# alanqrwang/nwhead

Measured on AMD Instinct MI355X. Metric: query-predictions/sec, higher is better.
Workload: dtype f32; 1 GPU; K3 predict('full'): B=256 queries/step vs bank N=50000 d=512 C=200, bank sharded 1-way, 26 query batches coalesced per launch; B=256, N_support=50000, d=512, C=200, parallelism=support-shard x1

## Files before the change

include/nwhead_hip.h:

```cpp
#ifndef NWHEAD_HIP_H
#define NWHEAD_HIP_H

#include <stddef.h>
#include <stdint.h>

#ifdef __cplusplus
extern "C" {
#endif

#define NW_ABI_VERSION 2

typedef enum {
    NW_SCORE_EUCLIDEAN = 0,
    NW_SCORE_HYPERSPHERE = 1,
    NW_SCORE_COSINE = 2,
    NW_SCORE_DOT = 3,
    NW_SCORE_CLIP = 4
} nw_score_kind;

typedef enum {
    NW_OK = 0,
    NW_ERR_INVALID_ARG = -1,
    NW_ERR_UNSUPPORTED = -2,
    NW_ERR_WORKSPACE = -3,
    NW_ERR_LAUNCH = -4,
    NW_ERR_NO_DEVICE = -5
} nw_status;

int nw_abi_version(void);
const char *nw_status_string(int status);
int nw_device_check(void);

int nw_scores_f32(const float *q, const float *s, float *scores,
                  int64_t B, int64_t N, int64_t d,
                  int kind, const float *logit_scale_dev, int sup_batched, void *stream);

int nw_row_norm2_f32(const float *x, float *n2, int64_t rows, int64_t d, void *stream);

int nw_split_rows_f16x2(const float *x, float *out_split, float *row_scale, float *row_norm2,
                        int64_t rows, int64_t d, void *stream);

int nw_pack_rows_f16(const float *x, uint16_t *out_rows, float *row_scale, float *row_norm2,
                     int64_t rows, int64_t d, void *stream);

int nw_bank_update_rows_f32(const float *x, const int64_t *rows, int64_t R, int64_t dx, float momentum,
                            float *s_rows, float *s_user, float *s_norm2,
                            float *s_split, float *s_scale,
                            void *s_f16, float *f16_scale, float *f16_norm2,
                            int64_t N, int64_t d, void *stream);

typedef struct nw_fwd_opts {
    uint32_t struct_size;
    int32_t persistent_wgs;
    int32_t force_split;
    int32_t operand_form;
    const void *tables;
    size_t tables_bytes;
    const int64_t *tables_sy;
    int64_t tables_N;
} nw_fwd_opts;

size_t nw_fwd_workspace_bytes(int64_t B, int64_t N, int64_t d, int64_t C);
int nw_fwd_f32(const float *q, const float *s, const int64_t *sy, const float *s_norm2,
               const float *s_split, const float *s_scale,
               float *out, float *scores_out, float *lse_out, float *weights_out,
               void *workspace, size_t workspace_bytes,
               int64_t B, int64_t N, int64_t d, int64_t C,
               int kind, const float *logit_scale_dev,
               int sup_batched, int labels_batched, const nw_fwd_opts *opts, void *stream);

int nw_fwd_partial_f32(const float *q, const float *s, const int64_t *sy, const float *s_norm2,
                       const float *s_split, const float *s_scale,
                       float *m, float *den, float *num,
                       void *workspace, size_t workspace_bytes,
                       int64_t B, int64_t N, int64_t d, int64_t C,
                       int kind, const float *logit_scale_dev, const nw_fwd_opts *opts, void *stream);
int nw_merge_finalize_f32(const float *m, const float *den, const float *num, float *out,
                          int64_t G, int64_t B, int64_t C,
                          int64_t stride_m, int64_t stride_den, int64_t stride_num,
                          const int64_t *class_lo, int64_t C_local, void *stream);

size_t nw_bank_tables_bytes(int64_t N);
int nw_bank_tables_build(const int64_t *sy, int64_t N, int64_t C, void *tables, size_t tables_bytes, void *stream);


size_t nw_bwd_workspace_bytes(int64_t B, int64_t N, int64_t d, int64_t C, int kind, int sup_batched);
int nw_bwd_f32(const float *q, const float *s, const int64_t *sy,
               const float *scores, const float *lse, const float *out, const float *gout,
               float *gq, float *gs, float *glogit_scale,
               void *workspace, size_t workspace_bytes,
               int64_t B, int64_t N, int64_t d, int64_t C,
               int kind, const float *logit_scale_dev,
               int sup_batched, int labels_batched, void *stream);
int nw_bwd_uses_split(int64_t B, int64_t N, int64_t d, int64_t C, int sup_batched);
int nw_bwd_bank_f32(const float *q, const float *s, const float *s_norm2, const float *s_split,
                    const float *s_scale, const int64_t *sy,
                    const float *scores, const float *lse, const float *out, const float *gout,
                    float *gq, float *gs, float *glogit_scale,
                    void *workspace, size_t workspace_bytes,
                    int64_t B, int64_t N, int64_t d, int64_t C,
                    int kind, const float *logit_scale_dev,
                    int sup_batched, int labels_batched, void *stream);


int nw_support_influence_f32(const float *probs, const int64_t *qy, const float *w,
                             const int64_t *sy, float *infl,
                             int64_t B, int64_t N, int64_t C, void *stream);

int nw_aggregate_f32(const float *scores, const int64_t *sy, float *out, float *lse_out, float *weights_out,
                     int64_t B, int64_t N, int64_t C, int labels_batched, void *stream);
int nw_aggregate_bwd_f32(const float *scores, const int64_t *sy, const float *lse, const float *out, const float *gout,
                         float *gscores, int64_t B, int64_t N, int64_t C, int labels_batched, void *stream);

int nw_fwd_influence_f32(const float *q, const float *s, const int64_t *sy, const float *s_norm2,
                         const float *s_split, const float *s_scale, const int64_t *qy,
                         float *out, float *lse_out, float *infl_out,
                         void *workspace, size_t workspace_bytes,
                         int64_t B, int64_t N, int64_t d, int64_t C,
                         int kind, const float *logit_scale_dev, const nw_fwd_opts *opts, void *stream);

int nw_topk_f32(const float *scores, int64_t *idx_out, float *val_out,
                int64_t B, int64_t N, int64_t k, void *stream);

size_t nw_knn_workspace_bytes(int64_t B, int64_t N, int64_t d, int64_t k);
int nw_knn_f32(const float *q, const float *s_split, const float *s_scale, const float *s_norm2,
               int64_t *idx_out, float *val_out, void *workspace, size_t workspace_bytes,
               int64_t B, int64_t N, int64_t d, int64_t k, int kind, const float *logit_scale_dev,
               void *stream);
int nw_knn_window_f32(const float *q, const float *s_split, const float *s_scale, const float *s_norm2,
                      const int32_t *row_lo, const int32_t *row_hi, int exclude,
                      int64_t *idx_out, float *val_out, void *workspace, size_t workspace_bytes,
                      int64_t B, int64_t N, int64_t d, int64_t k, int kind, const float *logit_scale_dev,
                      void *stream);
int nw_fwd_window_f32(const float *q, const float *s_split, const float *s_scale, const float *s_norm2,
                      const int64_t *sy, const int32_t *row_lo, const int32_t *row_hi, int exclude,
                      float *out, float *lse_out, void *workspace, size_t workspace_bytes,
                      int64_t B, int64_t N, int64_t d, int64_t C, int kind, const float *logit_scale_dev,
                      void *stream);
size_t nw_bwd_query_workspace_bytes(int64_t B, int64_t N, int64_t d, int64_t C, int row_chunks);
int nw_bwd_query_f32(const float *q, const float *s_split, const float *s_scale, const float *s_norm2,
                     const int64_t *sy, const int32_t *row_lo, const int32_t *row_hi, int exclude,
                     const float *lse, const float *out, const float *gout,
                     float *gq, float *glogit_scale, void *workspace, size_t workspace_bytes,
                     int64_t B, int64_t N, int64_t d, int64_t C, int kind, const float *logit_scale_dev,
                     int row_chunks, void *stream);
int nw_fwd_weighted_f32(const float *q, const float *s_split, const float *s_scale, const float *s_norm2,
                        const int64_t *sy, const float *row_logw,
                        const int32_t *row_lo, const int32_t *row_hi, int exclude,
                        float *out, float *lse_out, void *workspace, size_t workspace_bytes,
                        int64_t B, int64_t N, int64_t d, int64_t C, int kind, const float *logit_scale_dev, void *stream);
int nw_bwd_query_weighted_f32(const float *q, const float *s_split, const float *s_scale, const float *s_norm2,
                              const int64_t *sy, const float *row_logw,
                              const int32_t *row_lo, const int32_t *row_hi, int exclude,
                              const float *lse, const float *out, const float *gout,
                              float *gq, float *glogit_scale, void *workspace, size_t workspace_bytes,
                              int64_t B, int64_t N, int64_t d, int64_t C, int kind, const float *logit_scale_dev,
                              int row_chunks, void *stream);
size_t nw_bwd_logw_workspace_bytes(int64_t B, int64_t N, int64_t d, int64_t C, int row_chunks, int want_gq);
int nw_bwd_query_logw_f32(const float *q, const float *s_split, const float *s_scale, const float *s_norm2,
                          const int64_t *sy, const float *row_logw,
                          const int32_t *row_lo, const int32_t *row_hi, int exclude,
                          const float *lse, const float *out, const float *gout,
                          float *gq, float *glogw, float *glogit_scale, void *workspace, size_t workspace_bytes,
                          int64_t B, int64_t N, int64_t d, int64_t C, int kind, const float *logit_scale_dev,
                          int row_chunks, void *stream);
size_t nw_fwd_values_workspace_bytes(int64_t B, int64_t N, int64_t d, int64_t T, int row_chunks);
int nw_fwd_values_f32(const float *q, const float *s_split, const float *s_scale, const float *s_norm2,
                      const float *v_split, const float *v_scale, const float *row_logw,
                      const int32_t *row_lo, const int32_t *row_hi, int exclude,
                      const float *lse, float *out, void *workspace, size_t workspace_bytes,
                      int64_t B, int64_t N, int64_t d, int64_t T, int kind, const float *logit_scale_dev,
                      int row_chunks, void *stream);
size_t nw_bwd_values_query_workspace_bytes(int64_t B, int64_t N, int64_t d, int64_t T, int row_chunks);
int nw_bwd_values_query_f32(const float *q, const float *s_split, const float *s_scale, const float *s_norm2,
                            const float *v_split, const float *v_scale, const float *row_logw,
                            const int32_t *row_lo, const int32_t *row_hi, int exclude,
                            const float *lse, const float *out, const float *gout,
                            float *gq, float *glogit_scale, void *workspace, size_t workspace_bytes,
                            int64_t B, int64_t N, int64_t d, int64_t T, int kind, const float *logit_scale_dev,
                            int row_chunks, void *stream);
size_t nw_bwd_values_support_workspace_bytes(int64_t B, int64_t N, int64_t d, int64_t T, int query_chunks, int want_gvalues);
int nw_bwd_values_support_f32(const float *q, const float *s_split, const float *s_scale, const float *s_norm2,
                              const float *v_rows, const float *row_logw,
                              const int32_t *row_lo, const int32_t *row_hi, int exclude,
                              const float *lse, const float *out, const float *gout,
                              float *gvalues, float *glogw, void *workspace, size_t workspace_bytes,
                              int64_t B, int64_t N, int64_t d, int64_t T, int kind, const float *logit_scale_dev,
                              int query_chunks, void *stream);
int nw_influence_select_f32(const float *vals, const int64_t *rows, const int64_t *sy, const int64_t *qy,
                            const float *out, const float *lse, float *infl_out, int64_t *label_out,
                            int64_t B, int64_t k, int64_t N, int64_t C, void *stream);
int nw_scores_use_split(int64_t B, int64_t N, int64_t d);

size_t nw_knn_f16_workspace_bytes(int64_t B, int64_t N, int64_t d, int64_t k);
int nw_knn_f16(const float *q, const void *s_f16, const float *s_scale, const float *s_norm2,
               int64_t *idx_out, float *val_out, void *workspace, size_t workspace_bytes,
               int64_t B, int64_t N, int64_t d, int64_t k, int kind, const float *logit_scale_dev,
               const nw_fwd_opts *opts, void *stream);

int nw_knn_merge_f32(const float *vals, const int32_t *rows, const int32_t *labels,
                     int64_t G, int64_t B, int64_t kc, int64_t stride_g, int64_t k, int64_t C,
                     int64_t *idx_out, float *val_out, int64_t *label_out, float *out, void *stream);

int nw_scale_shift_relu_f32(const float *x, const float *scale, const float *shift, float *out,
                            int64_t n, int64_t c, int64_t hw, int64_t x_batch_stride, int relu,
                            void *stream);
int nw_scale_shift_relu_avgpool2_f32(const float *x, const float *scale, const float *shift, float *out,
                                     int64_t n, int64_t c, int64_t h, int64_t w, int64_t x_batch_stride,
                                     int relu, void *stream);

int nw_bias_act_nhwc_f32(const float *x, const float *bias, const float *residual, int relu, float *out,
                         int64_t rows, int64_t c, void *stream);

size_t nw_conv1x1_workspace_bytes(int64_t n, int64_t cin, int64_t cout, int64_t hw);
int nw_conv1x1_f32(const float *x, int64_t x_batch_stride, const float *pre_scale, const float *pre_shift,
                   int pre_relu, const float *w_t, const float *bias, int post_relu, float *out,
                   int64_t out_batch_stride, void *workspace, size_t workspace_bytes,
                   int64_t n, int64_t cin, int64_t cout, int64_t hw, void *stream);

size_t nw_conv3x3_workspace_bytes(int64_t n, int64_t cin, int64_t cout, int64_t H, int64_t W);
int nw_conv3x3_f32(const float *x, int64_t x_batch_stride, const float *w_t, const float *bias,
                   const float *residual, int64_t res_batch_stride, int post_relu, float *out,
                   int64_t out_batch_stride, void *workspace, size_t workspace_bytes,
                   int64_t n, int64_t cin, int64_t cout, int64_t H, int64_t W, void *stream);
int64_t nw_conv3x3_workgroups(int64_t n, int64_t cin, int64_t cout, int64_t H, int64_t W);


#define NW_AMAX_SLOTS 256
int nw_absmax_f32(const float *x, int64_t count, float *amax_out, void *stream);
int nw_to_nhwc_pad_f32(const float *x, float *y, float *amax_out, int64_t n, int64_t c, int64_t hw, int64_t cp,
                       int64_t stride_n, int64_t stride_c, int64_t stride_p, void *stream);
int nw_conv2d_nhwc_supported(int64_t n, int64_t H, int64_t W, int64_t Cin, int64_t Cout, int64_t KH, int64_t KW,
                             int64_t stride, int64_t pad);
int nw_conv2d_nhwc_f16x2(const float *x, const float *amax_in, const float *w_split, const float *w_scale,
                         const float *bias, const float *residual, int relu, float *y, float *amax_out,
                         int64_t n, int64_t H, int64_t W, int64_t Cin, int64_t Cout, int64_t KH, int64_t KW,
                         int64_t stride, int64_t pad, int64_t ldx, int64_t ldy, float *moments, void *stream);
int nw_conv2d_nhwc_bnrelu_f16x2(const float *x, const float *pre, const float *amax_in, int64_t raw_records,
                                const float *w_split, const float *w_scale, const float *bias, int relu, float *y,
                                float *amax_out, int64_t n,
                                int64_t H, int64_t W, int64_t Cin, int64_t Cout, int64_t KH, int64_t KW, int64_t stride,
                                int64_t pad, int64_t ldx, int64_t ldy, float *moments, void *stream);
int64_t nw_conv2d_nhwc_moments_groups(int64_t n, int64_t H, int64_t W, int64_t Cin, int64_t Cout, int64_t KH, int64_t KW,
                                      int64_t stride, int64_t pad);

int nw_bn_relu_train_fwd_f32(const float *x, const float *residual, const float *gamma, const float *beta, float *running_mean,
                             float *running_var, float *y, float *save_mean, float *save_invstd,
                             int64_t *num_batches_tracked, int64_t n, int64_t c, int64_t hw,
                             int64_t x_batch_stride, float momentum, float eps, int relu, void *stream);
int nw_bn_relu_train_bwd_f32(const float *x, const float *residual, const float *dy, const float *gamma,
                             const float *beta, const float *save_mean, const float *save_invstd, float *dx,
                             float *dresidual, float *dgamma, float *dbeta, const float *acc,
                             int64_t acc_batch_stride, int64_t n, int64_t c, int64_t hw,
                             int64_t x_batch_stride, int relu, void *stream);

int nw_split_conv_weights_f16x2(const int64_t *jobs, int64_t njobs, int64_t total_rows, float *split_base,
                                float *scale_base, void *stream);

int nw_conv2d_nhwc_wgrad_supported(int64_t n, int64_t H, int64_t W, int64_t Cin, int64_t Cout, int64_t KH, int64_t KW,
                                   int64_t stride, int64_t pad);
size_t nw_conv2d_nhwc_wgrad_workspace_bytes(int64_t n, int64_t H, int64_t W, int64_t Cin, int64_t Cout, int64_t KH,
                                            int64_t KW, int64_t stride, int64_t pad);
int nw_conv2d_nhwc_wgrad_f16x2(const float *x, const float *amax_x, const float *gy, const float *amax_g, float *dw,
                               void *workspace, size_t workspace_bytes, int64_t n, int64_t H, int64_t W, int64_t Cin,
                               int64_t Cout, int64_t KH, int64_t KW, int64_t stride, int64_t pad, int64_t ldx, int64_t ldg,
                               void *stream);
typedef struct nw_wgrad_job {
    const float *x, *amax_x, *gy, *amax_g;
    float *dw;
    int64_t n, H, W, Cin, Cout, KH, KW, stride, pad, ldx, ldg;
    int64_t out_oihw;
    const float *pre_x;
    int64_t rowrun_stride, in_H, in_W, row0, col0;
} nw_wgrad_job;
size_t nw_conv2d_nhwc_wgrad_batch_workspace_bytes(const nw_wgrad_job *jobs, int64_t njobs);
int nw_conv2d_nhwc_wgrad_batch_f16x2(const nw_wgrad_job *jobs, int64_t njobs, void *workspace, size_t workspace_bytes,
                                     void *stream);
const void *nw_conv_zero_page(void);

size_t nw_bn_nhwc_workspace_bytes(int64_t rows, int64_t c);
int nw_bn_relu_nhwc_train_fwd_f32(const float *x, int64_t ldx, const float *gamma, const float *beta, float *running_mean,
                                  float *running_var, float *y, float *save_mean, float *save_invstd,
                                  int64_t *num_batches_tracked, float *amax_out, void *workspace, size_t workspace_bytes,
                                  int64_t rows, int64_t c, float momentum, float eps, int relu, void *stream);
int nw_bn_nhwc_moments_f32(const float *x, int64_t ldx, int64_t rows, int64_t c, float eps, float *mean, float *invstd,
                           float *var, void *workspace, size_t workspace_bytes, void *stream);
int nw_bn_nhwc_moments_from_partials_f32(float *partials, int64_t groups, int64_t c, float eps, float *mean,
                                         float *invstd, float *var, void *stream);
int nw_bn_nhwc_moments_minmax_f32(const float *x, int64_t ldx, int64_t rows, int64_t c, float eps, float *mean, float *invstd,
                                  float *var, float *vmin, float *vmax, void *workspace, size_t workspace_bytes, void *stream);
size_t nw_bn_nhwc_minmax_workspace_bytes(int64_t rows, int64_t c);
int nw_bn_nhwc_prep_from_partials_f32(float *partials, int64_t groups, int64_t c, float eps, float *mean, float *invstd,
                                      float *var, float *vmin, float *vmax, const float *gamma, const float *beta,
                                      float *running_mean, float *running_var, int64_t *num_batches_tracked, float momentum,
                                      int relu, float *tab, float *amax_out, void *stream);
int nw_bn_nhwc_prep_window_from_partials_f32(float *partials, int64_t groups, int64_t c, int64_t offset, int64_t n_old, int64_t rows,
                                             float eps, float *mean, float *invstd, float *var, float *vmin, float *vmax,
                                             const float *gamma, const float *beta, float *running_mean, float *running_var,
                                             int64_t *num_batches_tracked, float momentum, int relu, float *tab, float *amax_out,
                                             void *stream);
int nw_bn_nhwc_prep_f32(const float *mean, const float *invstd, const float *var, const float *vmin, const float *vmax,
                        const float *gamma, const float *beta, float *running_mean, float *running_var,
                        int64_t *num_batches_tracked, float momentum, int relu, int64_t rows, int64_t c, float *tab,
                        float *amax_out, void *stream);
int nw_bn_relu_nhwc_apply_f32(const float *x, int64_t ldx, const float *mean, const float *invstd, const float *var,
                              const float *gamma, const float *beta, float *running_mean, float *running_var,
                              int64_t *num_batches_tracked, float momentum, float *y, float *amax_out, int64_t rows,
                              int64_t c, int relu, void *stream);
int nw_stem7x7s2_relu_maxpool_supported(int64_t n, int64_t H, int64_t W, int64_t cout);
int nw_stem7x7s2_relu_maxpool_f16x2(const float *x4, const float *amax_in, const float *w_split, const float *w_scale,
                                    const float *bias, float *y, float *amax_out, int64_t n, int64_t H, int64_t W, int64_t ldy,
                                    void *stream);
int nw_bn_relu_avgpool2x2_nhwc_f32(const float *x, int64_t ldx, const float *tab, float *y, int64_t ldy, float *amax_out,
                                   int64_t n, int64_t h, int64_t w, int64_t c, void *stream);
int nw_add_relu_f32(const float *a, const float *b, float *out, float *amax_out, int64_t count, void *stream);
int nw_relu_bwd_f32(const float *out, const float *g, float *dx, float *amax_out, int64_t count, void *stream);
int nw_bn_relu_nhwc_train_bwd_f32(const float *x, int64_t ldx, const float *dy, const float *gamma, const float *beta,
                                  const float *save_mean, const float *save_invstd, float *dx, float *dgamma,
                                  float *dbeta, const float *acc, int64_t ldacc, int64_t lddx, float *amax_out,
                                  void *workspace, size_t workspace_bytes, int64_t rows, int64_t c, int relu, void *stream);

int nw_avgpool2x2_nhwc_f32(const float *x, int64_t ldx, float *y, int64_t ldy, int64_t n, int64_t h, int64_t w, int64_t c,
                           void *stream);
int nw_avgpool2x2_nhwc_bwd_f32(const float *gy, int64_t ldgy, float *gx, int64_t ldgx, int64_t n, int64_t h, int64_t w,
                               int64_t c, void *stream);
int nw_maxpool3x3s2_nhwc_f32(const float *x, int64_t ldx, float *y, int64_t ldy, unsigned char *tap, int64_t n, int64_t h,
                             int64_t w, int64_t c, void *stream);
int nw_maxpool3x3s2_nhwc_bwd_f32(const float *gy, int64_t ldgy, const unsigned char *tap, float *gx, int64_t ldgx, int64_t n,
                                 int64_t h, int64_t w, int64_t c, void *stream);

typedef struct nw_sgd_param {
    float *param;
    const float *grad;
    float *momentum_buf;
    int64_t n;
} nw_sgd_param;
int nw_sgd_step_f32(const nw_sgd_param *params, int64_t nparams, float lr, float momentum, float weight_decay, int nesterov,
                    int init_buf, void *stream);

int nw_debug_tile_timing(int enable);
int nw_debug_set(const char *name, int value);
int nw_debug_tile_timing_read(double *total_us, int64_t *launches);
typedef struct nw_fwd_plan {
    int32_t status;
    int32_t rs, bs, n_stiles, n_qtiles, grid;
    int32_t mode, out;
    int32_t dma, persistent, variant, workgroups, qgroup;
    int32_t split_queries, run_tables;
    int32_t reserved;
    uint64_t lds_bytes;
} nw_fwd_plan;
int nw_debug_fwd_plan(int64_t B, int64_t N, int64_t d, int64_t C, int form, int outputs, int k, int norms, int kind,
                      int persistent_wgs, int cus, nw_fwd_plan *plan);
#define NW_FWD_AREAS 6
typedef struct nw_fwd_layout {
    uint64_t off[NW_FWD_AREAS], bytes[NW_FWD_AREAS];
    uint64_t total;
    int32_t n_slices, reserved;
} nw_fwd_layout;
int nw_debug_fwd_layout(int64_t B, int64_t N, int64_t d, int64_t C, nw_fwd_layout *layout);
#define NW_BWD_AREAS 15
typedef struct nw_bwd_plan {
    int32_t status, route;
    int32_t coeff_threads, parts_shared;
    int32_t gq_chunks, gq_k_chunk, gs_chunks, gs_k_chunk;
    int64_t ld, Bpad;
    uint64_t coeff_lds_bytes;
    uint64_t off[NW_BWD_AREAS], bytes[NW_BWD_AREAS];
    uint64_t total;
} nw_bwd_plan;
int nw_debug_bwd_plan(int64_t B, int64_t N, int64_t d, int64_t C, int sup_batched, nw_bwd_plan *plan);

#ifdef __cplusplus
}
#endif
#endif
```

nwhead_amd/_lib.py:

```python
from __future__ import annotations

import ctypes as C
import os

_HERE = os.path.dirname(os.path.abspath(__file__))
LIB_PATH = os.environ.get("NW_HIP_LIB") or os.path.join(_HERE, "csrc", "libnwhead_hip.so")

SCORE_KINDS = {"euclidean": 0, "hypersphere_euclidean": 1, "cosine": 2, "dotproduct": 3, "clip": 4}

_p = C.c_void_p
_i64 = C.c_int64
_int = C.c_int
_sz = C.c_size_t

SIGNATURES = {
    "nw_abi_version": (_int, []),
    "nw_status_string": (C.c_char_p, [_int]),
    "nw_device_check": (_int, []),
    "nw_scores_f32": (_int, [_p, _p, _p, _i64, _i64, _i64, _int, _p, _int, _p]),
    "nw_fwd_workspace_bytes": (_sz, [_i64, _i64, _i64, _i64]),
    "nw_row_norm2_f32": (_int, [_p, _p, _i64, _i64, _p]),
    "nw_split_rows_f16x2": (_int, [_p, _p, _p, _p, _i64, _i64, _p]),
    "nw_pack_rows_f16": (_int, [_p, _p, _p, _p, _i64, _i64, _p]),
    "nw_bank_update_rows_f32": (_int, [_p, _p, _i64, _i64, C.c_float, _p, _p, _p, _p, _p, _p, _p, _p, _i64, _i64, _p]),
    "nw_fwd_f32": (_int, [_p, _p, _p, _p, _p, _p, _p, _p, _p, _p, _p, _sz, _i64, _i64, _i64, _i64, _int, _p, _int, _int, _p, _p]),
    "nw_fwd_partial_f32": (_int, [_p, _p, _p, _p, _p, _p, _p, _p, _p, _p, _sz, _i64, _i64, _i64, _i64, _int, _p, _p, _p]),
    "nw_merge_finalize_f32": (_int, [_p, _p, _p, _p, _i64, _i64, _i64, _i64, _i64, _i64, _p, _i64, _p]),
    "nw_bank_tables_bytes": (_sz, [_i64]),
    "nw_bank_tables_build": (_int, [_p, _i64, _i64, _p, _sz, _p]),
    "nw_bwd_workspace_bytes": (_sz, [_i64, _i64, _i64, _i64, _int, _int]),
    "nw_bwd_f32": (_int, [_p] * 10 + [_p, _sz, _i64, _i64, _i64, _i64, _int, _p, _int, _int, _p]),
    "nw_bwd_uses_split": (_int, [_i64, _i64, _i64, _i64, _int]),
    "nw_bwd_bank_f32": (_int, [_p] * 13 + [_p, _sz, _i64, _i64, _i64, _i64, _int, _p, _int, _int, _p]),
    "nw_support_influence_f32": (_int, [_p, _p, _p, _p, _p, _i64, _i64, _i64, _p]),
    "nw_aggregate_f32": (_int, [_p] * 5 + [_i64, _i64, _i64, _int, _p]),
    "nw_aggregate_bwd_f32": (_int, [_p] * 6 + [_i64, _i64, _i64, _int, _p]),
    "nw_fwd_influence_f32": (_int, [_p] * 11 + [_sz, _i64, _i64, _i64, _i64, _int, _p, _p, _p]),
    "nw_topk_f32": (_int, [_p, _p, _p, _i64, _i64, _i64, _p]),
    "nw_knn_workspace_bytes": (_sz, [_i64, _i64, _i64, _i64]),
    "nw_scores_use_split": (_int, [_i64, _i64, _i64]),
    "nw_knn_f32": (_int, [_p, _p, _p, _p, _p, _p, _p, _sz, _i64, _i64, _i64, _i64, _int, _p, _p]),
    "nw_knn_window_f32": (_int, [_p, _p, _p, _p, _p, _p, _int, _p, _p, _p, _sz, _i64, _i64, _i64, _i64, _int, _p, _p]),
    "nw_fwd_window_f32": (_int, [_p, _p, _p, _p, _p, _p, _p, _int, _p, _p, _p, _sz, _i64, _i64, _i64, _i64, _int, _p, _p]),
    "nw_fwd_weighted_f32": (_int, [_p, _p, _p, _p, _p, _p, _p, _p, _int, _p, _p, _p, _sz, _i64, _i64, _i64, _i64, _int, _p, _p]),
    "nw_bwd_query_workspace_bytes": (_sz, [_i64, _i64, _i64, _i64, _int]),
    "nw_bwd_query_f32": (_int, [_p, _p, _p, _p, _p, _p, _p, _int, _p, _p, _p, _p, _p, _p, _sz, _i64, _i64, _i64, _i64, _int, _p, _int, _p]),
    "nw_bwd_query_weighted_f32": (_int, [_p, _p, _p, _p, _p, _p, _p, _p, _int, _p, _p, _p, _p, _p, _p, _sz, _i64, _i64, _i64, _i64, _int, _p,
                                         _int, _p]),
    "nw_bwd_logw_workspace_bytes": (_sz, [_i64, _i64, _i64, _i64, _int, _int]),
    "nw_bwd_query_logw_f32": (_int, [_p, _p, _p, _p, _p, _p, _p, _p, _int, _p, _p, _p, _p, _p, _p, _p, _sz, _i64, _i64, _i64, _i64, _int,
                                     _p, _int, _p]),
    "nw_fwd_values_workspace_bytes": (_sz, [_i64, _i64, _i64, _i64, _int]),
    "nw_fwd_values_f32": (_int, [_p, _p, _p, _p, _p, _p, _p, _p, _p, _int, _p, _p, _p, _sz, _i64, _i64, _i64, _i64, _int, _p, _int, _p]),
    "nw_bwd_values_query_workspace_bytes": (_sz, [_i64, _i64, _i64, _i64, _int]),
    "nw_bwd_values_query_f32": (_int, [_p, _p, _p, _p, _p, _p, _p, _p, _p, _int, _p, _p, _p, _p, _p, _p, _sz, _i64, _i64, _i64, _i64,
                                       _int, _p, _int, _p]),
    "nw_bwd_values_support_workspace_bytes": (_sz, [_i64, _i64, _i64, _i64, _int, _int]),
    "nw_bwd_values_support_f32": (_int, [_p, _p, _p, _p, _p, _p, _p, _p, _int, _p, _p, _p, _p, _p, _p, _sz, _i64, _i64, _i64, _i64,
                                         _int, _p, _int, _p]),
    "nw_influence_select_f32": (_int, [_p] * 8 + [_i64, _i64, _i64, _i64, _p]),
    "nw_knn_f16_workspace_bytes": (_sz, [_i64, _i64, _i64, _i64]),
    "nw_knn_f16": (_int, [_p, _p, _p, _p, _p, _p, _p, _sz, _i64, _i64, _i64, _i64, _int, _p, _p, _p]),
    "nw_knn_merge_f32": (_int, [_p, _p, _p, _i64, _i64, _i64, _i64, _i64, _i64, _p, _p, _p, _p, _p]),
    "nw_scale_shift_relu_f32": (_int, [_p, _p, _p, _p, _i64, _i64, _i64, _i64, _int, _p]),
    "nw_bias_act_nhwc_f32": (_int, [_p, _p, _p, _int, _p, _i64, _i64, _p]),
    "nw_scale_shift_relu_avgpool2_f32": (_int, [_p, _p, _p, _p, _i64, _i64, _i64, _i64, _i64, _int, _p]),
    "nw_conv3x3_workgroups": (_i64, [_i64, _i64, _i64, _i64, _i64]),
    "nw_conv3x3_workspace_bytes": (_sz, [_i64, _i64, _i64, _i64, _i64]),
    "nw_conv3x3_f32": (_int, [_p, _i64, _p, _p, _p, _i64, _int, _p, _i64, _p, _sz, _i64, _i64, _i64, _i64, _i64, _p]),
    "nw_conv1x1_workspace_bytes": (_sz, [_i64, _i64, _i64, _i64]),
    "nw_conv1x1_f32": (_int, [_p, _i64, _p, _p, _int, _p, _p, _int, _p, _i64, _p, _sz, _i64, _i64, _i64, _i64, _p]),
    "nw_bn_relu_train_fwd_f32": (_int, [_p] * 10 + [_i64, _i64, _i64, _i64, C.c_float, C.c_float, _int, _p]),
    "nw_bn_relu_train_bwd_f32": (_int, [_p] * 12 + [_i64, _i64, _i64, _i64, _i64, _int, _p]),
    "nw_absmax_f32": (_int, [_p, _i64, _p, _p]),
    "nw_to_nhwc_pad_f32": (_int, [_p, _p, _p, _i64, _i64, _i64, _i64, _i64, _i64, _i64, _p]),
    "nw_conv2d_nhwc_supported": (_int, [_i64] * 9),
    "nw_conv2d_nhwc_f16x2": (_int, [_p, _p, _p, _p, _p, _p, _int, _p, _p] + [_i64] * 11 + [_p, _p]),
    "nw_conv2d_nhwc_moments_groups": (_i64, [_i64] * 9),
    "nw_stem7x7s2_relu_maxpool_supported": (_int, [_i64] * 4),
    "nw_stem7x7s2_relu_maxpool_f16x2": (_int, [_p] * 7 + [_i64] * 4 + [_p]),
    "nw_bn_relu_avgpool2x2_nhwc_f32": (_int, [_p, _i64, _p, _p, _i64, _p, _i64, _i64, _i64, _i64, _p]),
    "nw_add_relu_f32": (_int, [_p, _p, _p, _p, _i64, _p]),
    "nw_relu_bwd_f32": (_int, [_p, _p, _p, _p, _i64, _p]),
    "nw_bn_nhwc_moments_f32": (_int, [_p, _i64, _i64, _i64, C.c_float, _p, _p, _p, _p, _sz, _p]),
    "nw_bn_nhwc_moments_from_partials_f32": (_int, [_p, _i64, _i64, C.c_float, _p, _p, _p, _p]),
    "nw_bn_nhwc_moments_minmax_f32": (_int, [_p, _i64, _i64, _i64, C.c_float, _p, _p, _p, _p, _p, _p, _sz, _p]),
    "nw_bn_nhwc_minmax_workspace_bytes": (_sz, [_i64, _i64]),
    "nw_bn_nhwc_prep_from_partials_f32": (_int, [_p, _i64, _i64, C.c_float, _p, _p, _p, _p, _p, _p, _p, _p, _p, _p, C.c_float, _int,
                                                 _p, _p, _p]),
    "nw_bn_nhwc_prep_window_from_partials_f32": (_int, [_p, _i64, _i64, _i64, _i64, _i64, C.c_float, _p, _p, _p, _p, _p, _p, _p, _p, _p,
                                                        _p, C.c_float, _int, _p, _p, _p]),
    "nw_bn_nhwc_prep_f32": (_int, [_p, _p, _p, _p, _p, _p, _p, _p, _p, _p, C.c_float, _int, _i64, _i64, _p, _p, _p]),
    "nw_conv2d_nhwc_bnrelu_f16x2": (_int, [_p] * 3 + [_i64] + [_p] * 3 + [_int, _p, _p] + [_i64] * 11 + [_p, _p]),
    "nw_bn_relu_nhwc_apply_f32": (_int, [_p, _i64] + [_p] * 8 + [C.c_float, _p, _p, _i64, _i64, _int, _p]),
    "nw_split_conv_weights_f16x2": (_int, [_p, _i64, _i64, _p, _p, _p]),
    "nw_conv2d_nhwc_wgrad_supported": (_int, [_i64] * 9),
    "nw_conv2d_nhwc_wgrad_workspace_bytes": (_sz, [_i64] * 9),
    "nw_conv2d_nhwc_wgrad_f16x2": (_int, [_p, _p, _p, _p, _p, _p, _sz] + [_i64] * 11 + [_p]),
    "nw_conv_zero_page": (_p, []),
    "nw_conv2d_nhwc_wgrad_batch_workspace_bytes": (_sz, [_p, _i64]),
    "nw_conv2d_nhwc_wgrad_batch_f16x2": (_int, [_p, _i64, _p, _sz, _p]),
    "nw_bn_nhwc_workspace_bytes": (_sz, [_i64, _i64]),
    "nw_bn_relu_nhwc_train_fwd_f32": (_int, [_p, _i64] + [_p] * 10 + [_sz, _i64, _i64, C.c_float, C.c_float, _int, _p]),
    "nw_bn_relu_nhwc_train_bwd_f32": (_int, [_p, _i64] + [_p] * 9 + [_i64, _i64, _p, _p, _sz, _i64, _i64, _int, _p]),
    "nw_avgpool2x2_nhwc_f32": (_int, [_p, _i64, _p, _i64, _i64, _i64, _i64, _i64, _p]),
    "nw_avgpool2x2_nhwc_bwd_f32": (_int, [_p, _i64, _p, _i64, _i64, _i64, _i64, _i64, _p]),
    "nw_maxpool3x3s2_nhwc_f32": (_int, [_p, _i64, _p, _i64, _p, _i64, _i64, _i64, _i64, _p]),
    "nw_maxpool3x3s2_nhwc_bwd_f32": (_int, [_p, _i64, _p, _p, _i64, _i64, _i64, _i64, _i64, _p]),
    "nw_sgd_step_f32": (_int, [_p, _i64, C.c_float, C.c_float, C.c_float, _int, _int, _p]),
    "nw_debug_set": (_int, [C.c_char_p, _int]),
    "nw_debug_tile_timing": (_int, [_int]),
    "nw_debug_tile_timing_read": (_int, [C.POINTER(C.c_double), C.POINTER(C.c_int64)]),
    "nw_debug_fwd_plan": (_int, [_i64, _i64, _i64, _i64, _int, _int, _int, _int, _int, _int, _int, _p]),
    "nw_debug_fwd_layout": (_int, [_i64, _i64, _i64, _i64, _p]),
    "nw_debug_bwd_plan": (_int, [_i64, _i64, _i64, _i64, _int, _p]),
}

_lib = None


class NWHipError(RuntimeError):
    pass


def load():
    global _lib
    if _lib is not None:
        return _lib
    if not os.path.exists(LIB_PATH):
        raise NWHipError(
            f"{LIB_PATH} not found: the HIP extension is not built. Run __graft_entry__.build() "
            "(or `make -C nwhead_amd/csrc`). There is no CPU fallback.")
    import torch
    lib = C.CDLL(LIB_PATH)
    for name, (res, args) in SIGNATURES.items():
        fn = getattr(lib, name)
        fn.restype = res
        fn.argtypes = args
    if lib.nw_abi_version() != 2:
        raise NWHipError("libnwhead_hip.so ABI version mismatch")
    _lib = lib
    sync_knobs()
    return lib


class WgradJob(C.Structure):
    _fields_ = [("x", C.c_void_p), ("amax_x", C.c_void_p), ("gy", C.c_void_p), ("amax_g", C.c_void_p), ("dw", C.c_void_p)] + \
               [(k, C.c_int64) for k in ("n", "H", "W", "Cin", "Cout", "KH", "KW", "stride", "pad", "ldx", "ldg", "out_oihw")] + \
               [("pre_x", C.c_void_p)] + [(k, C.c_int64) for k in ("rowrun_stride", "in_H", "in_W", "row0", "col0")]


class SgdParam(C.Structure):
    _fields_ = [("param", C.c_void_p), ("grad", C.c_void_p), ("momentum_buf", C.c_void_p), ("n", C.c_int64)]


class FwdOpts(C.Structure):
    _fields_ = [("struct_size", C.c_uint32), ("persistent_wgs", C.c_int32), ("force_split", C.c_int32),
                ("operand_form", C.c_int32), ("tables", C.c_void_p), ("tables_bytes", C.c_size_t),
                ("tables_sy", C.c_void_p), ("tables_N", C.c_int64)]


class FwdPlan(C.Structure):
    _fields_ = [(k, C.c_int32) for k in ("status", "rs", "bs", "n_stiles", "n_qtiles", "grid", "mode", "out", "dma", "persistent",
                                         "variant", "workgroups", "qgroup", "split_queries", "run_tables", "reserved")] + \
               [("lds_bytes", C.c_uint64)]


FORMS = {"fp32": 0, "split": 1, "half": 2}
OUTPUTS = {"log_probs": 0, "scores": 1, "candidates": 2}


def fwd_plan(B, N, d, C_, form="split", outputs="log_probs", k=0, norms=True, kind="euclidean", persistent_wgs=0, cus=0):
    p = FwdPlan()
    check(load().nw_debug_fwd_plan(B, N, d, C_, FORMS[form], OUTPUTS[outputs], k, int(norms), SCORE_KINDS[kind],
                                   persistent_wgs, cus, C.byref(p)), "nw_debug_fwd_plan")
    return p


FWD_AREAS = ("main", "q_rows", "q_scale", "q_norm2", "lse", "slices")


class FwdLayout(C.Structure):
    _fields_ = [("off", C.c_uint64 * len(FWD_AREAS)), ("bytes", C.c_uint64 * len(FWD_AREAS)), ("total", C.c_uint64),
                ("n_slices", C.c_int32), ("reserved", C.c_int32)]


def fwd_layout(B, N, d, C_):
    m = FwdLayout()
    check(load().nw_debug_fwd_layout(B, N, d, C_, C.byref(m)), "nw_debug_fwd_layout")
    return m


BWD_ROUTES = ("valu", "mfma", "split")
BWD_AREAS = ("A", "Rs", "rq", "gls", "qn2", "sn2", "rs", "s_split", "s_scale", "q_split", "ascale", "qv", "gfac", "part", "part2")


class BwdPlan(C.Structure):
    _fields_ = [(k, C.c_int32) for k in ("status", "route", "coeff_threads", "parts_shared", "gq_chunks", "gq_k_chunk",
                                         "gs_chunks", "gs_k_chunk")] + \
               [("ld", C.c_int64), ("Bpad", C.c_int64), ("coeff_lds_bytes", C.c_uint64),
                ("off", C.c_uint64 * len(BWD_AREAS)), ("bytes", C.c_uint64 * len(BWD_AREAS)), ("total", C.c_uint64)]


def bwd_plan(B, N, d, C_, sup=0):
    p = BwdPlan()
    check(load().nw_debug_bwd_plan(B, N, d, C_, int(sup), C.byref(p)), "nw_debug_bwd_plan")
    return p


KNOBS = ("pvar", "qg", "tile_rs", "no_persistent", "split_queries", "bwd_no_mfma", "bwd_split",
         "xgemm_wgs", "split_lbits", "conv_max_wgs", "conv_skip_cfgs", "conv_force_cfg")
_KNOB_UNSET = -2 ** 31
_knob_state = {}


def sync_knobs():
    if _lib is None:
        return
    for k in KNOBS:
        v = os.environ.get("NW_" + k.upper())
        val = _KNOB_UNSET if v is None or v == "" else int(v)
        if _knob_state.get(k, _KNOB_UNSET) != val:
            _lib.nw_debug_set(k.encode(), val)
            _knob_state[k] = val


def force_split():
    return os.environ.get("NW_SPLIT_ALWAYS", "") == "1"


def fwd_opts(tables=None, tables_bytes=0, persistent_wgs=0, tables_sy=None, tables_n=-1, operand_form=0):
    return FwdOpts(C.sizeof(FwdOpts), int(persistent_wgs), int(force_split()), int(operand_form), tables, int(tables_bytes),
                   tables_sy, int(tables_n))


def check(status: int, what: str):
    if status != 0:
        msg = load().nw_status_string(status).decode()
        raise NWHipError(f"{what}: {msg} (status {status})")
```

nwhead_amd/csrc/capi.hip:

```cpp
#include <cstddef>
#include <cstdlib>
#include <string.h>
#include "nw_internal.h"
#include "fused_plan.h"
#include "bwd_plan.h"

namespace {
inline bool bad_kind(int kind) { return kind < NW_SCORE_EUCLIDEAN || kind > NW_SCORE_CLIP; }
}

extern "C" int nw_scores_use_split(int64_t B, int64_t N, int64_t d);
static bool split_pays(int64_t B, int64_t N, int64_t d) {
    return nw::fwd_opts().force_split || nw_scores_use_split(B, N, d) != 0;
}
static bool takes_split(const float* q, const float* s_split, const float* s_scale, const float* s_norm2, int64_t B, int64_t N,
                        int64_t d) {
    return s_split && s_scale && s_norm2 && d % 32 == 0 && split_pays(B, N, d) &&
           ((reinterpret_cast<uintptr_t>(s_split) | reinterpret_cast<uintptr_t>(q)) & 15) == 0;
}

namespace nw {
namespace {
thread_local FwdOpts tl_fwd_opts;
int g_knobs[KNOB_COUNT];
bool g_knobs_init = [] { for (int& k : g_knobs) k = KNOB_UNSET; return true; }();
const char* const knob_names[KNOB_COUNT] = {
    "pvar", "qg", "tile_rs", "no_persistent", "split_queries", "bwd_no_mfma", "bwd_split",
    "xgemm_wgs", "split_lbits", "conv_max_wgs", "conv_skip_cfgs", "conv_force_cfg"};
}
const FwdOpts& fwd_opts() { return tl_fwd_opts; }
int knob(int id) { return (id >= 0 && id < KNOB_COUNT) ? __atomic_load_n(&g_knobs[id], __ATOMIC_RELAXED) : KNOB_UNSET; }
}

namespace {
struct OptsGuard {
    nw::FwdOpts saved;
    explicit OptsGuard(const nw_fwd_opts* o) : saved(nw::tl_fwd_opts) {
        nw::FwdOpts f;
        if (o && o->struct_size >= offsetof(nw_fwd_opts, tables)) {
            f.persistent_wgs = o->persistent_wgs;
            f.force_split = o->force_split;
            f.operand_form = o->operand_form;
        }
        if (o && o->struct_size >= sizeof(nw_fwd_opts)) {
            f.tables = static_cast<const char*>(o->tables);
            f.tables_bytes = o->tables_bytes;
            f.tables_sy = o->tables_sy;
            f.tables_N = o->tables_N;
        }
        nw::tl_fwd_opts = f;
    }
    ~OptsGuard() { nw::tl_fwd_opts = saved; }
};
}

static int half_form_check(const float* q, const float* s, const float* s_norm2, const float* s_split, const float* s_scale,
                           const void* per_pair_out, int batched, int64_t B, int64_t N, int64_t d, int64_t C) {
    if (per_pair_out || batched) return NW_ERR_UNSUPPORTED;
    if (!nw::half_form_shape_ok(d)) return NW_ERR_UNSUPPORTED;
    if (B == 0 || N == 0 || C == 0) return NW_OK;
    if (!s_split || !s_scale || !s_norm2) return NW_ERR_INVALID_ARG;
    if ((reinterpret_cast<uintptr_t>(s_split) | reinterpret_cast<uintptr_t>(q)) & 15) return NW_ERR_INVALID_ARG;
    if (!nw::fused_eligible(q, s_split, B, N, d, C)) return NW_ERR_UNSUPPORTED;
    (void)s;
    return NW_OK;
}

extern "C" int nw_debug_set(const char* name, int value) {
    if (!name) return NW_ERR_INVALID_ARG;
    for (int k = 0; k < nw::KNOB_COUNT; ++k)
        if (!strcmp(name, nw::knob_names[k])) {
            __atomic_store_n(&nw::g_knobs[k], value, __ATOMIC_RELAXED);
            return NW_OK;
        }
    return NW_ERR_INVALID_ARG;
}

extern "C" int nw_debug_fwd_plan(int64_t B, int64_t N, int64_t d, int64_t C, int form, int outputs, int k, int norms, int kind,
                                 int persistent_wgs, int cus, nw_fwd_plan* plan) {
    if (!plan || B < 0 || N < 0 || d < 0 || C < 0 || k < 0 || cus < 0 || cus > (1 << 20)) return NW_ERR_INVALID_ARG;
    if (form < nw::FORM_F32 || form > nw::FORM_HALF || outputs < nw::OUT_NONE || outputs > nw::OUT_CAND) return NW_ERR_INVALID_ARG;
    if (bad_kind(kind)) return NW_ERR_UNSUPPORTED;
    nw::FwdOpts o;
    o.persistent_wgs = persistent_wgs;
    const nw::FusedPlan p = nw::plan_fused(B, N, d, C, form, outputs, k, norms != 0, kind == NW_SCORE_DOT, cus, o);
    *plan = {p.status, p.rs, p.BS, p.n_stiles, p.n_qtiles, p.grid, p.mode, p.out, p.dma, p.persistent, p.variant, p.workgroups,
             p.qgroup, p.split_queries, p.run_tables, 0, (uint64_t)p.lds_bytes};
    return NW_OK;
}

extern "C" int nw_abi_version(void) { return NW_ABI_VERSION; }

extern "C" const char* nw_status_string(int status) {
    switch (status) {
        case NW_OK: return "ok";
        case NW_ERR_INVALID_ARG: return "invalid argument";
        case NW_ERR_UNSUPPORTED: return "unsupported score kind or size";
        case NW_ERR_WORKSPACE: return "workspace too small";
        case NW_ERR_LAUNCH: return "HIP launch failed";
        case NW_ERR_NO_DEVICE: return "no gfx950 device";
        default: return "unknown status";
    }
}

extern "C" int nw_device_check(void) {
    int n = 0;
    if (hipGetDeviceCount(&n) != hipSuccess || n <= 0) return NW_ERR_NO_DEVICE;
    int dev = 0;
    if (hipGetDevice(&dev) != hipSuccess) return NW_ERR_NO_DEVICE;
    hipDeviceProp_t prop;
    if (hipGetDeviceProperties(&prop, dev) != hipSuccess) return NW_ERR_NO_DEVICE;
    return strncmp(prop.gcnArchName, "gfx950", 6) == 0 ? NW_OK : NW_ERR_NO_DEVICE;
}

extern "C" int nw_scores_f32(const float* q, const float* s, float* scores, int64_t B, int64_t N,
                             int64_t d, int kind, const float* logit_scale_dev, int sup_batched,
                             void* stream) {
    if (B < 0 || N < 0 || d < 0) return NW_ERR_INVALID_ARG;
    if (bad_kind(kind)) return NW_ERR_UNSUPPORTED;
    if (B == 0 || N == 0) return NW_OK;
    if (!q || !s || !scores) return NW_ERR_INVALID_ARG;
    if (kind == NW_SCORE_CLIP && !logit_scale_dev) return NW_ERR_INVALID_ARG;
    return nw::launch_scores(q, s, scores, B, N, d, kind, logit_scale_dev, sup_batched,
                             static_cast<hipStream_t>(stream));
}

extern "C" size_t nw_fwd_workspace_bytes(int64_t B, int64_t N, int64_t d, int64_t C) {
    return nw::fwd_layout(B, N, d, C, nullptr).total;
}

extern "C" int nw_debug_fwd_layout(int64_t B, int64_t N, int64_t d, int64_t C, nw_fwd_layout* layout) {
    if (!layout || B < 0 || N < 0 || d < 0 || C < 0) return NW_ERR_INVALID_ARG;
    const nw::FwdLayout L = nw::fwd_layout(B, N, d, C, nullptr);
    const nw::FwdLayout::Area* const areas[NW_FWD_AREAS] = {&L.main, &L.q_rows, &L.q_scale, &L.q_norm2, &L.lse, &L.slices};
    *layout = {};
    for (int i = 0; i < NW_FWD_AREAS; ++i) layout->off[i] = areas[i]->off, layout->bytes[i] = areas[i]->bytes;
    layout->total = L.total;
    layout->n_slices = L.n_slices;
    return NW_OK;
}

extern "C" int nw_debug_bwd_plan(int64_t B, int64_t N, int64_t d, int64_t C, int sup_batched, nw_bwd_plan* plan) {
    static_assert(NW_BWD_AREAS == nw::BWD_AREAS, "nw_bwd_plan lists the areas of nw::BwdPlan");
    if (!plan || B < 0 || N < 0 || d < 0 || C < 0) return NW_ERR_INVALID_ARG;
    const nw::BwdPlan p = nw::plan_bwd(B, N, d, C, sup_batched);
    *plan = {};
    plan->status = p.status, plan->route = p.route, plan->coeff_threads = (int32_t)p.coeff_threads, plan->parts_shared = p.parts_shared;
    plan->gq_chunks = p.gq.nchunks, plan->gq_k_chunk = p.gq.k_chunk, plan->gs_chunks = p.gs.nchunks, plan->gs_k_chunk = p.gs.k_chunk;
    plan->ld = p.ld, plan->Bpad = p.Bpad, plan->coeff_lds_bytes = p.coeff_lds, plan->total = p.total;
    for (int i = 0; i < NW_BWD_AREAS; ++i) plan->off[i] = p.area[i].off, plan->bytes[i] = p.area[i].bytes;
    return NW_OK;
}

extern "C" int nw_row_norm2_f32(const float* x, float* n2, int64_t rows, int64_t d, void* stream) {
    if (rows < 0 || d < 0) return NW_ERR_INVALID_ARG;
    if (rows == 0) return NW_OK;
    if (!x || !n2) return NW_ERR_INVALID_ARG;
    return nw::launch_rownorm2(x, n2, rows, d, static_cast<hipStream_t>(stream));
}

static int fwd_f32(const float* q, const float* s, const int64_t* sy, const float* s_norm2, const float* s_split,
                   const float* s_scale, float* out, float* scores_out, float* lse_out, float* weights_out, void* workspace,
                   size_t workspace_bytes, const nw::FwdLayout* carved, int64_t B, int64_t N, int64_t d, int64_t C, int kind,
                   const float* logit_scale_dev, int sup_batched, int labels_batched, hipStream_t st) {
    if (B < 0 || N < 0 || d < 0 || C < 0) return NW_ERR_INVALID_ARG;
    if (bad_kind(kind)) return NW_ERR_UNSUPPORTED;
    if (B == 0) return NW_OK;
    if (!out && C > 0) return NW_ERR_INVALID_ARG;
    if (N > 0 && (!q || !s || !sy)) return NW_ERR_INVALID_ARG;
    if (kind == NW_SCORE_CLIP && !logit_scale_dev) return NW_ERR_INVALID_ARG;
    if (labels_batched && !sup_batched) return NW_ERR_INVALID_ARG;
    const int form = nw::fwd_opts().operand_form;
    if (form != 0 && form != 1) return NW_ERR_INVALID_ARG;
    const nw::FwdLayout L = carved ? *carved : nw::fwd_layout(B, N, d, C, workspace);
    nw::FusedArgs a = {q, s, sy, s_norm2, nullptr, logit_scale_dev, out, scores_out, lse_out, nullptr, nullptr, nullptr,
                       &L, (int)B, (int)N, (int)d, (int)C, st, nullptr};
    if (form == 1) {
        const int rc = half_form_check(q, s, s_norm2, s_split, s_scale, scores_out ? scores_out : weights_out,
                                       sup_batched || labels_batched, B, N, d, C);
        if (rc != NW_OK) return rc;
        if (N > 0 && C > 0) {
            if (!L.fits(workspace_bytes)) return NW_ERR_WORKSPACE;
            a.s = s_split, a.s_scale = s_scale;
            return nw::launch_fused(a, nw::FORM_HALF, kind);
        }
    }
    float* sc_buf = scores_out ? scores_out : weights_out;
    if (N > 0 && C > 0 && !sup_batched && nw::fused_eligible(q, s, B, N, d, C) &&
        (!sc_buf || (reinterpret_cast<uintptr_t>(sc_buf) & 15) == 0)) {
        if (!L.fits(workspace_bytes)) return NW_ERR_WORKSPACE;
        a.scores = sc_buf;
        if (weights_out && !a.lse) a.lse = L.at(L.lse);
        const bool split = takes_split(q, s_split, s_scale, s_norm2, B, N, d);
        if (split) a.s = s_split, a.s_scale = s_scale;
        const int rc = nw::launch_fused(a, split ? nw::FORM_SPLIT : nw::FORM_F32, kind);
        if (rc != NW_OK || !weights_out) return rc;
        return nw::launch_weights_from_scores(sc_buf, a.lse, weights_out, B, N, st);
    }
    float* scores = scores_out;
    if (!scores && N > 0) {
        if (!L.fits(workspace_bytes)) return NW_ERR_WORKSPACE;
        scores = L.at(L.main);
    }
    int rc = nw::launch_scores(q, s, scores, B, N, d, kind, logit_scale_dev, sup_batched, st);
    if (rc != NW_OK) return rc;
    const bool sliced = L.n_slices > 1 && L.fits(workspace_bytes);
    return nw::launch_aggregate(scores, sy, labels_batched, out, lse_out, weights_out, nullptr, nullptr, nullptr, B, N, C, st,
                                sliced ? L.at(L.slices) : nullptr, sliced ? L.slices.bytes / sizeof(float) : 0);
}

extern "C" int nw_fwd_f32(const float* q, const float* s, const int64_t* sy, const float* s_norm2,
                          const float* s_split, const float* s_scale, float* out, float* scores_out, float* lse_out, float* weights_out, void* workspace,
                          size_t workspace_bytes, int64_t B, int64_t N, int64_t d, int64_t C,
                          int kind, const float* logit_scale_dev, int sup_batched,
                          int labels_batched, const nw_fwd_opts* opts, void* stream) {
    OptsGuard opts_guard(opts);
    return fwd_f32(q, s, sy, s_norm2, s_split, s_scale, out, scores_out, lse_out, weights_out, workspace, workspace_bytes, nullptr,
                   B, N, d, C, kind, logit_scale_dev, sup_batched, labels_batched, static_cast<hipStream_t>(stream));
}

bool nw::bank_head_shape_ok(int64_t N, int64_t d, int64_t C) { return N > 25 && C >= 1 && d >= 32 && d % 32 == 0 && d <= (1 << 20); }

namespace {
enum { NEED_WINDOW = 1, NEED_LOGW = 2, NEED_GQ = 4, NEED_GLOGW = 8 };
inline uintptr_t addr(const void* p) { return reinterpret_cast<uintptr_t>(p); }

struct BankFwdCall {
    const float *q, *s_split, *s_scale, *s_norm2;
    const int64_t* sy;
    const float* row_logw;
    const int32_t *row_lo, *row_hi;
    int exclude;
    float *out, *lse_out;
    void* workspace;
    size_t workspace_bytes;
    int64_t B, N, d, C;
    int kind;
    const float* logit_scale_dev;
    void* stream;
};
int bank_fwd_checked(const BankFwdCall& c, int needs) {
    if (c.B < 0 || c.N < 0 || c.d < 0 || c.C < 0) return NW_ERR_INVALID_ARG;
    if ((c.row_lo != nullptr) != (c.row_hi != nullptr) || ((needs & NEED_WINDOW) && !c.row_lo)) return NW_ERR_INVALID_ARG;
    if (bad_kind(c.kind)) return NW_ERR_UNSUPPORTED;
    if (!nw::bank_head_shape_ok(c.N, c.d, c.C)) return NW_ERR_UNSUPPORTED;
    if (c.B == 0) return NW_OK;
    if (!c.q || !c.s_split || !c.s_scale || !c.s_norm2 || !c.sy || !c.out || ((needs & NEED_LOGW) && !c.row_logw))
        return NW_ERR_INVALID_ARG;
    if (c.kind == NW_SCORE_CLIP && !c.logit_scale_dev) return NW_ERR_INVALID_ARG;
    if (!nw::fused_eligible(c.q, c.s_split, c.B, c.N, c.d, c.C)) return NW_ERR_UNSUPPORTED;
    if (addr(c.row_logw) & 15) return NW_ERR_UNSUPPORTED;
    const nw::FwdLayout L = nw::fwd_layout(c.B, c.N, c.d, c.C, c.workspace);
    if (!L.fits(c.workspace_bytes)) return NW_ERR_WORKSPACE;
    if (addr(c.workspace) & 15) return NW_ERR_UNSUPPORTED;
    nw::FusedArgs a = {c.q, c.s_split, c.sy, c.s_norm2, c.s_scale, c.logit_scale_dev, c.out, nullptr, c.lse_out, nullptr, nullptr,
                       nullptr, &L, (int)c.B, (int)c.N, (int)c.d, (int)c.C, static_cast<hipStream_t>(c.stream), nullptr,
                       c.row_lo, c.row_hi, c.row_lo && c.exclude != 0, c.row_logw};
    return nw::launch_fused(a, nw::FORM_SPLIT, c.kind);
}

int bank_bwd_checked(const nw::BwdQueryCall& c, int needs) {
    if (c.B < 0 || c.N < 0 || c.d < 0 || c.C < 0 || c.row_chunks < 0) return NW_ERR_INVALID_ARG;
    if ((c.row_lo != nullptr) != (c.row_hi != nullptr)) return NW_ERR_INVALID_ARG;
    if (bad_kind(c.kind)) return NW_ERR_UNSUPPORTED;
    if (!nw::bwd_query_shape_ok(c.B, c.N, c.d, c.C)) return NW_ERR_UNSUPPORTED;
    if (c.B == 0) return NW_OK;
    if (!c.q || !c.s_split || !c.s_scale || !c.s_norm2 || !c.sy || !c.lse || !c.out || !c.gout ||
        ((needs & NEED_LOGW) && !c.row_logw) || ((needs & NEED_GQ) && !c.gq) || ((needs & NEED_GLOGW) && !c.glogw))
        return NW_ERR_INVALID_ARG;
    if (c.kind == NW_SCORE_CLIP && !c.logit_scale_dev) return NW_ERR_INVALID_ARG;
    if ((addr(c.q) | addr(c.s_split) | addr(c.gq) | addr(c.row_logw) | addr(c.glogw)) & 15) return NW_ERR_UNSUPPORTED;
    const size_t need = c.glogw ? nw::bwd_logw_workspace_bytes(c.B, c.N, c.d, c.C, c.row_chunks, c.gq != nullptr)
                                : nw::bwd_query_workspace_bytes(c.B, c.N, c.d, c.C, c.row_chunks);
    if (!c.workspace || c.workspace_bytes < need) return NW_ERR_WORKSPACE;
    if (addr(c.workspace) & 15) return NW_ERR_UNSUPPORTED;
    return nw::launch_bwd_query(c);
}
}

extern "C" int nw_fwd_window_f32(const float* q, const float* s_split, const float* s_scale, const float* s_norm2,
                                 const int64_t* sy, const int32_t* row_lo, const int32_t* row_hi, int exclude, float* out,
                                 float* lse_out, void* workspace, size_t workspace_bytes, int64_t B, int64_t N, int64_t d,
                                 int64_t C, int kind, const float* logit_scale_dev, void* stream) {
    return bank_fwd_checked({q, s_split, s_scale, s_norm2, sy, nullptr, row_lo, row_hi, exclude, out, lse_out, workspace,
                             workspace_bytes, B, N, d, C, kind, logit_scale_dev, stream}, NEED_WINDOW);
}

extern "C" int nw_fwd_weighted_f32(const float* q, const float* s_split, const float* s_scale, const float* s_norm2,
                                   const int64_t* sy, const float* row_logw, const int32_t* row_lo, const int32_t* row_hi,
                                   int exclude, float* out, float* lse_out, void* workspace, size_t workspace_bytes, int64_t B,
                                   int64_t N, int64_t d, int64_t C, int kind, const float* logit_scale_dev, void* stream) {
    return bank_fwd_checked({q, s_split, s_scale, s_norm2, sy, row_logw, row_lo, row_hi, exclude, out, lse_out, workspace,
                             workspace_bytes, B, N, d, C, kind, logit_scale_dev, stream}, NEED_LOGW);
}

extern "C" size_t nw_bwd_query_workspace_bytes(int64_t B, int64_t N, int64_t d, int64_t C, int row_chunks) {
    if (B <= 0 || N < 0 || d < 0 || C < 0) return 0;
    return nw::bwd_query_workspace_bytes(B, N, d, C, row_chunks);
}

extern "C" size_t nw_bwd_logw_workspace_bytes(int64_t B, int64_t N, int64_t d, int64_t C, int row_chunks, int want_gq) {
    if (B <= 0 || N < 0 || d < 0 || C < 0) return 0;
    return nw::bwd_logw_workspace_bytes(B, N, d, C, row_chunks, want_gq != 0);
}

extern "C" int nw_bwd_query_f32(const float* q, const float* s_split, const float* s_scale, const float* s_norm2,
                                const int64_t* sy, const int32_t* row_lo, const int32_t* row_hi, int exclude,
                                const float* lse, const float* out, const float* gout, float* gq, float* glogit_scale,
                                void* workspace, size_t workspace_bytes, int64_t B, int64_t N, int64_t d, int64_t C,
                                int kind, const float* logit_scale_dev, int row_chunks, void* stream) {
    return bank_bwd_checked({q, s_split, s_scale, s_norm2, sy, row_lo, row_hi, exclude, lse, out, gout, gq, glogit_scale,
                             workspace, workspace_bytes, B, N, d, C, kind, logit_scale_dev, row_chunks,
                             static_cast<hipStream_t>(stream), nullptr, nullptr}, NEED_GQ);
}

extern "C" int nw_bwd_query_weighted_f32(const float* q, const float* s_split, const float* s_scale, const float* s_norm2,
                                         const int64_t* sy, const float* row_logw, const int32_t* row_lo, const int32_t* row_hi,
                                         int exclude, const float* lse, const float* out, const float* gout, float* gq,
                                         float* glogit_scale, void* workspace, size_t workspace_bytes, int64_t B, int64_t N,
                                         int64_t d, int64_t C, int kind, const float* logit_scale_dev, int row_chunks,
                                         void* stream) {
    return bank_bwd_checked({q, s_split, s_scale, s_norm2, sy, row_lo, row_hi, exclude, lse, out, gout, gq, glogit_scale,
                             workspace, workspace_bytes, B, N, d, C, kind, logit_scale_dev, row_chunks,
                             static_cast<hipStream_t>(stream), row_logw, nullptr}, NEED_LOGW | NEED_GQ);
}

extern "C" int nw_bwd_query_logw_f32(const float* q, const float* s_split, const float* s_scale, const float* s_norm2,
                                     const int64_t* sy, const float* row_logw, const int32_t* row_lo, const int32_t* row_hi,
                                     int exclude, const float* lse, const float* out, const float* gout, float* gq, float* glogw,
                                     float* glogit_scale, void* workspace, size_t workspace_bytes, int64_t B, int64_t N,
                                     int64_t d, int64_t C, int kind, const float* logit_scale_dev, int row_chunks, void* stream) {
    return bank_bwd_checked({q, s_split, s_scale, s_norm2, sy, row_lo, row_hi, exclude, lse, out, gout, gq, glogit_scale,
                             workspace, workspace_bytes, B, N, d, C, kind, logit_scale_dev, row_chunks,
                             static_cast<hipStream_t>(stream), row_logw, glogw}, NEED_LOGW | NEED_GLOGW);
}

extern "C" size_t nw_fwd_values_workspace_bytes(int64_t B, int64_t N, int64_t d, int64_t T, int row_chunks) {
    if (B <= 0 || N < 0 || d < 0 || T < 0 || row_chunks < 0) return 0;
    return nw::fwd_values_workspace_bytes(B, N, d, T, row_chunks);
}

extern "C" int nw_fwd_values_f32(const float* q, const float* s_split, const float* s_scale, const float* s_norm2,
                                 const float* v_split, const float* v_scale, const float* row_logw, const int32_t* row_lo,
                                 const int32_t* row_hi, int exclude, const float* lse, float* out, void* workspace,
                                 size_t workspace_bytes, int64_t B, int64_t N, int64_t d, int64_t T, int kind,
                                 const float* logit_scale_dev, int row_chunks, void* stream) {
    if (B < 0 || N < 0 || d < 0 || T < 0 || row_chunks < 0) return NW_ERR_INVALID_ARG;
    if ((row_lo != nullptr) != (row_hi != nullptr)) return NW_ERR_INVALID_ARG;
    if (bad_kind(kind)) return NW_ERR_UNSUPPORTED;
    if (!nw::fwd_values_shape_ok(B, N, d, T)) return NW_ERR_UNSUPPORTED;
    if (B == 0) return NW_OK;
    if (!q || !s_split || !s_scale || !s_norm2 || !v_split || !v_scale || !lse || !out) return NW_ERR_INVALID_ARG;
    if (kind == NW_SCORE_CLIP && !logit_scale_dev) return NW_ERR_INVALID_ARG;
    if ((addr(q) | addr(s_split) | addr(v_split) | addr(out) | addr(row_logw)) & 15) return NW_ERR_UNSUPPORTED;
    const size_t need = nw::fwd_values_workspace_bytes(B, N, d, T, row_chunks);
    if (!workspace || workspace_bytes < need) return NW_ERR_WORKSPACE;
    if (addr(workspace) & 15) return NW_ERR_UNSUPPORTED;
    return nw::launch_fwd_values({q, s_split, s_scale, s_norm2, v_split, v_scale, row_logw, row_lo, row_hi, exclude, lse, out,
                                  workspace, workspace_bytes, B, N, d, T, kind, logit_scale_dev, row_chunks,
                                  static_cast<hipStream_t>(stream)});
}

extern "C" size_t nw_bwd_values_query_workspace_bytes(int64_t B, int64_t N, int64_t d, int64_t T, int row_chunks) {
    if (B <= 0 || N < 0 || d < 0 || T < 0 || row_chunks < 0) return 0;
    return nw::bwd_values_workspace_bytes(B, N, d, T, row_chunks);
}

extern "C" int nw_bwd_values_query_f32(const float* q, const float* s_split, const float* s_scale, const float* s_norm2,
                                       const float* v_split, const float* v_scale, const float* row_logw, const int32_t* row_lo,
                                       const int32_t* row_hi, int exclude, const float* lse, const float* out, const float* gout,
                                       float* gq, float* glogit_scale, void* workspace, size_t workspace_bytes, int64_t B,
// ... 197 lines not shown
```

nwhead_amd/csrc/fused.hip:

```cpp
#include <mutex>
#include <utility>
#include <vector>
#include "fused_impl.h"

namespace nw {

#define NW_EXTERN_FUSED_KIND(K) extern template int launch_fused_kind<K>(const FusedArgs&, const FusedPlan&);
NW_FOR_EACH_KIND(NW_EXTERN_FUSED_KIND)
#undef NW_EXTERN_FUSED_KIND

namespace {
struct TileTimer {
    bool on = false;
    std::vector<std::pair<hipEvent_t, hipEvent_t>> ev;
    std::vector<std::pair<hipEvent_t, hipEvent_t>> pool;
    std::mutex mu;
} g_tt;
}

int tile_timer_start(hipStream_t st) {
    if (!g_tt.on) return -1;
    std::lock_guard<std::mutex> lk(g_tt.mu);
    std::pair<hipEvent_t, hipEvent_t> p;
    if (!g_tt.pool.empty()) {
        p = g_tt.pool.back();
        g_tt.pool.pop_back();
    } else if (hipEventCreate(&p.first) != hipSuccess || hipEventCreate(&p.second) != hipSuccess) {
        return -1;
    }
    (void)hipEventRecord(p.first, st);
    g_tt.ev.push_back(p);
    return (int)g_tt.ev.size() - 1;
}
void tile_timer_stop(int slot, hipStream_t st) {
    if (slot < 0) return;
    std::lock_guard<std::mutex> lk(g_tt.mu);
    if (slot < (int)g_tt.ev.size()) (void)hipEventRecord(g_tt.ev[slot].second, st);
}
int tile_timer_enable(bool on) {
    std::lock_guard<std::mutex> lk(g_tt.mu);
    g_tt.on = on;
    return NW_OK;
}
int tile_timer_read(double* total_us, int64_t* launches) {
    std::lock_guard<std::mutex> lk(g_tt.mu);
    double tot = 0;
    for (auto& p : g_tt.ev) {
        float ms = 0.f;
        if (hipEventSynchronize(p.second) != hipSuccess || hipEventElapsedTime(&ms, p.first, p.second) != hipSuccess)
            return NW_ERR_LAUNCH;
        tot += (double)ms * 1e3;
        g_tt.pool.push_back(p);
    }
    if (total_us) *total_us = tot;
    if (launches) *launches = (int64_t)g_tt.ev.size();
    g_tt.ev.clear();
    return NW_OK;
}

namespace {
int device_cu_count() {
    static int n = [] {
        int dev = 0, v = 0;
        if (hipGetDevice(&dev) != hipSuccess) return 256;
        if (hipDeviceGetAttribute(&v, hipDeviceAttributeMultiprocessorCount, dev) != hipSuccess || v <= 0) return 256;
        return v;
    }();
    return n;
}
bool env_flag(int k) { return knob(k) == 1; }
}

inline size_t al256(size_t x) { return (x + 255) & ~(size_t)255; }

size_t fused_layout(int64_t B, int64_t n_stiles, int BS, char* base, FusedWs* ws, int64_t C) {
    size_t off = 0;
    auto take = [&](size_t bytes) {
        char* p = base ? base + off : nullptr;
        off += al256(bytes);
        return p;
    };
    FusedWs w;
    w.m = reinterpret_cast<float*>(take(fused_den_after_m(n_stiles, B) * sizeof(float)));
    w.den = reinterpret_cast<float*>(take((size_t)n_stiles * B * 4));
    w.nrun = reinterpret_cast<int*>(take((size_t)n_stiles * 4));
    w.lab = reinterpret_cast<int*>(take((size_t)n_stiles * BS * 4));
    w.num = reinterpret_cast<float*>(take((size_t)n_stiles * BS * B * 4));
    w.runid = reinterpret_cast<int*>(take(((size_t)n_stiles * BS + 64) * 4));
    w.bnd = reinterpret_cast<int*>(take((size_t)n_stiles * 2 * 4));
    w.ctab = reinterpret_cast<int*>(take((size_t)C * (3 + 4) * 4));
    if (ws) *ws = w;
    return off;
}

namespace {

constexpr int MTHREADS = 512, MENT = 4, MTPT = 16;
template <bool PARTIAL, int MQ, int TMODE>
__global__ __launch_bounds__(MTHREADS) void nw_merge_runs_kernel(
    const float* __restrict__ ws_m, const float* __restrict__ ws_den, const int* __restrict__ ws_nrun,
    const int* __restrict__ ws_lab, const float* __restrict__ ws_num, float* __restrict__ out,
    float* __restrict__ lse, float* __restrict__ m_out, float* __restrict__ den_out,
    float* __restrict__ num_out, int B, int C, int n_stiles, int BS, const int* __restrict__ ctab) {
    static_assert(TMODE == 1 || TMODE == 2, "the per-class tables live in LDS (1) or in the workspace (2)");
    constexpr bool LTAB = TMODE == 1;
    constexpr int ML = MTHREADS / MQ;
    constexpr int MNS = MQ + 1;
    constexpr int NW = MTHREADS / 64;
    constexpr float LN2 = 0.693147180559945309417f;
    static_assert(MQ <= 32 && (MQ & (MQ - 1)) == 0, "a wave holds whole groups of MQ queries");
    extern __shared__ __attribute__((aligned(16))) char smem[];
    float* red = reinterpret_cast<float*>(smem);
    float* Ms = red + 2 * NW * MQ;
    float* inv_s = Ms + MQ;
    int* lds_tab = reinterpret_cast<int*>(inv_s + MQ);
    int* cnt = TMODE == 2 ? const_cast<int*>(ctab) : lds_tab;
    int* tlo = cnt + C;
    int* thi = tlo + C;
    int* ent = thi + C;
    float* res = reinterpret_cast<float*>(lds_tab + (size_t)C * (3 + MENT));
    const int tid = threadIdx.x, bq = tid & (MQ - 1), sl = tid / MQ, wave = tid >> 6;
    const int b0 = blockIdx.x * MQ;
    const int b = min(b0 + bq, B - 1);

    const bool in_regs = n_stiles <= ML * MTPT;
    float mr[MTPT], dr[MTPT];
    float M = -INFINITY;
    if (in_regs) {
#pragma unroll
        for (int u = 0; u < MTPT; ++u) {
            const int t = sl + u * ML;
            const bool ok = t < n_stiles;
            mr[u] = ok ? ws_m[(size_t)t * B + b] : -INFINITY;
            dr[u] = ok ? ws_den[(size_t)t * B + b] : 0.f;
        }
    }
    int tnr = 0, tl3[3] = {-1, -1, -1};
    const bool one_pass_tables = LTAB && n_stiles <= MTHREADS;
    if (one_pass_tables && tid < n_stiles) {
        tnr = ws_nrun[tid];
        const int* lt = ws_lab + (size_t)tid * BS;
        tl3[0] = lt[0];
        tl3[1] = lt[1];
        tl3[2] = lt[2];
    }
    if (LTAB) {
        for (int c = tid; c < C; c += MTHREADS) {
            cnt[c] = 0;
            tlo[c] = 0x7fffffff;
            thi[c] = -1;
        }
    }
    if (in_regs) {
#pragma unroll
        for (int u = 0; u < MTPT; ++u) M = fmaxf(M, mr[u]);
    } else {
        for (int t = sl; t < n_stiles; t += ML) M = fmaxf(M, ws_m[(size_t)t * B + b]);
    }
#pragma unroll
    for (int o = 32; o >= MQ; o >>= 1) M = fmaxf(M, __shfl_xor(M, o));
    if ((tid & 63) < MQ) red[wave * MQ + bq] = M;
    __syncthreads();
    if (LTAB) {
        auto add_tile = [&](int t, int nr, const int (&l3)[3]) {
            const int* lt = ws_lab + (size_t)t * BS;
            for (int r = 0; r < nr; ++r) {
                const int y = r < 3 ? l3[r] : lt[r];
                if (y < 0) continue;
                atomicMin(&tlo[y], t);
                atomicMax(&thi[y], t);
                const int slot = atomicAdd(&cnt[y], 1);
                if (slot < MENT) ent[y * MENT + slot] = t * BS + r;
            }
        };
        if (one_pass_tables) {
            if (tid < n_stiles) add_tile(tid, tnr, tl3);
        } else {
            for (int t = tid; t < n_stiles; t += MTHREADS) {
                const int* lt = ws_lab + (size_t)t * BS;
                const int l3[3] = {lt[0], lt[1], lt[2]};
                add_tile(t, ws_nrun[t], l3);
            }
        }
    }
    M = red[bq];
#pragma unroll
    for (int k = 1; k < NW; ++k) M = fmaxf(M, red[k * MQ + bq]);
    const bool no_rows = M == -INFINITY;
    if (no_rows) M = 0.f;
    float den = 0.f;
    if (in_regs) {
#pragma unroll
        for (int u = 0; u < MTPT; ++u) den += dr[u] * __builtin_amdgcn_exp2f(mr[u] - M);
    } else {
        for (int t = sl; t < n_stiles; t += ML)
            den += ws_den[(size_t)t * B + b] * __builtin_amdgcn_exp2f(ws_m[(size_t)t * B + b] - M);
    }
#pragma unroll
    for (int o = 32; o >= MQ; o >>= 1) den += __shfl_xor(den, o);
    if ((tid & 63) < MQ) red[NW * MQ + wave * MQ + bq] = den;
    if (sl == 0) Ms[bq] = M;
    __syncthreads();
    if (LTAB) {
        for (int c = tid; c < C; c += MTHREADS) {
            const int n = cnt[c];
            if (n > 1 && n <= MENT) {
                int e[MENT];
#pragma unroll
                for (int k = 0; k < MENT; ++k) e[k] = k < n ? ent[c * MENT + k] : 0x7fffffff;
#pragma unroll
                for (int i = 1; i < MENT; ++i)
#pragma unroll
                    for (int j = MENT - 1; j >= i; --j)
                        if (e[j] < e[j - 1]) { const int x = e[j]; e[j] = e[j - 1]; e[j - 1] = x; }
#pragma unroll
                for (int k = 0; k < MENT; ++k)
                    if (k < n) ent[c * MENT + k] = e[k];
            }
        }
    }
    den = red[NW * MQ + bq];
#pragma unroll
    for (int k = 1; k < NW; ++k) den += red[NW * MQ + k * MQ + bq];
    if (sl == 0) inv_s[bq] = no_rows ? 0.f : 1.f / den;
    const int nq = min(MQ, B - b0);
    if (sl == 0 && bq < nq) {
        if (PARTIAL) {
            m_out[b] = M * LN2;
            den_out[b] = den;
        } else if (lse) {
            lse[b] = M * LN2 + logf(den);
        }
    }
    __syncthreads();
    int P = 1;
    while (P < 64 && 2 * P * C * MQ <= MTHREADS) P <<= 1;
    for (int xx = tid; xx < C * MQ * P; xx += MTHREADS) {
        const int x = xx / P, sub = xx - x * P;
        const int c = x / MQ, q = x - c * MQ;
        const int bb = min(b0 + q, B - 1);
        const float Mq = Ms[q];
        float acc = 0.f;
        const int n = cnt[c];
        if (n <= MENT) {
            int e[MENT];
            float v[MENT], mt[MENT];
#pragma unroll
            for (int k = 0; k < MENT; ++k) e[k] = ent[c * MENT + (k < n ? k : 0)];
#pragma unroll
            for (int k = 0; k < MENT; ++k) {
                if (k < n) {
                    v[k] = ws_num[(size_t)e[k] * B + bb];
                    mt[k] = ws_m[(size_t)(e[k] / BS) * B + bb];
                }
            }
#pragma unroll
            for (int k = 0; k < MENT; ++k)
                if (k < n) acc += v[k] * __builtin_amdgcn_exp2f(mt[k] - Mq);
        } else {
            const int t0 = tlo[c], t1 = thi[c];
            for (int t = t0 + sub; t <= t1; t += P) {
                const int nr = ws_nrun[t];
                const float f = __builtin_amdgcn_exp2f(ws_m[(size_t)t * B + bb] - Mq);
                const int* lt = ws_lab + (size_t)t * BS;
                for (int r = 0; r < nr; ++r)
                    if (lt[r] == c) acc += ws_num[((size_t)t * BS + r) * B + bb] * f;
            }
        }
        if (P > 1) {
            if (n <= MENT && sub != 0) acc = 0.f;
            for (int o = P >> 1; o > 0; o >>= 1) acc += __shfl_xor(acc, o);
            if (sub != 0) continue;
        }
        if (LTAB && MQ > 1) {
            res[c * MNS + q] = acc;
        } else if (q < nq) {
            if (PARTIAL) num_out[(size_t)bb * C + c] = acc;
            else out[(size_t)bb * C + c] = logf(acc * inv_s[q] + NW_LOG_EPS);
        }
    }
    if (!LTAB || MQ == 1) return;
    __syncthreads();
    for (int x = tid; x < nq * C; x += MTHREADS) {
        const int qq = x / C, c = x - qq * C;
        if (PARTIAL) num_out[(size_t)(b0 + qq) * C + c] = res[c * MNS + qq];
        else out[(size_t)(b0 + qq) * C + c] = logf(res[c * MNS + qq] * inv_s[qq] + NW_LOG_EPS);
    }
}

__global__ __launch_bounds__(1024) void nw_class_tables_kernel(const int* __restrict__ ws_nrun, const int* __restrict__ ws_lab,
                                                                int n_stiles, int BS, int C, int* __restrict__ ctab) {
    int* cnt = ctab;
    int* tlo = cnt + C;
    int* thi = tlo + C;
    int* ent = thi + C;
    const int tid = threadIdx.x;
    for (int c = tid; c < C; c += 1024) {
        cnt[c] = 0;
        tlo[c] = 0x7fffffff;
        thi[c] = -1;
    }
    __threadfence();
    __syncthreads();
    for (int t = tid; t < n_stiles; t += 1024) {
        const int nr = ws_nrun[t];
        const int* lt = ws_lab + (size_t)t * BS;
        for (int r = 0; r < nr; ++r) {
            const int y = lt[r];
            if (y < 0) continue;
            atomicMin(&tlo[y], t);
            atomicMax(&thi[y], t);
            const int slot = atomicAdd(&cnt[y], 1);
            if (slot < MENT) ent[y * MENT + slot] = t * BS + r;
        }
    }
    __threadfence();
    __syncthreads();
    for (int c = tid; c < C; c += 1024) {
        const int n = cnt[c];
        if (n > 1 && n <= MENT) {
            int e[MENT];
#pragma unroll
            for (int k = 0; k < MENT; ++k) e[k] = k < n ? ent[c * MENT + k] : 0x7fffffff;
#pragma unroll
            for (int i = 1; i < MENT; ++i)
#pragma unroll
                for (int j = MENT - 1; j >= i; --j)
                    if (e[j] < e[j - 1]) { const int x = e[j]; e[j] = e[j - 1]; e[j - 1] = x; }
#pragma unroll
            for (int k = 0; k < MENT; ++k)
                if (k < n) ent[c * MENT + k] = e[k];
        }
    }
}

__global__ __launch_bounds__(64) void nw_run_tables_kernel(const int64_t* __restrict__ sy, int N, int C, int BS,
                                                           int* __restrict__ runid, int* __restrict__ nrun,
                                                           int* __restrict__ lab_out, int* __restrict__ bnd) {
    const int st = blockIdx.x, lane = threadIdx.x, s0 = st * BS;
    if (lane < 2) bnd[2 * st + lane] = BS;
    __syncthreads();
    int lab[3], flag[3];
#pragma unroll
    for (int u = 0; u < 3; ++u) {
        const int t = 3 * lane + u, j = s0 + t;
        int64_t y = -1;
        if (t < BS && j < N) y = sy[j];
        lab[u] = ((uint64_t)y < (uint64_t)C) ? (int)y : -1;
    }
    const int prev_last = __shfl_up(lab[2], 1);
    flag[0] = (lane == 0) || (lab[0] != prev_last);
    flag[1] = lab[1] != lab[0];
    flag[2] = lab[2] != lab[1];
    int incl = flag[0] + flag[1] + flag[2];
#pragma unroll
    for (int o = 1; o < 64; o <<= 1) {
        const int v = __shfl_up(incl, o);
        if (lane >= o) incl += v;
    }
    int id = incl - (flag[0] + flag[1] + flag[2]) - 1;
#pragma unroll
    for (int u = 0; u < 3; ++u) {
        const int t = 3 * lane + u;
        id += flag[u];
        if (t < BS) {
            runid[(size_t)s0 + t] = id;
            if (flag[u]) lab_out[(size_t)s0 + id] = lab[u];
            if (flag[u] && (id == 1 || id == 2)) bnd[2 * st + id - 1] = t;
            if (t == BS - 1) nrun[st] = id + 1;
        }
    }
}

int env_rs() {
    const int v = knob(KNOB_TILE_RS);
    return v == KNOB_UNSET ? 0 : v;
}

}

int launch_run_tables(const FusedWs& ws, const int64_t* sy, int N, int C, int n_stiles, int BS, hipStream_t st) {
    if (BS > 192) return NW_ERR_UNSUPPORTED;
    hipLaunchKernelGGL(nw_run_tables_kernel, dim3(n_stiles), dim3(64), 0, st, sy, N, C, BS, ws.runid, ws.nrun, ws.lab, ws.bnd);
    NW_CHECK_LAUNCH();
    return NW_OK;
}

constexpr int BANK_BS = 128;

size_t bank_tables_layout(int64_t n_stiles, char* base, FusedWs* ws) {
    size_t off = 0;
    auto take = [&](size_t bytes) {
        char* p = base ? base + off : nullptr;
        off += al256(bytes);
        return p;
    };
    int* nrun = reinterpret_cast<int*>(take((size_t)n_stiles * 4));
    int* lab = reinterpret_cast<int*>(take((size_t)n_stiles * BANK_BS * 4));
    int* runid = reinterpret_cast<int*>(take(((size_t)n_stiles * BANK_BS + 64) * 4));
    int* bnd = reinterpret_cast<int*>(take((size_t)n_stiles * 2 * 4));
    if (ws) {
        ws->nrun = nrun;
        ws->lab = lab;
        ws->runid = runid;
        ws->bnd = bnd;
    }
    return off;
}

bool bank_tables_take(const int64_t* sy, int N, int C, int n_stiles, int BS, FusedWs* ws) {
    (void)C;
    const FwdOpts& o = fwd_opts();
    if (!o.tables || BS != BANK_BS) return false;
    if (o.tables_sy != sy || o.tables_N != (int64_t)N) return false;
    if (o.tables_bytes < bank_tables_layout(n_stiles, nullptr, nullptr)) return false;
    bank_tables_layout(n_stiles, const_cast<char*>(o.tables), ws);
    return true;
}

int launch_merge_runs(const FusedWs& ws, float* out, float* lse, float* m, float* den, float* num,
                      int B, int C, int n_stiles, int BS, hipStream_t st) {
    auto lds_bytes = [&](int mq, bool tables) {
        return ((size_t)2 * (MTHREADS / 64) * mq + 2 * mq + (tables ? (size_t)C * (3 + MENT + mq + 1) : 0)) * sizeof(float);
    };
    const size_t cap = 150 * 1024;
    int mq = 1;
    if (B >= 512) {
        mq = n_stiles >= 128 ? 16 : 32;
        if (lds_bytes(mq, true) > cap) mq = 16;
        if (lds_bytes(mq, true) > cap) mq = 1;
    }
    const bool tables = lds_bytes(mq, true) <= cap;
    const size_t lds = lds_bytes(mq, tables);
    const int grid = (B + mq - 1) / mq;
#define NW_MERGE(P_, Q_, T_)                                                                                       \
    hipLaunchKernelGGL((nw_merge_runs_kernel<P_, Q_, T_>), dim3(grid), dim3(MTHREADS), lds, st, ws.m, ws.den, ws.nrun, \
                       ws.lab, ws.num, out, lse, m, den, num, B, C, n_stiles, BS, ws.ctab)
    if (!tables) {
        hipLaunchKernelGGL(nw_class_tables_kernel, dim3(1), dim3(1024), 0, st, ws.nrun, ws.lab, n_stiles, BS, C, ws.ctab);
        if (out) NW_MERGE(false, 1, 2); else NW_MERGE(true, 1, 2);
    } else if (mq == 1) {
        if (out) NW_MERGE(false, 1, 1); else NW_MERGE(true, 1, 1);
    } else if (mq == 16) {
        if (out) NW_MERGE(false, 16, 1); else NW_MERGE(true, 16, 1);
    } else {
        if (out) NW_MERGE(false, 32, 1); else NW_MERGE(true, 32, 1);
    }
#undef NW_MERGE
    NW_CHECK_LAUNCH();
    return NW_OK;
}

int pick_rs(int64_t B, int64_t N, int64_t d, bool f16) {
    const int forced = env_rs();
    if (forced == 2 || forced == 4 || forced == 5 || forced == 6 || forced == 8 || forced == 10 || forced == 12)
        return forced;
    const int64_t nq = (B + BQ - 1) / BQ;
    if (forced == 0 && !f16 && d % BK == 0 && nq * ((N + 79) / 80) >= 480) return 5;
    if (forced == 0 && f16 && d % BK == 0 && nq * ((N + 127) / 128) >= 4 * 256) return 8;
    const int cand[] = {2, 4, 6, 8, 10, 12};
    const int ncand = f16 ? 5 : 6;
    double best = 1e30;
    int best_rs = 8;
    for (int ci = 0; ci < ncand; ++ci) {
        const int rs = cand[ci];
        const int64_t ns = (N + 16 * rs - 1) / (16 * rs);
        const int64_t nwg = nq * ns;
        const int64_t rounds = (nwg + 255) / 256;
        double cost = (double)rounds * (rs + 1.5);
        if (nwg >= 384) cost *= 0.85;
        if (cost < best - 1e-9) {
            best = cost;
            best_rs = rs;
        }
    }
    return best_rs;
}

bool half_form_shape_ok(int64_t d) {
    return d % 64 == 0 && d >= 192 && d <= (1 << 20);
}

namespace {
struct TileLds {
    size_t reg, dma;
};
template <int RS>
constexpr TileLds tile_lds() {
    return {FUSED_HDR + TileCfg<RS>::STAGE_BYTES, FUSED_HDR + DmaCfg<RS>::STAGE_BYTES};
}
constexpr size_t P64_LDS = PCfg<8, 1, false>::LDS_BYTES, P64X2_LDS = PCfg<8, 1, true>::LDS_BYTES,
                 P128_LDS = PCfg<8, 2, false>::LDS_BYTES;
static_assert(P128_LDS <= 160 * 1024 && P64X2_LDS <= 80 * 1024, "the LDS of one CU / of half a CU");
TileLds tile_lds_of(int rs) {
    return rs == 2 ? tile_lds<2>() : rs == 4 ? tile_lds<4>() : rs == 5 ? tile_lds<5>() : rs == 6 ? tile_lds<6>()
         : rs == 8 ? tile_lds<8>() : rs == 10 ? tile_lds<10>() : tile_lds<12>();
}
}

FusedPlan plan_tiles(int64_t B, int64_t N, int64_t d, int form) {
    FusedPlan p = {};
    p.form = form;
    p.rs = form == FORM_HALF ? BANK_BS / 16 : pick_rs(B, N, d, form == FORM_SPLIT);
    p.BS = 16 * p.rs;
    const int64_t n_stiles = (N + p.BS - 1) / p.BS, n_qtiles = (B + BQ - 1) / BQ;
    const int64_t grid = (n_stiles + 7) / 8 * 8 * n_qtiles;
    if (grid > 0x7fffffff) p.status = NW_ERR_UNSUPPORTED;
    else p.n_stiles = (int)n_stiles, p.n_qtiles = (int)n_qtiles, p.grid = (int)grid;
    return p;
}

FusedPlan plan_fused(int64_t B, int64_t N, int64_t d, int64_t C, int form, int out, int k, bool norms, bool dot, int cus,
                     const FwdOpts& opts) {
    (void)C;
    if (B < 0 || N < 0 || d < 0 || B >= (1 << 30) || N >= (1 << 30) || d >= (1 << 30)) {
        FusedPlan none = {};
        return none.status = NW_ERR_UNSUPPORTED, none;
    }
    FusedPlan p = plan_tiles(B, N, d, form);
    if (p.status != NW_OK) return p;
    auto refuse = [&p](int status) { p.status = status; return p; };
    if (cus <= 0) cus = device_cu_count();
    const TileLds lds = tile_lds_of(p.rs);
    const bool split = form == FORM_SPLIT;
    p.out = out;
    p.dma = (d % BK) == 0 && (uint64_t)(BQ + p.BS) * 2 * d * 4 < 0xffffffffull;
    if (form == FORM_HALF) {
        if ((out != OUT_NONE && out != OUT_CAND) || !half_form_shape_ok(d)) return refuse(NW_ERR_UNSUPPORTED);
        if (out == OUT_CAND && (k < 1 || k > 32)) return refuse(NW_ERR_UNSUPPORTED);
        p.persistent = true;
    } else {
        if (!p.dma && (p.rs & 1)) return refuse(NW_ERR_UNSUPPORTED);
        p.persistent = split && out == OUT_NONE && p.rs == 8 && p.grid >= 4 * (int64_t)cus && d >= 3 * BK &&
                       !env_flag(KNOB_NO_PERSISTENT);
    }
    p.run_tables = p.persistent && out != OUT_CAND;
    if (p.run_tables && p.BS > 192) return refuse(NW_ERR_UNSUPPORTED);
    if (split && (!p.dma || !norms)) return refuse(NW_ERR_INVALID_ARG);
    if (out == OUT_CAND && form == FORM_F32) return refuse(NW_ERR_INVALID_ARG);
    if (out == OUT_CAND && split && p.rs == 12) return refuse(NW_ERR_UNSUPPORTED);
    if (out_is_win(out) && form == FORM_F32) return refuse(NW_ERR_INVALID_ARG);
    if (out_is_win(out) && p.rs == 12) return refuse(NW_ERR_UNSUPPORTED);
    if (p.persistent) {
        p.mode = MODE_F16;
        p.split_queries = true;
        int wgs = cus & ~7;
        const int wg_cap = opts.persistent_wgs & ~7;
        if (wg_cap >= 8 && wg_cap < wgs) wgs = wg_cap;
        int variant = form == FORM_HALF ? 3 : knob(KNOB_PVAR);
        if (variant < 0 || variant > 3) {
            const double rows64 = 1.15 * ((B + 63) / 64 * 64);
            variant = ((B + 255) / 256 * 256 <= rows64) ? 3 : ((B + 127) / 128 * 128 <= rows64) ? 2 : 1;
        }
        p.variant = variant;
        p.workgroups = variant == 1 ? 2 * wgs : wgs;
        const int qg = (knob(KNOB_QG) >= 1 && knob(KNOB_QG) <= 64) ? knob(KNOB_QG) : 8;
        p.qgroup = variant != 3 ? qg : qg >= 2 ? qg / 2 : 1;
        p.lds_bytes = variant == 3 ? (size_t)P12::LDS_BYTES : variant == 2 ? P128_LDS : variant == 1 ? P64X2_LDS : P64_LDS;
        return p;
    }
    if (split) {
        const int force_split = knob(KNOB_SPLIT_QUERIES) == KNOB_UNSET ? -1 : knob(KNOB_SPLIT_QUERIES);
        const bool raw_ok = force_split == 0 || (force_split < 0 && 2 * (int64_t)p.grid <= 3 * (int64_t)cus);
        p.split_queries = !raw_ok;
        p.mode = raw_ok ? MODE_F16Q : MODE_F16;
    } else {
        p.mode = !p.dma ? MODE_REG : (norms && !dot) ? MODE_DMA_SN : MODE_DMA;
    }
    p.lds_bytes = p.mode == MODE_REG ? lds.reg : lds.dma;
    return p;
}

static size_t fused_workspace_bytes(int64_t B, int64_t N, int64_t d, int64_t C) {
    size_t need = 0;
    for (int form : {FORM_F32, FORM_SPLIT, FORM_HALF}) {
        if (form == FORM_HALF && !half_form_shape_ok(d)) continue;
        const int BS = plan_tiles(B, N, d, form).BS;
        const size_t n = fused_layout(B, (N + BS - 1) / BS, BS, nullptr, nullptr, C);
        need = n > need ? n : need;
    }
    return need;
}

FwdLayout fwd_layout(int64_t B, int64_t N, int64_t d, int64_t C, void* base) {
    FwdLayout L = {};
    L.base = static_cast<char*>(base);
    if (B <= 0 || N <= 0) return L;
    size_t off = 0;
    auto take = [&](size_t bytes) {
        const FwdLayout::Area a = {off, al256(bytes)};
        off += a.bytes;
        return a;
    };
    const size_t scores = (size_t)B * (size_t)N * sizeof(float), fused = fused_workspace_bytes(B, N, d, C);
    L.main = take(scores > fused ? scores : fused);
    L.q_rows = take((size_t)B * (size_t)d * sizeof(float));
    L.q_scale = take((size_t)B * sizeof(float));
    L.q_norm2 = take((size_t)B * sizeof(float));
    L.lse = take((size_t)B * sizeof(float));
    L.n_slices = aggregate_slices(B, N);
    L.slices = take(L.n_slices > 1 ? (size_t)L.n_slices * (size_t)B * (size_t)(2 + (C > 0 ? C : 0)) * sizeof(float) : 0);
    L.total = off;
    return L;
}

bool fused_eligible(const float* q, const float* s, int64_t B, int64_t N, int64_t d, int64_t C) {
    const bool aligned = ((reinterpret_cast<uintptr_t>(q) | reinterpret_cast<uintptr_t>(s)) & 15) == 0;
    return N > 25 && d >= 4 && (d % 4) == 0 && aligned && B < (1 << 30) && N < (1 << 30) &&
           d < (1 << 30) && C < (1 << 30) && (8 + C) * 4 <= 160 * 1024;
}

int launch_fused(const FusedArgs& a, int form, int kind) {
    const int out = a.cand ? OUT_CAND : a.row_logw ? OUT_WGT : (a.win_lo && a.win_hi) ? OUT_WIN : a.scores ? OUT_SCORES : OUT_NONE;
    const FusedPlan p = plan_fused(a.B, a.N, a.d, a.C, form, out, a.cand ? a.cand->k : 0, a.s_norm2 != nullptr,
                                   kind == NW_SCORE_DOT, 0, fwd_opts());
#define NW_KIND_CASE(K) case K: return launch_fused_kind<K>(a, p);
    switch (kind) {
        NW_FOR_EACH_KIND(NW_KIND_CASE)
        default: return NW_ERR_UNSUPPORTED;
    }
#undef NW_KIND_CASE
}

namespace {
struct KnnWs {
    CandOut cand;
    int64_t n_stiles;
    int kcp;
};
bool knn_shape_ok(int form, int64_t B, int64_t N, int64_t d, int64_t k) {
    const bool d_ok = form == FORM_HALF ? half_form_shape_ok(d) : form == FORM_SPLIT && d >= BK && d % BK == 0 && d <= (1 << 20);
    return B >= 0 && N > 25 && d_ok && k >= 1 && k <= 32 && k <= N && B < (1 << 30) && N < (1 << 30);
}
size_t knn_layout(int64_t B, int64_t N, int64_t d, int64_t k, int BS, char* base, KnnWs* out) {
    KnnWs w = {};
    w.n_stiles = (N + BS - 1) / BS;
    w.kcp = cand_slots((int)k, BS);
    size_t off = 0;
    auto take = [&](size_t bytes) {
        char* p = base ? base + off : nullptr;
        off += al256(bytes);
        return p;
    };
    const size_t slots = (size_t)B * (size_t)w.n_stiles * (size_t)w.kcp;
    w.cand.key = reinterpret_cast<unsigned*>(take(slots * 4));
    w.cand.row = reinterpret_cast<int*>(take(slots * 4));
    w.cand.q_rows = reinterpret_cast<float*>(take((size_t)B * (size_t)d * 4));
    w.cand.q_scale = reinterpret_cast<float*>(take((size_t)B * 4));
    w.cand.q_norm2 = reinterpret_cast<float*>(take((size_t)B * 4));
    w.cand.k = (int)k;
    if (out) *out = w;
    return off;
}
size_t knn_layout(int form, int64_t B, int64_t N, int64_t d, int64_t k, char* base, KnnWs* out) {
    return knn_layout(B, N, form == FORM_HALF ? d / 2 : d, k, plan_tiles(B, N, d, form).BS, base, out);
}
}

size_t knn_workspace_bytes(int form, int64_t B, int64_t N, int64_t d, int64_t k) {
    if (!knn_shape_ok(form, B, N, d, k) || B == 0) return 0;
    if (form == FORM_HALF) return knn_layout(form, B, N, d, k, nullptr, nullptr);
    if (pick_rs(B, N, d, true) > 10) return 0;
    size_t need = knn_layout(B, N, d, k, 16 * pick_rs(B, N, d, true), nullptr, nullptr);
    const int64_t nq = (B + BQ - 1) / BQ;
    for (int64_t qt = 1; qt <= nq && qt < 1024; ++qt) {
        const int64_t Bq = qt * BQ < B ? qt * BQ : B;
        for (int64_t n = 17; n <= N && qt * ((n + 127) / 128) < 1024; n += 16) {
            const int64_t nn = n > 26 ? n : 26;
            if (nn > N || k > nn) continue;
            const size_t x = knn_layout(Bq, nn, d, k, 16 * pick_rs(Bq, nn, d, true), nullptr, nullptr);
            need = x > need ? x : need;
        }
    }
    return need;
}

int launch_knn(const KnnCall& c) {
    const bool window = c.row_lo != nullptr && c.row_hi != nullptr;
    if (!knn_shape_ok(c.form, c.B, c.N, c.d, c.k)) return NW_ERR_UNSUPPORTED;
    if (window && c.form == FORM_HALF) return NW_ERR_UNSUPPORTED;
    if (c.B == 0) return NW_OK;
    KnnWs w;
    const size_t need = knn_layout(c.form, c.B, c.N, c.d, c.k, static_cast<char*>(c.workspace), &w);
    if (!c.workspace || c.workspace_bytes < need) return NW_ERR_WORKSPACE;
    if (w.n_stiles * w.kcp >= (1ll << 31)) return NW_ERR_UNSUPPORTED;
    if (window) w.cand.win_lo = c.row_lo, w.cand.win_hi = c.row_hi, w.cand.win_exclude = c.exclude != 0;
    FusedArgs a = {};
    a.q = c.q, a.s = static_cast<const float*>(c.s_rows), a.s_norm2 = c.s_norm2, a.s_scale = c.s_scale;
    a.ls = c.logit_scale_dev;
    a.B = (int)c.B, a.N = (int)c.N, a.d = (int)c.d, a.C = 1, a.st = c.st, a.cand = &w.cand;
    const int rc = launch_fused(a, c.form, c.kind);
    if (rc != NW_OK) return rc;
    return launch_topk_candidates(w.cand.key, w.cand.row, c.idx, c.vals, c.B, w.n_stiles * w.kcp, c.k, c.st, window);
}

}

extern "C" size_t nw_bank_tables_bytes(int64_t N) {
    if (N <= 0 || N > 0x7fffffffLL) return 0;
    return nw::bank_tables_layout((N + nw::BANK_BS - 1) / nw::BANK_BS, nullptr, nullptr);
}

extern "C" int nw_bank_tables_build(const int64_t* sy, int64_t N, int64_t C, void* tables, size_t tables_bytes,
                                    void* stream) {
    using namespace nw;
    if (N < 0 || C < 0 || N > 0x7fffffffLL || C > 0x7fffffffLL) return NW_ERR_INVALID_ARG;
    if (N == 0) return NW_OK;
    if (!sy || !tables || (reinterpret_cast<uintptr_t>(tables) & 15)) return NW_ERR_INVALID_ARG;
    const int64_t n_stiles = (N + BANK_BS - 1) / BANK_BS;
    FusedWs ws;
    if (tables_bytes < bank_tables_layout(n_stiles, static_cast<char*>(tables), &ws)) return NW_ERR_WORKSPACE;
    return launch_run_tables(ws, sy, (int)N, (int)C, (int)n_stiles, BANK_BS, static_cast<hipStream_t>(stream));
}
```

nwhead_amd/csrc/fused_impl.h:

```cpp
#pragma once
#include <type_traits>
#include "tile_core.h"
#include "tile_dma.h"
#include "tile_f16.h"
#include "fused_plan.h"

namespace nw {

constexpr int RUN_CAP = 192;

struct FusedWs {
    float* m;
    float* den;
    int* nrun;
    int* lab;
    float* num;
    int* runid;
    int* bnd;
    int* ctab;
};
size_t fused_layout(int64_t B, int64_t n_stiles, int BS, char* base, FusedWs* ws, int64_t C = 0);
int launch_run_tables(const FusedWs& ws, const int64_t* sy, int N, int C, int n_stiles, int BS, hipStream_t st);
bool bank_tables_take(const int64_t* sy, int N, int C, int n_stiles, int BS, FusedWs* ws);
int launch_merge_runs(const FusedWs& ws, float* out, float* lse, float* m, float* den, float* num,
                      int B, int C, int n_stiles, int BS, hipStream_t st);
struct CandOut {
    unsigned* key;
    int* row;
    int k;
    float *q_rows, *q_scale, *q_norm2;
    const int *win_lo, *win_hi;
    int win_exclude;
};
constexpr int CAND_EXCLUDE = 1 << 8;
constexpr int OUT_CAND_WIN = 3;
constexpr bool out_is_cand(int out) { return out == OUT_CAND || out == OUT_CAND_WIN; }
constexpr int WIN_EXCLUDE = 1 << 30;
__host__ __device__ inline size_t fused_den_after_m(int64_t n_stiles, int64_t B) {
    return (((size_t)n_stiles * (size_t)B * 4 + 255) & ~(size_t)255) / 4;
}
__host__ __device__ inline int cand_slots(int k, int BS) { return ((k < BS ? k : BS) + 3) & ~3; }
int tile_timer_start(hipStream_t st);
void tile_timer_stop(int slot, hipStream_t st);

namespace {

template <int BS>
__device__ __forceinline__ void run_scan_wave(const int (&lab)[3], int lane, int* runid, int* runlab, int* nrun_s) {
    int flag[3];
    if (lane < 2) nrun_s[1 + lane] = BS;
    const int prev_last = __shfl_up(lab[2], 1);
    flag[0] = (lane == 0) || (lab[0] != prev_last);
    flag[1] = lab[1] != lab[0];
    flag[2] = lab[2] != lab[1];
    int incl = flag[0] + flag[1] + flag[2];
#pragma unroll
    for (int o = 1; o < 64; o <<= 1) {
        const int v = __shfl_up(incl, o);
        if (lane >= o) incl += v;
    }
    int id = incl - (flag[0] + flag[1] + flag[2]) - 1;
#pragma unroll
    for (int u = 0; u < 3; ++u) {
        const int t = 3 * lane + u;
        id += flag[u];
        if (t < BS) {
            runid[t] = id;
            if (flag[u] && (id == 1 || id == 2)) nrun_s[id] = t;
            if (flag[u]) runlab[id] = lab[u];
            if (t == BS - 1) *nrun_s = id + 1;
        }
    }
}
template <int BS>
__device__ __forceinline__ void load_tile_labels(const int64_t* __restrict__ sy, int s0, int N, int C, int lane, int (&lab)[3]) {
#pragma unroll
    for (int u = 0; u < 3; ++u) {
        const int t = 3 * lane + u, j = s0 + t;
        int64_t y = -1;
        if (t < BS && j < N) y = sy[j];
        lab[u] = ((uint64_t)y < (uint64_t)C) ? (int)y : -1;
    }
}

template <int RS, bool WIN = false>
__device__ __forceinline__ void tile_candidates(const float (&sc)[RS][4], unsigned* __restrict__ cand_key,
                                                int* __restrict__ cand_row, int B, int N, int b, int s0, int g, int st,
                                                int n_stiles, int k, const int* __restrict__ win_lo = nullptr,
                                                const int* __restrict__ win_hi = nullptr) {
    constexpr int BS = 16 * RS;
    constexpr float LN2 = 0.693147180559945309417f;
    constexpr unsigned NOPOS = 1u << 20;
    unsigned key[RS][4];
#pragma unroll
    for (int r = 0; r < RS; ++r)
#pragma unroll
        for (int e = 0; e < 4; ++e) key[r][e] = ordered_bits(sc[r][e] * LN2);
    if (s0 + BS > N) {
#pragma unroll
        for (int r = 0; r < RS; ++r)
#pragma unroll
            for (int e = 0; e < 4; ++e)
                if (s0 + 16 * r + 4 * g + e >= N) key[r][e] = 0u;
    }
    bool dead = false;
    if constexpr (WIN) {
        const bool exclude = (k & CAND_EXCLUDE) != 0;
        k &= CAND_EXCLUDE - 1;
        const int bb = b < B ? b : B - 1;
        const int lo = min(max(win_lo[bb], 0), N), hi = min(max(win_hi[bb], 0), N);
        const unsigned width = hi > lo ? (unsigned)(hi - lo) : 0u;
        const int tile_end = s0 + BS < N ? s0 + BS : N;
        const bool disjoint = width == 0u || hi <= s0 || lo >= tile_end;
        const bool covered = lo <= s0 && hi >= tile_end;
        dead = exclude ? covered : disjoint;
        if (!(exclude ? disjoint : covered)) {
            const int rel = s0 + 4 * g - lo;
#pragma unroll
            for (int r = 0; r < RS; ++r)
#pragma unroll
                for (int e = 0; e < 4; ++e)
                    if (((unsigned)(rel + 16 * r + e) < width) == exclude) key[r][e] = 0u;
        }
    }
    const int kc = k < BS ? k : BS, kcp = cand_slots(k, BS);
    const size_t base = ((size_t)b * n_stiles + st) * kcp + g;
    if (WIN && __all(dead)) {
        for (int j0 = 0; j0 < kcp; j0 += 4)
            if (b < B) {
                cand_key[base + j0] = 0u;
                cand_row[base + j0] = s0;
            }
        return;
    }
    for (int j0 = 0; j0 < kcp; j0 += 4) {
        unsigned okey = 0u;
        int orow = 0;
#pragma unroll
        for (int u = 0; u < 4; ++u) {
            if (j0 + u >= kc) break;
            unsigned m = 0u;
#pragma unroll
            for (int r = 0; r < RS; ++r) m = max(max(m, key[r][0]), max(key[r][1], max(key[r][2], key[r][3])));
            m = group4_max_u32(m);
            unsigned pos = NOPOS;
#pragma unroll
            for (int r = RS - 1; r >= 0; --r)
#pragma unroll
                for (int e = 3; e >= 0; --e) pos = key[r][e] == m ? (unsigned)(16 * r + e) : pos;
            const unsigned win = group4_min_u32(pos + 4u * g);
            const unsigned mine = win - 4u * g;
#pragma unroll
            for (int r = 0; r < RS; ++r)
#pragma unroll
                for (int e = 0; e < 4; ++e) key[r][e] = (unsigned)(16 * r + e) == mine ? 0u : key[r][e];
            if (g == u) {
                okey = m;
                orow = s0 + (int)win;
            }
        }
        if (b < B) {
            cand_key[base + j0] = okey;
            cand_row[base + j0] = orow;
        }
    }
}

template <int RS>
__device__ __forceinline__ void window_scores(float (&sc)[RS][4], const int* __restrict__ win_lo, const int* __restrict__ win_hi,
                                              bool exclude, int b, int B, int N, int s0, int g) {
    constexpr int BS = 16 * RS;
    const int bb = b < B ? b : B - 1;
    const int lo = min(max(win_lo[bb], 0), N), hi = min(max(win_hi[bb], 0), N);
    const unsigned width = hi > lo ? (unsigned)(hi - lo) : 0u;
    const int tile_end = s0 + BS < N ? s0 + BS : N;
    const bool disjoint = width == 0u || hi <= s0 || lo >= tile_end;
    const bool covered = lo <= s0 && hi >= tile_end;
    if (!(exclude ? disjoint : covered)) {
// ... 183 lines not shown
                    }
            }
            const float s0v = group4_sum(S0[0] + S0[1]);
            float s1v = 0.f, s2v = 0.f;
            if (nrun >= 2) s1v = group4_sum(S1[0] + S1[1]);
            if (nrun == 3) s2v = group4_sum(S2[0] + S2[1]);
            dloc = (s0v + s1v) + s2v;
            if (g == 0 && b < B) {
                ws_num[((size_t)st * BS) * B + b] = s0v;
                if (nrun >= 2) ws_num[((size_t)st * BS + 1) * B + b] = s1v;
                if (nrun == 3) ws_num[((size_t)st * BS + 2) * B + b] = s2v;
            }
        } else {
            float dl[4] = {0.f, 0.f, 0.f, 0.f};
#pragma unroll
            for (int r = 0; r < RS; ++r) dl[r & 3] += (sc[r][0] + sc[r][1]) + (sc[r][2] + sc[r][3]);
            dloc = group4_sum((dl[0] + dl[1]) + (dl[2] + dl[3]));
            for (int run_base = 0; run_base < nrun; run_base += 16) {
                f32x4 P0 = {0.f, 0.f, 0.f, 0.f}, P1 = P0, P2 = P0, P3 = P0;
                const int want = run_base + i;
#pragma unroll
                for (int r = 0; r < RS; ++r) {
                    const int4 rid = *reinterpret_cast<const int4*>(runid + 16 * r + 4 * g);
                    P0 = __builtin_amdgcn_mfma_f32_16x16x4f32(rid.x == want ? 1.f : 0.f, sc[r][0], P0, 0, 0, 0);
                    P1 = __builtin_amdgcn_mfma_f32_16x16x4f32(rid.y == want ? 1.f : 0.f, sc[r][1], P1, 0, 0, 0);
                    P2 = __builtin_amdgcn_mfma_f32_16x16x4f32(rid.z == want ? 1.f : 0.f, sc[r][2], P2, 0, 0, 0);
                    P3 = __builtin_amdgcn_mfma_f32_16x16x4f32(rid.w == want ? 1.f : 0.f, sc[r][3], P3, 0, 0, 0);
                }
                const f32x4 P = (P0 + P1) + (P2 + P3);
                if (b < B) {
#pragma unroll
                    for (int j = 0; j < 4; ++j) {
                        const int run = run_base + 4 * g + j;
                        if (run < nrun) ws_num[((size_t)st * BS + run) * B + b] = P[j];
                    }
                }
            }
        }
        NW_FSTAMP(4);
        if (g == 0 && b < B) {
            ws_m[(size_t)st * B + b] = mloc;
            ws_den[(size_t)st * B + b] = dloc;
        }
    }
    NW_FSTAMP(5);
    if (qt == 0) {
        const int nrun = *nrun_s;
        if (tid == 0) ws_nrun[st] = nrun;
        for (int x = tid; x < nrun; x += TILE_THREADS) ws_lab[(size_t)st * BS + x] = runlab[x];
    }
}


template <int RS, int KIND, int OUT, int MODE>
__global__ __launch_bounds__(TILE_THREADS, (RS <= 5 ? 4 : 2)) void nw_fused_kernel(
    const float* __restrict__ q, const float* __restrict__ s, const int64_t* __restrict__ sy,
    const float* __restrict__ s_norm2, const float* __restrict__ s_scale, const float* __restrict__ q_norm2,
    const float* __restrict__ q_scale, const float* __restrict__ logit_scale,
    float* __restrict__ scores, float* __restrict__ ws_m,
    float* __restrict__ ws_den, int* __restrict__ ws_nrun, int* __restrict__ ws_lab,
    float* __restrict__ ws_num, int B, int N, int d, int C, int n_stiles, int n_qtiles,
    const float* __restrict__ row_logw) {
    using Cfg = TileCfg<RS>;
    constexpr int BS = Cfg::BS;
    constexpr bool NEED_NORM = (KIND != NW_SCORE_DOT);
    extern __shared__ __attribute__((aligned(16))) char smem[];
    float* qn2 = reinterpret_cast<float*>(smem);
    float* qsc_s = qn2 + 64;
    float* sn2 = qsc_s + 64;
    float* ssc = sn2 + RUN_CAP;
    int* runid = reinterpret_cast<int*>(ssc + RUN_CAP);
    int* runlab = runid + RUN_CAP;
    int* nrun_s = runlab + RUN_CAP;
    constexpr int HDR = (128 + 4 * RUN_CAP + 4) * 4;
    static_assert(HDR % 16 == 0, "stage buffers must stay 16-byte aligned");
    float4* stage = reinterpret_cast<float4*>(smem + HDR);

    int qt, st;
    if (!decode_block(n_stiles, n_qtiles, qt, st)) return;
    const int q0 = qt * BQ, s0 = st * BS;
    const int tid = threadIdx.x, wave = tid >> 6, lane = tid & 63;
    const int i = lane & 15, g = lane >> 4;
    NW_FSTAMP(0);

    if ((MODE == MODE_DMA_SN || mode_is_f16(MODE)) && NEED_NORM) {
        for (int t = tid; t < BS; t += TILE_THREADS) sn2[t] = s_norm2[min(s0 + t, N - 1)];
    }
    if (mode_is_f16(MODE)) {
        for (int t = tid; t < BS; t += TILE_THREADS) ssc[t] = s_scale[min(s0 + t, N - 1)];
    }
    if (MODE == MODE_F16) {
        if (NEED_NORM)
            for (int t = tid; t < BQ; t += TILE_THREADS) qn2[t] = q_norm2[min(q0 + t, B - 1)];
        for (int t = tid; t < BQ; t += TILE_THREADS) qsc_s[t] = q_scale[min(q0 + t, B - 1)];
    }
    if (!out_is_cand(OUT) && wave == 0) {
        int lab[3];
        load_tile_labels<BS>(sy, s0, N, out_is_win(OUT) ? C & (WIN_EXCLUDE - 1) : C, lane, lab);
        run_scan_wave<BS>(lab, lane, runid, runlab, nrun_s);
    }

    NW_FSTAMP(1);
    const int nk = (d + BK - 1) / BK;
    const int rot = st % nk;
    f32x4 acc[RS];
    if (mode_is_f16(MODE)) {
        tile_dots_f16x2<RS, MODE == MODE_F16Q>(q, s, B, N, d, q0, s0, stage, acc, rot, qn2, qsc_s);
        __syncthreads();
    } else if (MODE == MODE_REG) {
        tile_dots<RS, NEED_NORM>(q, s, B, N, d, q0, s0, stage, qn2, sn2, acc, rot);
    } else {
        tile_dots_dma<RS, NEED_NORM, NEED_NORM && MODE == MODE_DMA>(q, s, B, N, d, q0, s0, stage, qn2, sn2, acc, rot);
    }
    if (MODE != MODE_DMA_SN && !mode_is_f16(MODE) && NEED_NORM && s_norm2 != nullptr) {
        for (int t = tid; t < BS; t += TILE_THREADS) sn2[t] = s_norm2[min(s0 + t, N - 1)];
        __syncthreads();
    }

    NW_FSTAMP(2);
    fused_epilogue<RS, KIND, OUT, MODE>(acc, qn2, sn2, ssc, runid, runlab, nrun_s, qsc_s, logit_scale,
                                        scores, ws_m, ws_den, ws_nrun, ws_lab, ws_num, B, N, q0, s0, qt, st, n_stiles, C, row_logw);
    NW_FSTAMP(6);
}


constexpr size_t FUSED_HDR = (128 + 4 * RUN_CAP + 4) * 4;

struct QueryRows {
    const float *rows, *norm2, *scale;
};

template <int RS, int KIND>
int launch_f16p(const FusedArgs& a, const FusedPlan& p, const QueryRows& q, const FusedWs& ws);
template <int KIND, bool HALF, bool CAND>
int launch_p12(const FusedPlan& p, const FusedArgs& a, const QueryRows& q, const FusedWs& ws);

template <int RS, int KIND>
int launch_fused_rs(const FusedArgs& a, const FusedPlan& p) {
    constexpr int BS = 16 * RS;
    const CandOut* cand = a.cand;
    hipStream_t st = a.st;
    FusedWs ws = {};
    if (!cand) {
        if (!a.ws || !a.ws->base) return NW_ERR_WORKSPACE;
        const size_t need = fused_layout(a.B, p.n_stiles, BS, a.ws->base + a.ws->main.off, &ws, a.C);
        if (need > a.ws->main.bytes) return NW_ERR_WORKSPACE;
    }
    if (p.status != NW_OK) return p.status;
    if (p.run_tables && !bank_tables_take(a.sy, a.N, a.C, p.n_stiles, BS, &ws)) {
        const int rc = launch_run_tables(ws, a.sy, a.N, a.C, p.n_stiles, BS, st);
        if (rc != NW_OK) return rc;
    }
    QueryRows q = {a.q, nullptr, nullptr};
    if (p.split_queries) {
        float* const qr = cand ? cand->q_rows : a.ws->at(a.ws->q_rows);
        float* const qsc = cand ? cand->q_scale : a.ws->at(a.ws->q_scale);
        float* const qn = cand ? cand->q_norm2 : a.ws->at(a.ws->q_norm2);
        const int rc = p.form == FORM_HALF ? launch_pack_rows_f16(a.q, qr, qsc, qn, a.B, a.d, st) : launch_split_rows(a.q, qr, qsc, qn, a.B, a.d, st);
        if (rc != NW_OK) return rc;
        q = {qr, qn, qsc};
    }
    const bool head_window = out_is_win(p.out);
    float* scores = cand ? reinterpret_cast<float*>(cand->key) : head_window ? reinterpret_cast<float*>(const_cast<int*>(a.win_lo)) : a.scores;
    int* lab = cand ? cand->row : ws.lab;
    const bool window = cand && cand->win_lo && cand->win_hi;
    const int c_or_k = cand ? (cand->k | (window && cand->win_exclude ? CAND_EXCLUDE : 0))
                            : (a.C | (head_window && a.win_exclude ? WIN_EXCLUDE : 0));
    if (window) {
        ws.nrun = const_cast<int*>(cand->win_lo);
        ws.m = reinterpret_cast<float*>(const_cast<int*>(cand->win_hi));
    }
#define NW_TILE(OUT_, MODE_)                                                                                           \
    hipLaunchKernelGGL((nw_fused_kernel<RS, KIND, OUT_, MODE_>), dim3(p.grid), dim3(TILE_THREADS), p.lds_bytes, st, q.rows, \
                       a.s, a.sy, a.s_norm2, a.s_scale, q.norm2, q.scale, a.ls, scores, ws.m, ws.den, ws.nrun, lab, ws.num, \
                       a.B, a.N, a.d, c_or_k, p.n_stiles, p.n_qtiles, p.out == OUT_WGT ? a.row_logw : nullptr)
#define NW_TILE_CASE(MODE_) \
    case MODE_: if (p.out == OUT_SCORES) NW_TILE(OUT_SCORES, MODE_); else NW_TILE(OUT_NONE, MODE_); break
    if (p.out == OUT_CAND && p.persistent) {
        if constexpr (RS == 8) {
            if (p.form == FORM_HALF && p.variant == 3) return launch_p12<KIND, true, true>(p, a, q, ws);
        }
        return NW_ERR_UNSUPPORTED;
    }
    if (p.out == OUT_CAND) {
        if constexpr (RS == 12) {
            return NW_ERR_UNSUPPORTED;
        } else {
            if (window) {
                if (p.mode == MODE_F16Q) NW_TILE(OUT_CAND_WIN, MODE_F16Q); else NW_TILE(OUT_CAND_WIN, MODE_F16);
            } else {
                if (p.mode == MODE_F16Q) NW_TILE(OUT_CAND, MODE_F16Q); else NW_TILE(OUT_CAND, MODE_F16);
            }
            NW_CHECK_LAUNCH();
            return NW_OK;
        }
    }
    if (out_is_win(p.out)) {
        if constexpr (RS == 12) {
            return NW_ERR_UNSUPPORTED;
        } else {
            const bool weighted = p.out == OUT_WGT;
            if (p.persistent || p.run_tables || !mode_is_f16(p.mode)) return NW_ERR_UNSUPPORTED;
            if (weighted ? (!a.row_logw || !a.win_lo != !a.win_hi) : (!a.win_lo || !a.win_hi)) return NW_ERR_UNSUPPORTED;
            float* const den = ws.den;
            if (den != ws.m + fused_den_after_m(p.n_stiles, a.B) || a.C >= WIN_EXCLUDE) return NW_ERR_UNSUPPORTED;
            ws.den = reinterpret_cast<float*>(const_cast<int*>(a.win_hi));
            if (weighted) {
                if (p.mode == MODE_F16Q) NW_TILE(OUT_WGT, MODE_F16Q); else NW_TILE(OUT_WGT, MODE_F16);
            } else {
                if (p.mode == MODE_F16Q) NW_TILE(OUT_WIN, MODE_F16Q); else NW_TILE(OUT_WIN, MODE_F16);
            }
            ws.den = den;
            NW_CHECK_LAUNCH();
            return launch_merge_runs(ws, a.out, a.lse, a.m, a.den, a.num, a.B, a.C, p.n_stiles, BS, st);
        }
    }
    const int timer_slot = tile_timer_start(st);
    if (p.persistent) {
        const int rc = launch_f16p<RS, KIND>(a, p, q, ws);
        if (rc != NW_OK) return rc;
    } else {
        switch (p.mode) {
            NW_TILE_CASE(MODE_REG);
            NW_TILE_CASE(MODE_DMA);
            NW_TILE_CASE(MODE_DMA_SN);
            NW_TILE_CASE(MODE_F16);
            NW_TILE_CASE(MODE_F16Q);
        }
    }
#undef NW_TILE_CASE
#undef NW_TILE
    tile_timer_stop(timer_slot, st);
    NW_CHECK_LAUNCH();
    return launch_merge_runs(ws, a.out, a.lse, a.m, a.den, a.num, a.B, a.C, p.n_stiles, BS, st);
}

}

template <int KIND>
int launch_fused_kind(const FusedArgs& a, const FusedPlan& p) {
    switch (p.rs) {
        case 2: return launch_fused_rs<2, KIND>(a, p);
        case 4: return launch_fused_rs<4, KIND>(a, p);
        case 5: return launch_fused_rs<5, KIND>(a, p);
        case 6: return launch_fused_rs<6, KIND>(a, p);
        case 8: return launch_fused_rs<8, KIND>(a, p);
        case 10: return launch_fused_rs<10, KIND>(a, p);
        default: return launch_fused_rs<12, KIND>(a, p);
    }
}

}
#include "fused_f16p.h"
#include "fused_f16p12.h"
namespace nw {
namespace {
template <int KIND, bool HALF, bool CAND>
int launch_p12(const FusedPlan& p, const FusedArgs& a, const QueryRows& q, const FusedWs& ws) {
    static const bool attr = hipFuncSetAttribute(reinterpret_cast<const void*>(nw_fused_f16p_kernel_w12<KIND, HALF, CAND>),
                                                 hipFuncAttributeMaxDynamicSharedMemorySize, (int)P12::LDS_BYTES) == hipSuccess;
    (void)attr;
    float* m = CAND ? reinterpret_cast<float*>(a.cand->key) : ws.m;
    float* den = CAND ? reinterpret_cast<float*>(a.cand->row) : ws.den;
    hipLaunchKernelGGL((nw_fused_f16p_kernel_w12<KIND, HALF, CAND>), dim3(p.workgroups), dim3(P12::THREADS), p.lds_bytes, a.st,
                       q.rows, a.s, a.s_norm2, a.s_scale, q.norm2, q.scale, a.ls, ws.runid, ws.nrun, ws.bnd, m, den, ws.num, a.B,
                       a.N, HALF ? a.d / 2 : a.d, p.n_stiles, (a.B + P12::BQP - 1) / P12::BQP, p.qgroup, CAND ? a.cand->k : 0);
    NW_CHECK_LAUNCH();
    return NW_OK;
}

template <int RS, int KIND>
int launch_f16p(const FusedArgs& a, const FusedPlan& p, const QueryRows& q, const FusedWs& ws) {
    if constexpr (RS == 8) {
#define NW_LAUNCH_P(TWO_, QB_)                                                                                        \
    hipLaunchKernelGGL((nw_fused_f16p_kernel<RS, KIND, TWO_, QB_>), dim3(p.workgroups), dim3(TILE_THREADS), p.lds_bytes, \
                       a.st, q.rows, a.s, a.s_norm2, a.s_scale, q.norm2, q.scale, a.ls, ws.runid, ws.nrun, ws.bnd, ws.m, \
                       ws.den, ws.num, a.B, a.N, a.d, p.n_stiles, (a.B + 64 * (QB_) - 1) / (64 * (QB_)), p.qgroup)
        switch (p.variant) {
            case 3: return p.form == FORM_HALF ? launch_p12<KIND, true, false>(p, a, q, ws) : launch_p12<KIND, false, false>(p, a, q, ws);
            case 2: NW_LAUNCH_P(false, 2); break;
            case 1: NW_LAUNCH_P(true, 1); break;
            default: NW_LAUNCH_P(false, 1); break;
        }
#undef NW_LAUNCH_P
        NW_CHECK_LAUNCH();
        return NW_OK;
    } else {
        return NW_ERR_UNSUPPORTED;
    }
}
}

#define NW_INSTANTIATE_FUSED_KIND(K) template int launch_fused_kind<K>(const FusedArgs&, const FusedPlan&);

}
```

nwhead_amd/csrc/fused_plan.h:

```cpp
#pragma once
#include <hip/hip_runtime.h>
#include <stddef.h>
#include <stdint.h>

namespace nw {

struct FwdOpts;
struct FwdLayout;
struct CandOut;
#define NW_FOR_EACH_KIND(X) \
    X(NW_SCORE_EUCLIDEAN) X(NW_SCORE_HYPERSPHERE) X(NW_SCORE_COSINE) X(NW_SCORE_DOT) X(NW_SCORE_CLIP)

enum { MODE_REG = 0, MODE_DMA = 1, MODE_DMA_SN = 2, MODE_F16 = 3, MODE_F16Q = 4 };
constexpr bool mode_is_f16(int m) { return m == MODE_F16 || m == MODE_F16Q; }
enum { OUT_NONE = 0, OUT_SCORES = 1, OUT_CAND = 2, OUT_WIN = 4, OUT_WGT = 5 };
constexpr bool out_is_win(int out) { return out == OUT_WIN || out == OUT_WGT; }
enum { FORM_F32 = 0, FORM_SPLIT = 1, FORM_HALF = 2 };

struct FusedPlan {
    int form;
    int status;
    int rs, BS, n_stiles;
    int n_qtiles, grid;
    int mode, out;
    bool dma;
    bool persistent;
    bool split_queries;
    bool run_tables;
    int variant, workgroups, qgroup;
    size_t lds_bytes;
};
FusedPlan plan_tiles(int64_t B, int64_t N, int64_t d, int form);
FusedPlan plan_fused(int64_t B, int64_t N, int64_t d, int64_t C, int form, int out, int k, bool norms, bool dot, int cus,
                     const FwdOpts& opts);

struct FusedArgs {
    const float* q;
    const float* s;
    const int64_t* sy;
    const float *s_norm2, *s_scale, *ls;
    float *out, *scores, *lse, *m, *den, *num;
    const FwdLayout* ws;
    int B, N, d, C;
    hipStream_t st;
    const CandOut* cand;
    const int *win_lo, *win_hi;
    int win_exclude;
    const float* row_logw;
};
int launch_fused(const FusedArgs& a, int form, int kind);

}
```

nwhead_amd/csrc/nw_internal.h:

```cpp
#pragma once
#include <hip/hip_runtime.h>
#include <stdint.h>
#include "../../include/nwhead_hip.h"

#define NW_LOG_EPS 1e-12f
#define NW_NORM_EPS 1e-12f

#define NW_CHECK_LAUNCH()                          \
    do {                                           \
        if (hipGetLastError() != hipSuccess) return NW_ERR_LAUNCH; \
    } while (0)

namespace nw {

int launch_scores(const float* q, const float* s, float* scores, int64_t B, int64_t N, int64_t d,
                  int kind, const float* logit_scale_dev, int sup_batched, hipStream_t st);

int aggregate_slices(int64_t B, int64_t N);
int launch_aggregate(const float* scores, const int64_t* sy, int labels_batched, float* out,
                     float* lse, float* weights, float* m, float* den, float* num, int64_t B,
                     int64_t N, int64_t C, hipStream_t st, float* slice_ws = nullptr, size_t slice_ws_floats = 0);

int launch_merge(const float* m, const float* den, const float* num, float* out, int64_t G,
                 int64_t B, int64_t C, int64_t sm, int64_t sd, int64_t sn, const int64_t* class_lo,
// ... 12 lines not shown
    int nchunks, k_chunk;
};

constexpr size_t XGEMM_TAIL_BYTES = 512;
KSplit xgemm_plan(int64_t M, int64_t Nn, int64_t K);
struct XgemmReduce {
    const float* part;
    const float* fac;
    const float* gfac;
    const float* rowscale;
    const float* Xo;
    float* out;
    int64_t M, Nn;
    int nchunks, fac_inverse, blocks;
};
int launch_xgemm(bool x_km, const float* X, int64_t ldx, int64_t x_rows, const float* Y, int64_t ldy, int64_t y_rows,
                 float* part, const float* fac, int fac_inverse, const float* gfac, const float* rowscale,
                 const float* Xo, float* out, int64_t M, int64_t Nn, int64_t K, const KSplit& p, hipStream_t st,
                 XgemmReduce* defer = nullptr, const XgemmReduce* pending = nullptr);

struct BwdQueryCall {
    const float *q, *s_split, *s_scale, *s_norm2;
    const int64_t* sy;
    const int32_t *row_lo, *row_hi;
    int exclude;
    const float *lse, *out, *gout;
    float *gq, *glogit_scale;
    void* workspace;
    size_t workspace_bytes;
    int64_t B, N, d, C;
    int kind;
    const float* logit_scale_dev;
    int row_chunks;
    hipStream_t st;
    const float* row_logw;
    float* glogw;
};
bool bank_head_shape_ok(int64_t N, int64_t d, int64_t C);
bool bwd_query_shape_ok(int64_t B, int64_t N, int64_t d, int64_t C);
size_t bwd_query_workspace_bytes(int64_t B, int64_t N, int64_t d, int64_t C, int row_chunks);
size_t bwd_logw_workspace_bytes(int64_t B, int64_t N, int64_t d, int64_t C, int row_chunks, bool want_gq);
int launch_bwd_query(const BwdQueryCall& c);

struct FwdValuesCall {
    const float *q, *s_split, *s_scale, *s_norm2;
    const float *v_split, *v_scale;
    const float* row_logw;
    const int32_t *row_lo, *row_hi;
    int exclude;
    const float* lse;
    float* out;
    void* workspace;
    size_t workspace_bytes;
    int64_t B, N, d, T;
    int kind;
    const float* logit_scale_dev;
    int row_chunks;
    hipStream_t st;
};
bool fwd_values_shape_ok(int64_t B, int64_t N, int64_t d, int64_t T);
size_t fwd_values_workspace_bytes(int64_t B, int64_t N, int64_t d, int64_t T, int row_chunks);
int launch_fwd_values(const FwdValuesCall& c);

struct BwdValuesCall {
    const float *q, *s_split, *s_scale, *s_norm2;
    const float *v_split, *v_scale;
    const float* row_logw;
    const int32_t *row_lo, *row_hi;
    int exclude;
    const float *lse, *out, *gout;
    float *gq, *glogit_scale;
    void* workspace;
    size_t workspace_bytes;
    int64_t B, N, d, T;
    int kind;
    const float* logit_scale_dev;
    int row_chunks;
    hipStream_t st;
};
bool bwd_values_shape_ok(int64_t B, int64_t N, int64_t d, int64_t T);
size_t bwd_values_workspace_bytes(int64_t B, int64_t N, int64_t d, int64_t T, int row_chunks);
int launch_bwd_values(const BwdValuesCall& c);

struct BwdValuesSupportCall {
    const float *q, *s_split, *s_scale, *s_norm2;
    const float* v_rows;
    const float* row_logw;
    const int32_t *row_lo, *row_hi;
    int exclude;
    const float *lse, *out, *gout;
    float *gvalues, *glogw;
    void* workspace;
    size_t workspace_bytes;
    int64_t B, N, d, T;
    int kind;
    const float* logit_scale_dev;
    int query_chunks;
    hipStream_t st;
};
size_t bwd_values_support_workspace_bytes(int64_t B, int64_t N, int64_t d, int64_t T, int query_chunks, bool want_gvalues);
int launch_bwd_values_support(const BwdValuesSupportCall& c);

struct FwdOpts {
    const char* tables = nullptr;
    size_t tables_bytes = 0;
    const int64_t* tables_sy = nullptr;
    int64_t tables_N = -1;
    int persistent_wgs = 0;
    int force_split = 0;
    int operand_form = 0;
};
const FwdOpts& fwd_opts();
constexpr int KNOB_UNSET = -2147483647 - 1;
enum Knob { KNOB_PVAR, KNOB_QG, KNOB_TILE_RS, KNOB_NO_PERSISTENT, KNOB_SPLIT_QUERIES, KNOB_BWD_NO_MFMA, KNOB_BWD_SPLIT,
            KNOB_XGEMM_WGS, KNOB_SPLIT_LBITS, KNOB_CONV_MAX_WGS, KNOB_CONV_SKIP_CFGS, KNOB_CONV_FORCE_CFG, KNOB_COUNT };
int knob(int id);

int launch_topk(const float* scores, int64_t* idx, float* vals, int64_t B, int64_t N, int64_t k, hipStream_t st);
int launch_topk_candidates(const unsigned* keys, const int* rows, int64_t* idx, float* vals, int64_t B, int64_t M, int64_t k,
                           hipStream_t st, bool pad_empty = false);
struct KnnCall {
    const float* q;
    const void* s_rows;
    const float *s_scale, *s_norm2;
    int64_t* idx;
    float* vals;
    void* workspace;
    size_t workspace_bytes;
    int64_t B, N, d, k;
    int kind;
    const float* logit_scale_dev;
    hipStream_t st;
    int form;
    const int32_t *row_lo, *row_hi;
    int exclude;
};
size_t knn_workspace_bytes(int form, int64_t B, int64_t N, int64_t d, int64_t k);
int launch_knn(const KnnCall& c);
int launch_influence_select(const float* vals, const int64_t* rows, const int64_t* sy, const int64_t* qy, const float* logp,
                            const float* lse, float* infl, int64_t* labels, int64_t B, int64_t k, int64_t N, int64_t C,
                            hipStream_t st);
int launch_knn_merge(const float* vals, const int* rows, const int* labels, int64_t G, int64_t B, int64_t kc, int64_t stride_g,
                     int64_t k, int64_t C, int64_t* idx, float* val_out, int64_t* label_out, float* out, hipStream_t st);
int tile_timer_enable(bool on);
int tile_timer_read(double* total_us, int64_t* launches);
int pick_rs(int64_t B, int64_t N, int64_t d, bool f16 = false);
bool fused_eligible(const float* q, const float* s, int64_t B, int64_t N, int64_t d, int64_t C);
struct FwdLayout {
    using Area = nw::Area;
    Area main, q_rows, q_scale, q_norm2, lse, slices;
    int n_slices;
    size_t total;
    char* base;
    float* at(const Area& a) const { return base ? reinterpret_cast<float*>(base + a.off) : nullptr; }
    bool fits(size_t buffer_bytes) const { return base && buffer_bytes >= total; }
};
FwdLayout fwd_layout(int64_t B, int64_t N, int64_t d, int64_t C, void* base);
int launch_split_rows(const float* x, float* out, float* scale, float* norm2, int64_t rows, int64_t d,
                      hipStream_t st);
int launch_pack_rows_f16(const float* x, void* out, float* scale, float* norm2, int64_t rows, int64_t d, hipStream_t st);
bool half_form_shape_ok(int64_t d);

__device__ __forceinline__ float wave_sum(float v) {
#pragma unroll
    for (int o = 32; o > 0; o >>= 1) v += __shfl_xor(v, o);
    return v;
}
__device__ __forceinline__ float wave_max(float v) {
#pragma unroll
    for (int o = 32; o > 0; o >>= 1) v = fmaxf(v, __shfl_xor(v, o));
    return v;
}

__device__ __forceinline__ float block_sum(float v, float* red) {
    v = wave_sum(v);
    __syncthreads();
    if ((threadIdx.x & 63) == 0) red[threadIdx.x >> 6] = v;
    __syncthreads();
    float r = 0.f;
    const int nw_ = (blockDim.x + 63) >> 6;
    for (int w = 0; w < nw_; ++w) r += red[w];
    return r;
}
template <int N>
__device__ __forceinline__ void wait_vmcnt() {
    static_assert(N >= 0 && N < 64, "vmcnt is a 6-bit field");
    asm volatile("s_waitcnt vmcnt(%0)" ::"n"(N) : "memory");
}

__device__ __forceinline__ float block_max(float v, float* red) {
    v = wave_max(v);
    __syncthreads();
    if ((threadIdx.x & 63) == 0) red[threadIdx.x >> 6] = v;
    __syncthreads();
    float r = -INFINITY;
    const int nw_ = (blockDim.x + 63) >> 6;
    for (int w = 0; w < nw_; ++w) r = fmaxf(r, red[w]);
    return r;
}

__device__ __forceinline__ float fast_exp_neg(float x) {
    const float L2E_HI = 1.44269502162933349609375f, L2E_LO = 1.925963033500011e-8f;
    const float t = x * L2E_HI;
    const float e = __builtin_fmaf(x, L2E_HI, -t) + x * L2E_LO;
    const float r = __builtin_amdgcn_exp2f(t);
    return (x == -INFINITY) ? 0.f : __builtin_fmaf(r * e, 0.693147182464599609375f, r);
}

__device__ __forceinline__ float fast_sqrt_pos(float x) { return __builtin_amdgcn_sqrtf(fmaxf(x, 0.f)); }

__device__ __forceinline__ float group4_sum(float x) {
    typedef unsigned u2_ __attribute__((ext_vector_type(2)));
    u2_ r = __builtin_amdgcn_permlane32_swap(__float_as_uint(x), __float_as_uint(x), false, false);
    x = __uint_as_float(r[0]) + __uint_as_float(r[1]);
    r = __builtin_amdgcn_permlane16_swap(__float_as_uint(x), __float_as_uint(x), false, false);
    return __uint_as_float(r[0]) + __uint_as_float(r[1]);
}
__device__ __forceinline__ float group4_min(float x);
__device__ __forceinline__ float group4_max(float x) {
    typedef unsigned u2_ __attribute__((ext_vector_type(2)));
    u2_ r = __builtin_amdgcn_permlane32_swap(__float_as_uint(x), __float_as_uint(x), false, false);
    x = fmaxf(__uint_as_float(r[0]), __uint_as_float(r[1]));
    r = __builtin_amdgcn_permlane16_swap(__float_as_uint(x), __float_as_uint(x), false, false);
    return fmaxf(__uint_as_float(r[0]), __uint_as_float(r[1]));
}

__device__ __forceinline__ float group4_min(float x) {
    typedef unsigned u2_ __attribute__((ext_vector_type(2)));
    u2_ r = __builtin_amdgcn_permlane32_swap(__float_as_uint(x), __float_as_uint(x), false, false);
    x = fminf(__uint_as_float(r[0]), __uint_as_float(r[1]));
    r = __builtin_amdgcn_permlane16_swap(__float_as_uint(x), __float_as_uint(x), false, false);
    return fminf(__uint_as_float(r[0]), __uint_as_float(r[1]));
}

template <int NV, typename Op>
__device__ __forceinline__ void group4_each(float (&v)[NV], Op op) {
    typedef unsigned u2_ __attribute__((ext_vector_type(2)));
    u2_ r[NV];
#pragma unroll
    for (int k = 0; k < NV; ++k) r[k] = __builtin_amdgcn_permlane32_swap(__float_as_uint(v[k]), __float_as_uint(v[k]), false, false);
#pragma unroll
    for (int k = 0; k < NV; ++k) v[k] = op(__uint_as_float(r[k][0]), __uint_as_float(r[k][1]));
#pragma unroll
    for (int k = 0; k < NV; ++k) r[k] = __builtin_amdgcn_permlane16_swap(__float_as_uint(v[k]), __float_as_uint(v[k]), false, false);
#pragma unroll
    for (int k = 0; k < NV; ++k) v[k] = op(__uint_as_float(r[k][0]), __uint_as_float(r[k][1]));
}

__device__ __forceinline__ unsigned group4_max_u32(unsigned x) {
    typedef unsigned u2_ __attribute__((ext_vector_type(2)));
    u2_ r = __builtin_amdgcn_permlane32_swap(x, x, false, false);
    x = max(r[0], r[1]);
    r = __builtin_amdgcn_permlane16_swap(x, x, false, false);
    return max(r[0], r[1]);
}
__device__ __forceinline__ unsigned group4_min_u32(unsigned x) {
    typedef unsigned u2_ __attribute__((ext_vector_type(2)));
    u2_ r = __builtin_amdgcn_permlane32_swap(x, x, false, false);
    x = min(r[0], r[1]);
    r = __builtin_amdgcn_permlane16_swap(x, x, false, false);
    return min(r[0], r[1]);
}

__device__ __forceinline__ unsigned ordered_bits(float f) {
    unsigned b = __float_as_uint(f);
    if ((b & 0x7fffffffu) > 0x7f800000u) return 0xffffffffu;
    if ((b << 1) == 0) b = 0;
    return (b & 0x80000000u) ? ~b : (b | 0x80000000u);
}
__device__ __forceinline__ float ordered_bits_to_float(unsigned u) {
    return __uint_as_float((u & 0x80000000u) ? (u ^ 0x80000000u) : ~u);
}

template <int KIND>
__device__ __forceinline__ float score_from_dot(float dot, float qn2, float sn2, float scale) {
    if (KIND == NW_SCORE_DOT) return dot;
    if (KIND == NW_SCORE_EUCLIDEAN) return -fast_sqrt_pos(qn2 + sn2 - 2.f * dot);
    const float nq = fmaxf(sqrtf(qn2), NW_NORM_EPS), ns = fmaxf(sqrtf(sn2), NW_NORM_EPS);
    const float c = dot / (nq * ns);
    if (KIND == NW_SCORE_COSINE) return c;
    if (KIND == NW_SCORE_CLIP) return scale * c;
    const float a = qn2 / (nq * nq), b = sn2 / (ns * ns);
    return -fast_sqrt_pos(a + b - 2.f * c);
}


template <int KIND>
struct ScoreFactors {
    static constexpr float L2E = 1.44269504088896340736f;
    static constexpr bool DIST = (KIND == NW_SCORE_EUCLIDEAN || KIND == NW_SCORE_HYPERSPHERE);
    static constexpr bool NORMALISED = (KIND == NW_SCORE_HYPERSPHERE || KIND == NW_SCORE_COSINE || KIND == NW_SCORE_CLIP);
    static __device__ __forceinline__ float inv_norm(float n2) {
        return __builtin_amdgcn_rcpf(fmaxf(__builtin_amdgcn_sqrtf(n2), NW_NORM_EPS));
    }
    static __device__ __forceinline__ void support(float n2, float sscale, float& K, float& Base) {
        const float in = NORMALISED ? inv_norm(n2) : 1.f;
        K = sscale * in * (DIST ? -2.f * L2E * L2E : L2E);
        Base = DIST ? (NORMALISED ? n2 * in * in : n2) * (L2E * L2E) : 0.f;
    }
    static __device__ __forceinline__ void query(float n2, float qscale, float clip_scale, float& Cq, float& Bq) {
        const float in = NORMALISED ? inv_norm(n2) : 1.f;
        Cq = qscale * in * (KIND == NW_SCORE_CLIP ? clip_scale : 1.f);
        Bq = DIST ? (NORMALISED ? n2 * in * in : n2) * (L2E * L2E) : 0.f;
    }
    static __device__ __forceinline__ float base_plus(float n2, float Bq, bool separate) {
        if (!DIST) return 0.f;
        const float in = NORMALISED ? inv_norm(n2) : 1.f;
        const float t = NORMALISED ? n2 * in * in : n2;
        return separate ? __fadd_rn(__fmul_rn(t, L2E * L2E), Bq) : __builtin_fmaf(t, L2E * L2E, Bq);
    }
    static __device__ __forceinline__ float finish(float x) { return DIST ? -fast_sqrt_pos(x) : x; }
    static __device__ __forceinline__ float finish_abs(float x) { return DIST ? fast_sqrt_pos(x) : x; }
// ... 4 lines not shown
```

nwhead_amd/csrc/row_forms.h:

```cpp
#pragma once
#include "nw_internal.h"

namespace nw {

typedef _Float16 half4 __attribute__((ext_vector_type(4)));

__device__ __forceinline__ float row_amax4(float m, const float4 v) {
    return fmaxf(fmaxf(m, fmaxf(fabsf(v.x), fabsf(v.y))), fmaxf(fabsf(v.z), fabsf(v.w)));
}

__device__ __forceinline__ void row_split_accum(float& mx, float& n2, const float4 v) {
    mx = fmaxf(fmaxf(mx, fmaxf(fabsf(v.x), fabsf(v.y))), fmaxf(fabsf(v.z), fabsf(v.w)));
    n2 += v.x * v.x + v.y * v.y + v.z * v.z + v.w * v.w;
}

__device__ __forceinline__ int row_scale_exponent(float mx) {
    int e = 0;
    if (mx > 0.f && mx < INFINITY) {
        frexpf(mx, &e);
        e = 14 - e;
        if (e > 126) e = 126;
    }
    return e;
}

__device__ __forceinline__ void row_split_emit(_Float16* dst, int64_t c, const float4 v, float up, unsigned lmask) {
    const float sv[4] = {v.x * up, v.y * up, v.z * up, v.w * up};
    half4 h, l;
#pragma unroll
    for (int k = 0; k < 4; ++k) {
        h[k] = (_Float16)sv[k];
        l[k] = (_Float16)(sv[k] - (float)h[k]);
    }
    if (lmask != 0xffffu) {
        typedef unsigned short us4 __attribute__((ext_vector_type(4)));
        us4 b = __builtin_bit_cast(us4, l);
        b &= (unsigned short)lmask;
        l = __builtin_bit_cast(half4, b);
    }
    const int64_t chunk = c >> 3, within = (c & 7) * 4;
    *reinterpret_cast<half4*>(dst + chunk * 64 + within) = h;
    *reinterpret_cast<half4*>(dst + chunk * 64 + 32 + within) = l;
}

__device__ __forceinline__ void row_pack_emit(half4* dst, int64_t c, const float4 v, float up, float down, float& n2) {
    const float sv[4] = {v.x * up, v.y * up, v.z * up, v.w * up};
    half4 h;
#pragma unroll
    for (int k = 0; k < 4; ++k) {
        h[k] = (_Float16)sv[k];
        const float back = (float)h[k] * down;
        n2 = __builtin_fmaf(back, back, n2);
    }
    dst[c] = h;
}

template <typename At>
__device__ __forceinline__ float row_norm2_lane(At at, int64_t d, int lane) {
    float a = 0.f;
    for (int64_t k = lane; k < d; k += 64) {
        const float v = at(k);
        a += v * v;
    }
    return a;
}

}
```

nwhead_amd/csrc/split.hip:

```cpp
#include "nw_internal.h"
#include "row_forms.h"
#include <type_traits>
#include <cstdlib>

namespace nw {
namespace {

__global__ __launch_bounds__(256) void nw_split_rows_kernel(const float* __restrict__ x,
                                                             float* __restrict__ out,
                                                             float* __restrict__ scale,
                                                             float* __restrict__ norm2, int64_t rows,
                                                             int64_t d, unsigned lmask) {
    const int64_t r = (int64_t)blockIdx.x * 4 + (threadIdx.x >> 6);
    const int lane = threadIdx.x & 63;
    if (r >= rows) return;
    const float4* src = reinterpret_cast<const float4*>(x + r * d);
    const int64_t n4 = d / 4;
    constexpr int KEEP = 8;
    const bool in_regs = n4 <= 64 * KEEP;
    float4 keep[KEEP];
    float mx = 0.f, n2 = 0.f;
    if (in_regs) {
#pragma unroll
        for (int u = 0; u < KEEP; ++u) {
            const int64_t c = lane + 64 * u;
            keep[u] = (c < n4) ? src[c] : make_float4(0.f, 0.f, 0.f, 0.f);
        }
#pragma unroll
        for (int u = 0; u < KEEP; ++u) row_split_accum(mx, n2, keep[u]);
    } else {
        for (int64_t c = lane; c < n4; c += 64) row_split_accum(mx, n2, src[c]);
    }
    mx = wave_max(mx);
    n2 = wave_sum(n2);
    const int e = row_scale_exponent(mx);
    const float up = ldexpf(1.f, e);
    if (lane == 0) {
        scale[r] = ldexpf(1.f, -e);
        norm2[r] = n2;
    }
    _Float16* dst = reinterpret_cast<_Float16*>(out + r * d);
    auto emit = [&](int64_t c, const float4 v) { row_split_emit(dst, c, v, up, lmask); };
    if (in_regs) {
#pragma unroll
        for (int u = 0; u < KEEP; ++u) {
            const int64_t c = lane + 64 * u;
            if (c < n4) emit(c, keep[u]);
        }
    } else {
        for (int64_t c = lane; c < n4; c += 64) emit(c, src[c]);
    }
}

}

static unsigned split_lmask() {
    const int kb = knob(KNOB_SPLIT_LBITS);
    const int keep = kb == KNOB_UNSET ? 10 : kb;
    return keep >= 10 ? 0xffffu : (0xffffu << (10 - (keep < 0 ? 0 : keep))) & 0xffffu;
}

int launch_split_rows(const float* x, float* out, float* scale, float* norm2, int64_t rows, int64_t d,
                      hipStream_t st) {
    if (rows <= 0) return NW_OK;
    if ((rows + 3) / 4 > 0x7fffffffLL) return NW_ERR_INVALID_ARG;
    hipLaunchKernelGGL(nw_split_rows_kernel, dim3((unsigned)((rows + 3) / 4)), dim3(256), 0, st, x, out, scale,
                       norm2, rows, d, split_lmask());
    NW_CHECK_LAUNCH();
    return NW_OK;
}

}

extern "C" int nw_split_rows_f16x2(const float* x, float* out_split, float* row_scale, float* row_norm2,
                                   int64_t rows, int64_t d, void* stream) {
    if (rows < 0 || d < 0) return NW_ERR_INVALID_ARG;
    if (d % 32 != 0) return NW_ERR_UNSUPPORTED;
    if (rows == 0) return NW_OK;
    if (!x || !out_split || !row_scale || !row_norm2) return NW_ERR_INVALID_ARG;
    if ((reinterpret_cast<uintptr_t>(x) | reinterpret_cast<uintptr_t>(out_split)) & 15) return NW_ERR_INVALID_ARG;
    return nw::launch_split_rows(x, out_split, row_scale, row_norm2, rows, d, static_cast<hipStream_t>(stream));
}

namespace nw {
namespace {

__global__ __launch_bounds__(256) void nw_pack_rows_f16_kernel(const float* __restrict__ x, _Float16* __restrict__ out,
                                                                float* __restrict__ scale, float* __restrict__ norm2,
                                                                int64_t rows, int64_t d) {
    const int64_t r = (int64_t)blockIdx.x * 4 + (threadIdx.x >> 6);
    const int lane = threadIdx.x & 63;
    if (r >= rows) return;
    const float4* src = reinterpret_cast<const float4*>(x + r * d);
    const int64_t n4 = d / 4;
    constexpr int KEEP = 8;
    const bool in_regs = n4 <= 64 * KEEP;
    float4 keep[KEEP];
    float mx = 0.f;
    if (in_regs) {
#pragma unroll
        for (int u = 0; u < KEEP; ++u) {
            const int64_t c = lane + 64 * u;
            keep[u] = (c < n4) ? src[c] : make_float4(0.f, 0.f, 0.f, 0.f);
        }
#pragma unroll
        for (int u = 0; u < KEEP; ++u) mx = row_amax4(mx, keep[u]);
    } else {
        for (int64_t c = lane; c < n4; c += 64) mx = row_amax4(mx, src[c]);
    }
    mx = wave_max(mx);
    const int e = row_scale_exponent(mx);
    const float up = ldexpf(1.f, e), down = ldexpf(1.f, -e);
    half4* dst = reinterpret_cast<half4*>(out + r * d);
    float n2 = 0.f;
    auto emit = [&](int64_t c, const float4 v) { row_pack_emit(dst, c, v, up, down, n2); };
    if (in_regs) {
#pragma unroll
        for (int u = 0; u < KEEP; ++u) {
            const int64_t c = lane + 64 * u;
            if (c < n4) emit(c, keep[u]);
        }
    } else {
        for (int64_t c = lane; c < n4; c += 64) emit(c, src[c]);
    }
    n2 = wave_sum(n2);
    if (lane == 0) {
        scale[r] = down;
        norm2[r] = n2;
    }
}

}

int launch_pack_rows_f16(const float* x, void* out, float* scale, float* norm2, int64_t rows, int64_t d, hipStream_t st) {
    if (rows <= 0) return NW_OK;
    if ((rows + 3) / 4 > 0x7fffffffLL) return NW_ERR_INVALID_ARG;
    hipLaunchKernelGGL(nw_pack_rows_f16_kernel, dim3((unsigned)((rows + 3) / 4)), dim3(256), 0, st, x,
                       static_cast<_Float16*>(out), scale, norm2, rows, d);
    NW_CHECK_LAUNCH();
    return NW_OK;
}

}

extern "C" int nw_pack_rows_f16(const float* x, uint16_t* out_rows, float* row_scale, float* row_norm2, int64_t rows,
                                int64_t d, void* stream) {
    if (rows < 0 || d < 0) return NW_ERR_INVALID_ARG;
    if (d % 64 != 0) return NW_ERR_UNSUPPORTED;
    if (rows == 0) return NW_OK;
    if (!x || !out_rows || !row_scale || !row_norm2) return NW_ERR_INVALID_ARG;
    if ((reinterpret_cast<uintptr_t>(x) | reinterpret_cast<uintptr_t>(out_rows)) & 15) return NW_ERR_INVALID_ARG;
    return nw::launch_pack_rows_f16(x, out_rows, row_scale, row_norm2, rows, d, static_cast<hipStream_t>(stream));
}

namespace nw {
namespace {

struct BankUpdate {
    const float* x;
    const int64_t* rows;
    int64_t R, dx;
    float momentum;
    float* s_rows;
    float* s_user;
    float* s_norm2;
    float *s_split, *s_scale;
    _Float16* s_f16;
    float *f16_scale, *f16_norm2;
    int64_t N, d;
    unsigned lmask;
    int vec_x;
};

__device__ __forceinline__ float blend_rounded(float m, float om, float old, float nw_) {
#pragma clang fp contract(off)
    const float a = m * old;
    const float b = om * nw_;
    return a + b;
}

__global__ __launch_bounds__(256) void nw_bank_update_rows_kernel(const BankUpdate a) {
    const int64_t i = (int64_t)blockIdx.x * 4 + (threadIdx.x >> 6);
    const int lane = threadIdx.x & 63;
    if (i >= a.R) return;
    const int64_t r = a.rows[i];
    if (r < 0 || r >= a.N) return;
    bool later = false;
    for (int64_t j = i + 1 + lane; j < a.R; j += 64) later |= a.rows[j] == r;
    if (__any(later)) return;

    const int64_t d = a.d, dx = a.dx, n4 = d / 4;
    const float* xi = a.x + i * dx;
    float* row = a.s_rows + r * d;
    const float m = a.momentum, om = 1.0f - a.momentum;
    const bool blend = m != 0.f;
    auto mix = [&](float old, float nw_) { return blend_rounded(m, om, old, nw_); };
    auto elem = [&](int64_t k) -> float {
        const float v = k < dx ? xi[k] : 0.f;
        return blend ? mix(row[k], v) : v;
    };
    auto chunk = [&](int64_t c) -> float4 {
        float4 v;
        if (a.vec_x) {
            v = 4 * c < dx ? reinterpret_cast<const float4*>(xi)[c] : make_float4(0.f, 0.f, 0.f, 0.f);
        } else {
            const int64_t k = 4 * c;
            v.x = k < dx ? xi[k] : 0.f;
            v.y = k + 1 < dx ? xi[k + 1] : 0.f;
            v.z = k + 2 < dx ? xi[k + 2] : 0.f;
// ... 208 lines not shown
```

nwhead_amd/ops.py:

```python
from __future__ import annotations

import collections
import ctypes
import os
import weakref

import torch
from torch.autograd.function import once_differentiable

from . import _lib
from ._lib import SCORE_KINDS, NWHipError


_raw_stream = getattr(torch._C, "_cuda_getCurrentRawStream", None)


def _stream(t: torch.Tensor):
    if _raw_stream is not None:
        idx = t.device.index
        return _raw_stream(torch.cuda.current_device() if idx is None else idx)
    return torch.cuda.current_stream(t.device).cuda_stream


class _OnDevice:
# ... 528 lines not shown
            q, _ = _pad_to_bank(bank, q, None)
        return _new_call(_Call, (q, None, None, bank.packed_norm2, bank.packed, bank.packed_scale,
                                 _default_opts(persistent_wgs)))
    if bank.split is None or bank.sorted_rows is not None or q.shape[1] + bank.pad != bank.shape[1]:
        return None
    if bank.pad:
        q, s = _pad_to_bank(bank, q, s)
    sy = bank._zero_labels
    if sy is None and s is not None:
        sy = bank._zero_labels = torch.zeros(bank.shape[0], dtype=torch.int64, device=q.device)
    return _new_call(_Call, (q, s, sy, bank.norm2, bank.split, bank.scale, _default_opts()))


def _resolve(bank, q, s, sy, n_classes, positional=False, s_in_graph=False, half=False, persistent_wgs=0, norm2=None,
             torch_pad=None, run_tables=True):
    if bank is not None and bank.sorted_rows is not None and s.data_ptr() != bank.sorted_rows.data_ptr():
        ref = bank._labels_ref
        if positional or s_in_graph or not (sy is ref or (sy.data_ptr() == ref.data_ptr() and sy.shape == ref.shape)):
            bank = None
        else:
            s, sy = bank.sorted_rows, bank.sorted_labels
    if bank is not None and bank.pad:
        if s_in_graph:
            norm2, bank = bank.norm2, None
        else:
            q, s = _pad_to_bank(bank, q, s)
    if torch_pad is not None and q.shape[-1] % 4 and s.dim() == 2 and s.shape[0] > 25:
        pad = (-q.shape[-1]) % 4
        if bank is not None:
            norm2, bank = bank.norm2, None
        q, s = torch.nn.functional.pad(q, (0, pad)), torch.nn.functional.pad(s, (0, pad))
    if torch_pad:
        _lib.sync_knobs()
        d = q.shape[-1]
        if (bank is None and s.dim() == 2 and d % 32 and d >= 256
                and _lib.load().nw_bwd_uses_split(q.shape[0], s.shape[0], d + (-d) % 32, int(n_classes), 0)):
            pad = (-d) % 32
            q, s = torch.nn.functional.pad(q, (0, pad)), torch.nn.functional.pad(s, (0, pad))
    syc = _i64c(sy)
    if bank is None:
        return _new_call(_Call, (q, s, syc, norm2, None, None, _default_opts(persistent_wgs)))
    norm2, operand, scale, form = bank.norm2, bank.split, bank.scale, 0
    if half and bank.packed is not None:
        if q.shape[1] != bank.shape[1]:
            raise ValueError(f"queries of width {q.shape[1]} against an fp16 bank of (padded) width {bank.shape[1]}")
        norm2, operand, scale, form = bank.packed_norm2, bank.packed, bank.packed_scale, 1
    opts = bank._call_opts(sy, syc, n_classes, persistent_wgs, form) if run_tables else _default_opts(persistent_wgs)
    return _new_call(_Call, (q, s, syc, norm2, operand, scale, opts))


class _NoCtx:
    needs_input_grad = (False, False, False)

    @staticmethod
    def mark_non_differentiable(*a):
        pass


class _NWHeadFn(torch.autograd.Function):

    @staticmethod
    def forward(ctx, q, s, logit_scale, call, n_classes, kind_id, want_weights):
        _, _, syc, sn2, ssplit, sscale, opts = call
        _need_hip(q, s, syc, logit_scale, sn2)
        lib = _lib.load()
        qc, sc = _f32c(q), _f32c(s)
        B, d = qc.shape
        sup_b = sc.dim() == 3
        lab_b = syc.dim() == 2
        N = sc.shape[-2]
        dev = qc.device
        need_bwd = any(ctx.needs_input_grad[:2]) or (logit_scale is not None and ctx.needs_input_grad[2])
        if need_bwd and ssplit is None and not sup_b and N > 0 and lib.nw_bwd_uses_split(B, N, d, n_classes, 0):
            ssplit, sscale = torch.empty_like(sc), torch.empty(N, dtype=torch.float32, device=dev)
            sn2 = torch.empty(N, dtype=torch.float32, device=dev)
            with _OnDevice(dev):
                _lib.check(lib.nw_split_rows_f16x2(_ptr(sc), _ptr(ssplit), _ptr(sscale), _ptr(sn2), N, d, _stream(qc)),
                           "nw_split_rows_f16x2")
        out = torch.empty(B, n_classes, dtype=torch.float32, device=dev)
        scores = torch.empty(B, N, dtype=torch.float32, device=dev) if need_bwd else None
        lse = torch.empty(B, dtype=torch.float32, device=dev) if need_bwd else None
        weights = torch.empty(B, N, dtype=torch.float32, device=dev) if want_weights else None
        ls = None if logit_scale is None else _f32c(logit_scale)
        st = _stream(qc)
        ws, ws_bytes = _fwd_workspace(lib, B, N, d, n_classes, dev, st)
        with _OnDevice(dev):
            rc = lib.nw_fwd_f32(_ptr(qc), _ptr(sc), _ptr(syc), _ptr(sn2), _ptr(ssplit), _ptr(sscale), _ptr(out),
                                _ptr(scores), _ptr(lse), _ptr(weights), _ptr(ws), ws_bytes, B, N, d, n_classes, kind_id,
                                _ptr(ls), int(sup_b), int(lab_b), opts, st)
        if rc:
            _lib.check(rc, "nw_fwd_f32")
        if need_bwd:
            ctx.save_for_backward(qc, sc, syc, scores, lse, out, ls if ls is not None else torch.empty(0, device=dev))
            ctx.meta = (B, N, d, n_classes, kind_id, sup_b, lab_b, ls is not None)
            ctx.bank = (sn2, ssplit, sscale) if (ssplit is not None and not sup_b) else (None, None, None)
        if want_weights:
            ctx.mark_non_differentiable(weights)
            return out, weights
        return out

    @staticmethod
    def backward(ctx, gout, *unused):
        lib = _lib.load()
        qc, sc, syc, scores, lse, out, ls = ctx.saved_tensors
        B, N, d, C, kind_id, sup_b, lab_b, has_ls = ctx.meta
        dev = qc.device
        g = _f32c(gout)
        gq = torch.empty_like(qc)
        gs = torch.empty_like(sc)
        gls = torch.empty((), dtype=torch.float32, device=dev) if has_ls else None
        ws_bytes = lib.nw_bwd_workspace_bytes(B, N, d, C, kind_id, int(sup_b))
        ws = _workspace(ws_bytes, dev)
        bn2, bsplit, bscale = ctx.bank
        with _OnDevice(dev):
            _lib.check(lib.nw_bwd_bank_f32(_ptr(qc), _ptr(sc), _ptr(bn2), _ptr(bsplit), _ptr(bscale), _ptr(syc),
                                           _ptr(scores), _ptr(lse), _ptr(out),
                                           _ptr(g), _ptr(gq), _ptr(gs), _ptr(gls), _ptr(ws), ws_bytes,
                                           B, N, d, C, kind_id, _ptr(ls) if has_ls else None,
                                           int(sup_b), int(lab_b), _stream(qc)), "nw_bwd_bank_f32")
        return gq, gs, gls, None, None, None, None


def nw_head(q, s, sy, n_classes, kind="euclidean", logit_scale=None, return_weights=False,
            support_norm2=None, support_cache=None, validate_labels=False, row_window=None, exclude=False, row_logw=None):
    if validate_labels and sy.numel():
        _check_label_range(*(int(v) for v in torch.aminmax(sy.detach())), n_classes, one_hot=True)
    kid = _kind_id(kind)
    if kid == SCORE_KINDS["clip"] and logit_scale is None:
        raise ValueError("clip kernel needs logit_scale")
    if s.dim() == 2 and sy.dim() != 1 or s.dim() == 3 and sy.dim() != 2:
        raise ValueError("support labels must be (N,) for (N,d) supports and (B,N) for (B,N,d)")
    if support_norm2 is not None:
        if s.dim() != 2 or support_norm2.shape != (s.shape[0],):
            raise ValueError("support_norm2 must be (N,) for an (N,d) support")
        support_norm2 = _f32c(support_norm2)
    if support_cache is not None:
        if s.dim() != 2 or not support_cache.matches(s):
            raise ValueError("support_cache was prepared from another support tensor (or the tensor was modified in place "
                             "since): build a new ops.SplitBank(s) -- the split rows and norms it holds are those of the "
                             "tensor it was built from")
        _check_label_range(None, support_cache.label_max, n_classes)
    grad = torch.is_grad_enabled()
    needs_grad = grad and (q.requires_grad or s.requires_grad or (logit_scale is not None and logit_scale.requires_grad))
    if row_window is not None or row_logw is not None:
        if needs_grad or return_weights or support_cache is None:
            raise ValueError("nw_head(row_window=... / row_logw=...) is inference over a prepared bank: it needs support_cache "
                             "and has no gradients (nw_head_bank has the queries') and no return_weights")
        return nw_head_window(q, s, sy, n_classes, support_cache, row_window, exclude, kind, logit_scale, row_logw=row_logw)
    call = _resolve(support_cache, q, s, sy, n_classes, return_weights, grad and s.requires_grad,
                    not (needs_grad or return_weights), 0, support_norm2, needs_grad)
    if not needs_grad:
        return _NWHeadFn.forward(_NoCtx, call.q, call.s, logit_scale, call, int(n_classes), kid, bool(return_weights))
    return _NWHeadFn.apply(call.q, call.s, logit_scale, call, int(n_classes), kid, bool(return_weights))


def _window_empty(lo, hi, exclude, N):
    lo, hi = lo.clamp(0, N), hi.clamp(0, N)
    return ((lo <= 0) & (hi >= N)) if exclude else (hi <= lo)


def _bank_head_fwd(q, call, syc, logw, lo, hi, exclude, out, lse, kind_id, ls):
    lib = _lib.load()
    (B, d), N, C, st = q.shape, call.operand.shape[0], out.shape[1], _stream(q)
    ws, ws_bytes = _fwd_workspace(lib, B, N, d, C, q.device, st)
    entry = "nw_fwd_window_f32" if logw is None else "nw_fwd_weighted_f32"
    with _OnDevice(q.device):
        _lib.check(getattr(lib, entry)(_ptr(q), _ptr(call.operand), _ptr(call.scale), _ptr(call.norm2), _ptr(syc),
                                       *(() if logw is None else (_ptr(logw),)), _ptr(lo), _ptr(hi), int(bool(exclude)),
                                       _ptr(out), _ptr(lse), _ptr(ws), ws_bytes, B, N, d, C, kind_id, _ptr(ls), st), entry)


def _bank_head_bwd(q, operands, logw, lo, hi, exclude, lse, out, gout, kind_id, ls, want_gq=True, want_glogw=False):
    lib = _lib.load()
    ssplit, sscale, sn2, syc = operands
    (B, d), N, C, dev = q.shape, ssplit.shape[0], out.shape[1], q.device
    gq = torch.empty_like(q) if want_gq else None
    gls = torch.empty((), dtype=torch.float32, device=dev) if ls is not None else None
    glogw = torch.empty(N, dtype=torch.float32, device=dev) if want_glogw else None
    if want_glogw:
        entry, ws_bytes = "nw_bwd_query_logw_f32", lib.nw_bwd_logw_workspace_bytes(B, N, d, C, 0, int(want_gq))
    else:
        entry = "nw_bwd_query_f32" if logw is None else "nw_bwd_query_weighted_f32"
        ws_bytes = lib.nw_bwd_query_workspace_bytes(B, N, d, C, 0)
    ws = _workspace(ws_bytes, dev)
    with _OnDevice(dev):
        _lib.check(getattr(lib, entry)(_ptr(q), _ptr(ssplit), _ptr(sscale), _ptr(sn2), _ptr(syc),
                                       *(() if logw is None else (_ptr(logw),)), _ptr(lo), _ptr(hi), int(exclude), _ptr(lse),
                                       _ptr(out), _ptr(gout), _ptr(gq), *((_ptr(glogw),) if want_glogw else ()), _ptr(gls),
                                       _ptr(ws), ws_bytes, B, N, d, C, kind_id, _ptr(ls), 0, _stream(q)), entry)
    return gq, gls, glogw


def nw_head_window(q, s, sy, n_classes, bank, row_window, exclude=False, kind="euclidean", logit_scale=None, return_lse=False,
                   row_logw=None):
    _need_hip(q, s, sy, logit_scale)
    if not isinstance(bank, SplitBank):
        raise TypeError("nw_head_window runs over a prepared bank: pass ops.SplitBank(support)")
    if s.dim() != 2 or sy.dim() != 1 or sy.shape[0] != s.shape[0] or not bank.matches(s):
        raise ValueError("nw_head_window: `s` (N,d) must be the tensor the bank was prepared from and `sy` its (N,) labels")
    lib = _lib.load()
    q = _f32c(q)
    B, N, C = q.shape[0], s.shape[0], int(n_classes)
    if row_window is None and row_logw is None:
        raise ValueError("nw_head_window: needs row_window=(lo, hi), row_logw, or both")
    lo, hi = _row_window(row_window, B, q.device) if row_window is not None else (None, None)
    logw = None if row_logw is None else _row_logw(row_logw, N, q.device, "nw_head_window")
    ls = None if logit_scale is None else _f32c(logit_scale)
    kid = _kind_id(kind)
    if kid == SCORE_KINDS["clip"] and ls is None:
        raise ValueError("clip kernel needs logit_scale")
    syc = _i64c(sy)
    out = torch.empty(B, C, dtype=torch.float32, device=q.device)
    lse = torch.empty(B, dtype=torch.float32, device=q.device)
    facts = dict(split=bank.split is not None, sorted_copy=bank.sorted_rows is not None, shape=bank.shape, pad=bank.pad,
                 width=q.shape[1], B=B, n_classes=C)
    route = head_window_route(**facts) if logw is None else head_weighted_route(**facts)
    if route == "fused":
        call = _resolve_scores(bank, q)
        _bank_head_fwd(call.q, call, syc, logw, lo, hi, exclude, out, lse, kid, ls)
    elif B > 0:
        scores = nw_scores(q, s, kind, logit_scale, support_cache=bank)
        if logw is not None:
            scores += logw
        if lo is not None:
            cols = torch.arange(N, device=q.device)
            keep = (cols >= lo[:, None]) & (cols < hi[:, None])
            if exclude:
                keep = ~keep
            scores.masked_fill_(~keep, float("-inf"))
        with _OnDevice(q.device):
            _lib.check(lib.nw_aggregate_f32(_ptr(scores), _ptr(syc), _ptr(out), _ptr(lse), None, B, N, C, 0, _stream(q)),
                       "nw_aggregate_f32")
        empty = _window_empty(lo, hi, exclude, N) if logw is None else ~(scores > float("-inf")).any(dim=1)
        out = torch.where(empty[:, None], out.new_tensor(1e-12).log(), out)
        lse = lse.masked_fill(empty, float("-inf"))
    return (out, lse) if return_lse else out


def head_bank_route(*, split, sorted_copy, shape, pad, width, B, n_classes):
    return "fused" if head_bank_refusal(split=split, sorted_copy=sorted_copy, shape=shape, pad=pad, width=width, B=B,
                                        n_classes=n_classes) is None else "matrix"


HEAD_VALUES_MAX_T = 16384


def head_values_route(*, split, sorted_copy, shape, pad, width, B, T):
    fused = 1 <= T <= HEAD_VALUES_MAX_T and head_bank_refusal(split=split, sorted_copy=sorted_copy, shape=shape, pad=pad,
                                                              width=width, B=B, n_classes=1) is None
    return "fused" if fused else "matrix"


class BankValues:

    def __init__(self, values, bank):
        if not isinstance(bank, SplitBank):
            raise TypeError("BankValues: `bank` is the ops.SplitBank whose rows the values belong to")
        if not torch.is_tensor(values) or not values.is_floating_point() or values.dim() != 2 or values.shape[1] < 1:
            raise ValueError("BankValues: values is an (N, T) float tensor, T >= 1: one target row per bank row")
        if values.shape[0] != bank.shape[0]:
            raise ValueError(f"BankValues: {values.shape[0]} value rows for a bank of {bank.shape[0]} rows")
        _need_hip(values)
        self._src, self._ref = _sig(values), weakref.ref(values)
        self.requires_grad = bool(values.requires_grad)
        N, T = values.shape
        self.T, self.width = T, T + (-T) % 32
        vc = _f32c(values)
        self.rows = torch.nn.functional.pad(vc, (0, self.width - T)) if self.width != T else (vc.clone() if vc.data_ptr() == values.data_ptr() else vc)
        self.split = self.scale = None
        if N > 0 and self.width <= HEAD_VALUES_MAX_T:
            self.split = torch.empty_like(self.rows)
            self.scale = torch.empty(N, dtype=torch.float32, device=vc.device)
            norm2 = self._norm2 = torch.empty(N, dtype=torch.float32, device=vc.device)
            with _OnDevice(vc.device):
                _lib.check(_lib.load().nw_split_rows_f16x2(_ptr(self.rows), _ptr(self.split), _ptr(self.scale), _ptr(norm2),
                                                           N, self.width, _stream(vc)), "nw_split_rows_f16x2")

    def source(self):
        return self._ref()

    def refresh(self):
        t = self._ref()
        if t is None:
            raise NWHipError("BankValues.refresh: the tensor this object was prepared from is gone; build a new ops.BankValues")
        if t.data_ptr() != self._src[0] or tuple(t.shape) != self._src[1]:
            raise NWHipError("BankValues.refresh: the source tensor was replaced or reshaped; build a new ops.BankValues")
        with torch.no_grad():
            self.rows[:, :self.T].copy_(t.detach())
        if self.split is not None:
            with _OnDevice(self.rows.device):
                _lib.check(_lib.load().nw_split_rows_f16x2(_ptr(self.rows), _ptr(self.split), _ptr(self.scale), _ptr(self._norm2),
                                                           self.rows.shape[0], self.width, _stream(self.rows)),
                           "nw_split_rows_f16x2")
        self._src = _sig(t)
        self.requires_grad = bool(t.requires_grad)
        return self

    def matches(self, values):
        return _sig(values) == self._src

    def stale(self):
        t = self._ref()
        return t is not None and _sig(t) != self._src


def nw_head_values(q, s, bank, values, kind="euclidean", logit_scale=None, row_window=None, exclude=False, row_logw=None,
# ... 1704 lines not shown
```

nwhead_amd/sharded.py:

```python
from __future__ import annotations

import torch
import torch.distributed as dist

from . import ops
from ._lib import NWHipError


def shard_bounds(n_rows: int, world: int, rank: int):
    base, extra = divmod(n_rows, world)
    lo = rank * base + min(rank, extra)
    return lo, lo + base + (1 if rank < extra else 0)


def _coalesce(chunk):
    first = chunk[0]
    if first.is_contiguous() and first.dim() == 2:
        base = first.untyped_storage().data_ptr()
        step = first.numel() * first.element_size()
        if all(c.dtype == first.dtype and c.shape == first.shape and c.is_contiguous() and
               c.untyped_storage().data_ptr() == base and c.data_ptr() == first.data_ptr() + k * step
               for k, c in enumerate(chunk)):
            return first.as_strided((len(chunk) * first.shape[0], first.shape[1]), (first.shape[1], 1))
    return torch.cat(chunk, dim=0)


class ShardedBank:
    def __init__(self, feat_shard, y_shard, n_classes, kind="euclidean", logit_scale=None, group=None,
                 partial_fn=None, merge_fn=None, persistent_wgs=None, precision="fp32", row_lo=None, search_fn=None,
                 knn_merge_fn=None, search_precision="fp32"):
        if search_precision not in ("fp32", "fp16"):
            raise ValueError(f"search_precision must be 'fp32' or 'fp16', got {search_precision!r}")
        if search_precision == "fp16" and precision != "fp16":
            raise ValueError("search_precision='fp16' searches the half-precision bank: it needs precision='fp16'")
        self.search_precision = search_precision
        self.feat = feat_shard.detach().to(torch.float32).contiguous()
        self.y = y_shard.detach().to(torch.int64).contiguous()
        self.C = int(n_classes)
        self.kind, self.logit_scale, self.group = kind, logit_scale, group
        self.world = dist.get_world_size(group) if dist.is_initialized() else 1
        self._partial = partial_fn or self._hip_partial
        self._merge = merge_fn or self._hip_merge
        self._ws = None
        if persistent_wgs is None:
            persistent_wgs = 0
            if self.world > 1 and self.feat.is_cuda:
                cus = torch.cuda.get_device_properties(self.feat.device).multi_processor_count
                persistent_wgs = max(8, (cus - 8) // 8 * 8)
        self.persistent_wgs = int(persistent_wgs)
        self.class_lo, self.CL, self.y_local = None, self.C, self.y
        self._search = search_fn or self._hip_search
        self._knn_merge = knn_merge_fn or ops.nw_knn_merge
        self._search_bank = None
        self.n_total = int(self.feat.shape[0])
        if self.world > 1:
            lo = int(self.y.min()) if self.y.numel() else 0
            hi = int(self.y.max()) if self.y.numel() else -1
            box = torch.tensor([lo, hi, self.feat.shape[0]], dtype=torch.int64, device=self.feat.device)
            allb = torch.empty(self.world, 3, dtype=torch.int64, device=self.feat.device)
            dist.all_gather_into_tensor(allb.view(-1), box, group=group)
            sizes = allb[:, 2].tolist()
            self.n_total = int(sum(sizes))
            if row_lo is None:
                row_lo = sum(sizes[:dist.get_rank(group)])
            width = int((allb[:, 1] - allb[:, 0] + 1).clamp_min(1).max())
            if width < self.C:
                self.CL = width
                self.class_lo = allb[:, 0].clamp(0, max(self.C - 1, 0)).contiguous()
                self.y_local = (self.y - lo).contiguous()
        self.cache = ops.SplitBank(self.feat, precision=precision) if (partial_fn is None and self.feat.is_cuda) else None
        self.norm2 = self.cache.norm2 if self.cache is not None else None
        if self.cache is not None and self.cache.has_operand_rows:
            self.cache.build_tables(self.y_local)
        self.row_lo = int(row_lo or 0)

    def _hip_partial(self, packed_row, q):
        self._ws = ops._partials(packed_row, q, self.feat, self.y_local, self.CL, self.kind, self.logit_scale, ws=self._ws,
                                 cache=self.cache, persistent_wgs=self.persistent_wgs, own_ws=True)

    def _hip_merge(self, gathered_rows, B):
        return ops.nw_merge(gathered_rows, B, self.C, class_lo=self.class_lo, c_local=self.CL)

    def _hip_search(self, q, k):
        half = self.search_precision == "fp16" and self.cache is not None
        if half and self.cache.packed is not None:
            return ops.nw_knn(q, self.cache, k, self.kind, self.logit_scale, return_values=True, rounded=True,
                              persistent_wgs=self.persistent_wgs)
        bank = self.cache if half else self._search_bank
        if bank is None:
            bank = self.cache if (self.cache is not None and self.cache.precision == "fp32") else ops.SplitBank(self.feat)
            self._search_bank = bank
        return ops.nw_knn(q, bank, k, self.kind, self.logit_scale, return_values=True, support=self.feat)

    def knn_partial(self, q, k):
        k = int(k)
        q = q.detach().to(torch.float32).contiguous()
        B, n = q.shape[0], self.feat.shape[0]
        kk = min(k, n)
        buf = torch.empty(3, B, k, dtype=torch.int32, device=self.feat.device)
        vals = buf[0].view(torch.float32)
        if kk < k:
            vals.fill_(float("-inf"))
            buf[1:].fill_(-1)
        if kk > 0 and B > 0:
            idx, val = self._search(q, kk)
            vals[:, :kk] = val
            buf[1, :, :kk] = idx + self.row_lo
            buf[2, :, :kk] = self.y[idx]
        return buf.view(-1)

    def _knn(self, q, k, n_classes):
        k = int(k)
        if k > ops.KNN_MERGE_MAX_K:
            raise NWHipError(f"ShardedBank: k = {k} neighbours; the cross-shard merge takes at most {ops.KNN_MERGE_MAX_K}")
        if k < 1 or k > self.n_total:
            raise NWHipError(f"ShardedBank: k = {k} outside [1, N = {self.n_total}] (the rows of the whole bank)")
        if self.world > ops.KNN_MERGE_MAX_SHARDS or self.n_total >= 2 ** 31:
            raise NWHipError(f"ShardedBank: the cross-shard merge takes at most {ops.KNN_MERGE_MAX_SHARDS} shards and "
                             f"2^31 - 1 bank rows, got {self.world} and {self.n_total}")
        B, G = q.shape[0], self.world
        packed = self.knn_partial(q, k)
        if G > 1:
            gathered = torch.empty(G, packed.numel(), dtype=torch.int32, device=packed.device)
            dist.all_gather_into_tensor(gathered.view(-1), packed, group=self.group)
        else:
            gathered = packed.view(1, -1)
        n = B * k
        vals, rows, labels = (gathered[:, i * n:(i + 1) * n].view(G, B, k) for i in range(3))
        return self._knn_merge(vals.view(torch.float32), rows, labels, k, n_classes)

    def neighbors(self, q, k, return_values=False, return_labels=False):
        idx, vals, labels = self._knn(q, k, None)
        res = (idx,) + ((vals,) if return_values else ()) + ((labels,) if return_labels else ())
        return res if len(res) > 1 else idx

    def predict_knn(self, q, k):
        return self._knn(q, k, self.C)[3]

    def row_len(self, B):
        return 2 * B + B * self.CL

    def predict(self, q):
        return self.predict_stream([q], bucket=1)[0]

    def predict_stream(self, batches, bucket=8):
        if not batches:
            return []
        d = batches[0].shape[-1]
        for k, qb in enumerate(batches):
            if qb.dim() != 2 or qb.shape[1] != d:
                raise ValueError(f"predict_stream: batch {k} has shape {tuple(qb.shape)}, expected (B, {d})")
        dev, G = self.feat.device, self.world
        outs, pending = [], None
        ring = {}

        def split(out, sizes):
            pos = 0
            for n in sizes:
                outs.append(out[pos:pos + n])
                pos += n

        def finish(p):
            work, gathered, sizes = p
            if work is not None:
                work.wait()
            split(self._merge(gathered, sum(sizes)), sizes)

        for n_bucket, i0 in enumerate(range(0, len(batches), bucket)):
            chunk = batches[i0:i0 + bucket]
            sizes = [int(c.shape[0]) for c in chunk]
            Bq = sum(sizes)
            L = self.row_len(Bq)
            key = (n_bucket % 3, Bq)
            if key not in ring:
                ring[key] = (torch.empty(L, dtype=torch.float32, device=dev),
                             torch.empty(G, L, dtype=torch.float32, device=dev))
            packed, gathered = ring[key]
            qcat = chunk[0] if len(chunk) == 1 else _coalesce(chunk)
            if G == 1 and self._partial == self._hip_partial:
                split(ops.nw_head(qcat, self.feat, self.y, self.C, self.kind, self.logit_scale, support_cache=self.cache),
                      sizes)
                continue
            self._partial(packed, qcat.detach().to(torch.float32).contiguous())
            if G > 1:
                work = dist.all_gather_into_tensor(gathered.view(-1), packed, group=self.group, async_op=True)
            else:
                gathered, work = packed.view(1, L), None
            if pending is not None:
                finish(pending)
            pending = (work, gathered, sizes)
        if pending is not None:
            finish(pending)
        return outs
```

Baseline: 8.127 million query-predictions/s.

## Stream query buckets and fold next bucket's query split into merge kernel

Adds a streaming forward entry point that runs every coalesced query bucket over one shared workspace. Each bucket's merge kernel gets extra workgroups that split the next bucket's queries into f16 halves, so that preprocessing launch is hidden inside the previous launch. The merge kernel also caches per-tile maxima in LDS when there is room, to avoid re-reading them from global memory. This adds grid and LDS pressure on the merge kernel and more complex workspace aliasing between buckets.

```diff
diff --git a/include/nwhead_hip.h b/include/nwhead_hip.h
--- a/include/nwhead_hip.h
+++ b/include/nwhead_hip.h
@@ -68,6 +68,14 @@
                int64_t B, int64_t N, int64_t d, int64_t C,
                int kind, const float *logit_scale_dev,
                int sup_batched, int labels_batched, const nw_fwd_opts *opts, void *stream);
+
+size_t nw_fwd_stream_workspace_bytes(const int64_t *rows, int64_t n, int64_t N, int64_t d, int64_t C);
+int nw_fwd_stream_f32(const float *const *q, const int64_t *rows, float *const *out, int64_t n, int64_t first, int64_t count,
+                      const float *s, const int64_t *sy, const float *s_norm2,
+                      const float *s_split, const float *s_scale,
+                      void *workspace, size_t workspace_bytes,
+                      int64_t N, int64_t d, int64_t C,
+                      int kind, const float *logit_scale_dev, const nw_fwd_opts *opts, void *stream);
 
 int nw_fwd_partial_f32(const float *q, const float *s, const int64_t *sy, const float *s_norm2,
                        const float *s_split, const float *s_scale,
@@ -359,6 +367,7 @@
     int32_t n_slices, reserved;
 } nw_fwd_layout;
 int nw_debug_fwd_layout(int64_t B, int64_t N, int64_t d, int64_t C, nw_fwd_layout *layout);
+int nw_debug_fwd_stream_layout(const int64_t *rows, int64_t n, int64_t N, int64_t d, int64_t C, int64_t i, nw_fwd_layout *layout);
 #define NW_BWD_AREAS 15
 typedef struct nw_bwd_plan {
     int32_t status, route;
diff --git a/nwhead_amd/_lib.py b/nwhead_amd/_lib.py
--- a/nwhead_amd/_lib.py
+++ b/nwhead_amd/_lib.py
@@ -24,6 +24,8 @@
     "nw_pack_rows_f16": (_int, [_p, _p, _p, _p, _i64, _i64, _p]),
     "nw_bank_update_rows_f32": (_int, [_p, _p, _i64, _i64, C.c_float, _p, _p, _p, _p, _p, _p, _p, _p, _i64, _i64, _p]),
     "nw_fwd_f32": (_int, [_p, _p, _p, _p, _p, _p, _p, _p, _p, _p, _p, _sz, _i64, _i64, _i64, _i64, _int, _p, _int, _int, _p, _p]),
+    "nw_fwd_stream_workspace_bytes": (_sz, [_p, _i64, _i64, _i64, _i64]),
+    "nw_fwd_stream_f32": (_int, [_p, _p, _p, _i64, _i64, _i64, _p, _p, _p, _p, _p, _p, _sz, _i64, _i64, _i64, _int, _p, _p, _p]),
     "nw_fwd_partial_f32": (_int, [_p, _p, _p, _p, _p, _p, _p, _p, _p, _p, _sz, _i64, _i64, _i64, _i64, _int, _p, _p, _p]),
     "nw_merge_finalize_f32": (_int, [_p, _p, _p, _p, _i64, _i64, _i64, _i64, _i64, _i64, _p, _i64, _p]),
     "nw_bank_tables_bytes": (_sz, [_i64]),
@@ -113,6 +115,7 @@
     "nw_debug_tile_timing_read": (_int, [C.POINTER(C.c_double), C.POINTER(C.c_int64)]),
     "nw_debug_fwd_plan": (_int, [_i64, _i64, _i64, _i64, _int, _int, _int, _int, _int, _int, _int, _p]),
     "nw_debug_fwd_layout": (_int, [_i64, _i64, _i64, _i64, _p]),
+    "nw_debug_fwd_stream_layout": (_int, [_p, _i64, _i64, _i64, _i64, _i64, _p]),
     "nw_debug_bwd_plan": (_int, [_i64, _i64, _i64, _i64, _int, _p]),
 }
 
@@ -191,6 +194,13 @@
     return m
 
 
+def fwd_stream_layout(rows, i, N, d, C_):
+    m = FwdLayout()
+    arr = (C.c_int64 * len(rows))(*rows)
+    check(load().nw_debug_fwd_stream_layout(arr, len(rows), N, d, C_, i, C.byref(m)), "nw_debug_fwd_stream_layout")
+    return m
+
+
 BWD_ROUTES = ("valu", "mfma", "split")
 BWD_AREAS = ("A", "Rs", "rq", "gls", "qn2", "sn2", "rs", "s_split", "s_scale", "q_split", "ascale", "qv", "gfac", "part", "part2")
 
diff --git a/nwhead_amd/csrc/capi.hip b/nwhead_amd/csrc/capi.hip
--- a/nwhead_amd/csrc/capi.hip
+++ b/nwhead_amd/csrc/capi.hip
@@ -140,6 +140,20 @@
     return NW_OK;
 }
 
+extern "C" int nw_debug_fwd_stream_layout(const int64_t* rows, int64_t n, int64_t N, int64_t d, int64_t C, int64_t i,
+                                          nw_fwd_layout* layout) {
+    if (!layout || !rows || n < 0 || N < 0 || d < 0 || C < 0 || i < 0 || i >= n) return NW_ERR_INVALID_ARG;
+    for (int64_t k = 0; k < n; ++k)
+        if (rows[k] < 0) return NW_ERR_INVALID_ARG;
+    const nw::FwdLayout L = nw::fwd_stream_bucket(nw::fwd_stream_layout(rows, n, N, d, C, nullptr), i, rows[i], N, d, C);
+    const nw::FwdLayout::Area* const areas[NW_FWD_AREAS] = {&L.main, &L.q_rows, &L.q_scale, &L.q_norm2, &L.lse, &L.slices};
+    *layout = {};
+    for (int k = 0; k < NW_FWD_AREAS; ++k) layout->off[k] = areas[k]->off, layout->bytes[k] = areas[k]->bytes;
+    layout->total = L.total;
+    layout->n_slices = L.n_slices;
+    return NW_OK;
+}
+
 extern "C" int nw_debug_bwd_plan(int64_t B, int64_t N, int64_t d, int64_t C, int sup_batched, nw_bwd_plan* plan) {
     static_assert(NW_BWD_AREAS == nw::BWD_AREAS, "nw_bwd_plan lists the areas of nw::BwdPlan");
     if (!plan || B < 0 || N < 0 || d < 0 || C < 0) return NW_ERR_INVALID_ARG;
@@ -159,10 +173,16 @@
     return nw::launch_rownorm2(x, n2, rows, d, static_cast<hipStream_t>(stream));
 }
 
+struct StreamLink {
+    bool q_ready;
+    const nw::SplitJob* next;
+};
+
 static int fwd_f32(const float* q, const float* s, const int64_t* sy, const float* s_norm2, const float* s_split,
                    const float* s_scale, float* out, float* scores_out, float* lse_out, float* weights_out, void* workspace,
                    size_t workspace_bytes, const nw::FwdLayout* carved, int64_t B, int64_t N, int64_t d, int64_t C, int kind,
-                   const float* logit_scale_dev, int sup_batched, int labels_batched, hipStream_t st) {
+                   const float* logit_scale_dev, int sup_batched, int labels_batched, hipStream_t st,
+                   const StreamLink* link = nullptr) {
     if (B < 0 || N < 0 || d < 0 || C < 0) return NW_ERR_INVALID_ARG;
     if (bad_kind(kind)) return NW_ERR_UNSUPPORTED;
     if (B == 0) return NW_OK;
@@ -175,6 +195,7 @@
     const nw::FwdLayout L = carved ? *carved : nw::fwd_layout(B, N, d, C, workspace);
     nw::FusedArgs a = {q, s, sy, s_norm2, nullptr, logit_scale_dev, out, scores_out, lse_out, nullptr, nullptr, nullptr,
                        &L, (int)B, (int)N, (int)d, (int)C, st, nullptr};
+    if (link) a.q_ready = link->q_ready, a.next = link->next;
     if (form == 1) {
         const int rc = half_form_check(q, s, s_norm2, s_split, s_scale, scores_out ? scores_out : weights_out,
                                        sup_batched || labels_batched, B, N, d, C);
@@ -197,6 +218,7 @@
         if (rc != NW_OK || !weights_out) return rc;
         return nw::launch_weights_from_scores(sc_buf, a.lse, weights_out, B, N, st);
     }
+    if (a.q_ready || a.next) return NW_ERR_UNSUPPORTED;
     float* scores = scores_out;
     if (!scores && N > 0) {
         if (!L.fits(workspace_bytes)) return NW_ERR_WORKSPACE;
@@ -217,6 +239,49 @@
     OptsGuard opts_guard(opts);
     return fwd_f32(q, s, sy, s_norm2, s_split, s_scale, out, scores_out, lse_out, weights_out, workspace, workspace_bytes, nullptr,
                    B, N, d, C, kind, logit_scale_dev, sup_batched, labels_batched, static_cast<hipStream_t>(stream));
+}
+
+static bool stream_links(const float* q, const float* s, const float* s_norm2, const float* s_split, const float* s_scale,
+                         const float* out, int64_t B, int64_t N, int64_t d, int64_t C, int kind) {
+    if (B <= 0 || N <= 0 || C <= 0 || !q || !s || !out || nw::fwd_opts().operand_form != 0) return false;
+    if (!nw::fused_eligible(q, s, B, N, d, C) || !takes_split(q, s_split, s_scale, s_norm2, B, N, d)) return false;
+    const nw::FusedPlan p = nw::plan_fused(B, N, d, C, nw::FORM_SPLIT, nw::OUT_NONE, 0, true, kind == NW_SCORE_DOT, 0, nw::fwd_opts());
+    return p.status == NW_OK && p.persistent && p.split_queries;
+}
+
+extern "C" size_t nw_fwd_stream_workspace_bytes(const int64_t* rows, int64_t n, int64_t N, int64_t d, int64_t C) {
+    return nw::fwd_stream_layout(rows, n, N, d, C, nullptr).total;
+}
+
+extern "C" int nw_fwd_stream_f32(const float* const* q, const int64_t* rows, float* const* out, int64_t n, int64_t first,
+                                 int64_t count, const float* s, const int64_t* sy, const float* s_norm2, const float* s_split,
+                                 const float* s_scale, void* workspace, size_t workspace_bytes, int64_t N, int64_t d, int64_t C,
+                                 int kind, const float* logit_scale_dev, const nw_fwd_opts* opts, void* stream) {
+    if (n < 0 || first < 0 || count < 0 || first > n || count > n - first || N < 0 || d < 0 || C < 0) return NW_ERR_INVALID_ARG;
+    if (count == 0) return NW_OK;
+    if (!q || !rows || !out) return NW_ERR_INVALID_ARG;
+    for (int64_t i = 0; i < n; ++i)
+        if (rows[i] < 0) return NW_ERR_INVALID_ARG;
+    OptsGuard opts_guard(opts);
+    const nw::FwdLayout S = nw::fwd_stream_layout(rows, n, N, d, C, workspace);
+    auto links = [&](int64_t i) {
+        return !bad_kind(kind) && stream_links(q[i], s, s_norm2, s_split, s_scale, out[i], rows[i], N, d, C, kind);
+    };
+    bool mine = links(first), handed = first > 0 && mine && links(first - 1);
+    for (int64_t i = first; i < first + count; ++i) {
+        const bool following = i + 1 < n && links(i + 1);
+        const bool hand = mine && following;
+        const nw::FwdLayout L = nw::fwd_stream_bucket(S, i, rows[i], N, d, C);
+        const nw::SplitJob job = {hand ? q[i + 1] : nullptr, L.at(L.q_alt[0]), L.at(L.q_alt[1]), L.at(L.q_alt[2]),
+                                  hand ? rows[i + 1] : 0, d};
+        const StreamLink link = {handed, hand ? &job : nullptr};
+        const int rc = fwd_f32(q[i], s, sy, s_norm2, s_split, s_scale, out[i], nullptr, nullptr, nullptr, workspace,
+                               workspace_bytes, &L, rows[i], N, d, C, kind, logit_scale_dev, 0, 0,
+                               static_cast<hipStream_t>(stream), &link);
+        if (rc != NW_OK) return rc;
+        handed = hand, mine = following;
+    }
+    return NW_OK;
 }
 
 bool nw::bank_head_shape_ok(int64_t N, int64_t d, int64_t C) { return N > 25 && C >= 1 && d >= 32 && d % 32 == 0 && d <= (1 << 20); }
diff --git a/nwhead_amd/csrc/fused.hip b/nwhead_amd/csrc/fused.hip
--- a/nwhead_amd/csrc/fused.hip
+++ b/nwhead_amd/csrc/fused.hip
@@ -2,6 +2,7 @@
 #include <utility>
 #include <vector>
 #include "fused_impl.h"
+#include "row_forms.h"
 
 namespace nw {
 
@@ -101,8 +102,14 @@
     const float* __restrict__ ws_m, const float* __restrict__ ws_den, const int* __restrict__ ws_nrun,
     const int* __restrict__ ws_lab, const float* __restrict__ ws_num, float* __restrict__ out,
     float* __restrict__ lse, float* __restrict__ m_out, float* __restrict__ den_out,
-    float* __restrict__ num_out, int B, int C, int n_stiles, int BS, const int* __restrict__ ctab) {
+    float* __restrict__ num_out, int B, int C, int n_stiles, int BS, const int* __restrict__ ctab, int merge_grid,
+    const SplitJob next, unsigned lmask, int mt_lds) {
     static_assert(TMODE == 1 || TMODE == 2, "the per-class tables live in LDS (1) or in the workspace (2)");
+    if ((int)blockIdx.x >= merge_grid) {
+        const int64_t r = (int64_t)((int)blockIdx.x - merge_grid) * (MTHREADS / 64) + (threadIdx.x >> 6);
+        if (r < next.rows) row_split_wave(next.x, next.out, next.scale, next.norm2, r, next.d, threadIdx.x & 63, lmask);
+        return;
+    }
     constexpr bool LTAB = TMODE == 1;
     constexpr int ML = MTHREADS / MQ;
     constexpr int MNS = MQ + 1;
@@ -119,6 +126,7 @@
     int* thi = tlo + C;
     int* ent = thi + C;
     float* res = reinterpret_cast<float*>(lds_tab + (size_t)C * (3 + MENT));
+    float* mtile = res + (size_t)C * MNS;
     const int tid = threadIdx.x, bq = tid & (MQ - 1), sl = tid / MQ, wave = tid >> 6;
     const int b0 = blockIdx.x * MQ;
     const int b = min(b0 + bq, B - 1);
@@ -133,6 +141,13 @@
             const bool ok = t < n_stiles;
             mr[u] = ok ? ws_m[(size_t)t * B + b] : -INFINITY;
             dr[u] = ok ? ws_den[(size_t)t * B + b] : 0.f;
+        }
+        if (mt_lds) {
+#pragma unroll
+            for (int u = 0; u < MTPT; ++u) {
+                const int t = sl + u * ML;
+                if (t < n_stiles) mtile[t * MQ + bq] = mr[u];
+            }
         }
     }
     int tnr = 0, tl3[3] = {-1, -1, -1};
@@ -155,7 +170,11 @@
 #pragma unroll
         for (int u = 0; u < MTPT; ++u) M = fmaxf(M, mr[u]);
     } else {
-        for (int t = sl; t < n_stiles; t += ML) M = fmaxf(M, ws_m[(size_t)t * B + b]);
+        for (int t = sl; t < n_stiles; t += ML) {
+            const float mt = ws_m[(size_t)t * B + b];
+            if (mt_lds) mtile[t * MQ + bq] = mt;
+            M = fmaxf(M, mt);
+        }
     }
 #pragma unroll
     for (int o = 32; o >= MQ; o >>= 1) M = fmaxf(M, __shfl_xor(M, o));
@@ -251,7 +270,7 @@
             for (int k = 0; k < MENT; ++k) {
                 if (k < n) {
                     v[k] = ws_num[(size_t)e[k] * B + bb];
-                    mt[k] = ws_m[(size_t)(e[k] / BS) * B + bb];
+                    mt[k] = mt_lds ? mtile[(e[k] / BS) * MQ + q] : ws_m[(size_t)(e[k] / BS) * B + bb];
                 }
             }
 #pragma unroll
@@ -261,7 +280,7 @@
             const int t0 = tlo[c], t1 = thi[c];
             for (int t = t0 + sub; t <= t1; t += P) {
                 const int nr = ws_nrun[t];
-                const float f = __builtin_amdgcn_exp2f(ws_m[(size_t)t * B + bb] - Mq);
+                const float f = __builtin_amdgcn_exp2f((mt_lds ? mtile[t * MQ + q] : ws_m[(size_t)t * B + bb]) - Mq);
                 const int* lt = ws_lab + (size_t)t * BS;
                 for (int r = 0; r < nr; ++r)
                     if (lt[r] == c) acc += ws_num[((size_t)t * BS + r) * B + bb] * f;
@@ -419,7 +438,7 @@
 }
 
 int launch_merge_runs(const FusedWs& ws, float* out, float* lse, float* m, float* den, float* num,
-                      int B, int C, int n_stiles, int BS, hipStream_t st) {
+                      int B, int C, int n_stiles, int BS, hipStream_t st, const SplitJob* next) {
     auto lds_bytes = [&](int mq, bool tables) {
         return ((size_t)2 * (MTHREADS / 64) * mq + 2 * mq + (tables ? (size_t)C * (3 + MENT + mq + 1) : 0)) * sizeof(float);
     };
@@ -431,11 +450,21 @@
         if (lds_bytes(mq, true) > cap) mq = 1;
     }
     const bool tables = lds_bytes(mq, true) <= cap;
-    const size_t lds = lds_bytes(mq, tables);
-    const int grid = (B + mq - 1) / mq;
+    const size_t mt_bytes = (size_t)mq * n_stiles * sizeof(float);
+    const bool mt_lds = tables && lds_bytes(mq, true) + mt_bytes <= cap;
+    const size_t lds = lds_bytes(mq, tables) + (mt_lds ? mt_bytes : 0);
+    const int merge_grid = (B + mq - 1) / mq;
+    const SplitJob none = {};
+    const bool with_split = next && next->rows > 0 && tables;
+    const int64_t split_blocks = with_split ? (next->rows + MTHREADS / 64 - 1) / (MTHREADS / 64) : 0;
+    if (merge_grid + split_blocks > 0x7fffffffLL) return NW_ERR_UNSUPPORTED;
+    const int grid = merge_grid + (int)split_blocks;
+    const SplitJob& job = with_split ? *next : none;
+    const unsigned lmask = with_split ? split_lmask() : 0xffffu;
 #define NW_MERGE(P_, Q_, T_)                                                                                       \
     hipLaunchKernelGGL((nw_merge_runs_kernel<P_, Q_, T_>), dim3(grid), dim3(MTHREADS), lds, st, ws.m, ws.den, ws.nrun, \
-                       ws.lab, ws.num, out, lse, m, den, num, B, C, n_stiles, BS, ws.ctab)
+                       ws.lab, ws.num, out, lse, m, den, num, B, C, n_stiles, BS, ws.ctab, merge_grid, job, lmask,     \
+                       (int)mt_lds)
     if (!tables) {
         hipLaunchKernelGGL(nw_class_tables_kernel, dim3(1), dim3(1024), 0, st, ws.nrun, ws.lab, n_stiles, BS, C, ws.ctab);
         if (out) NW_MERGE(false, 1, 2); else NW_MERGE(true, 1, 2);
@@ -448,6 +477,8 @@
     }
 #undef NW_MERGE
     NW_CHECK_LAUNCH();
+    if (next && next->rows > 0 && !with_split)
+        return launch_split_rows(next->x, next->out, next->scale, next->norm2, next->rows, next->d, st);
     return NW_OK;
 }
 
@@ -604,6 +635,50 @@
     return L;
 }
 
+FwdLayout fwd_stream_layout(const int64_t* rows, int64_t n, int64_t N, int64_t d, int64_t C, void* base) {
+    FwdLayout L = {};
+    L.base = static_cast<char*>(base);
+    if (!rows || n <= 0 || N <= 0) return L;
+    size_t need[6] = {0, 0, 0, 0, 0, 0};
+    int64_t seen[8];
+    int n_seen = 0;
+    for (int64_t i = 0; i < n; ++i) {
+        const int64_t B = rows[i];
+        if (B <= 0) continue;
+        bool known = false;
+        for (int k = 0; k < n_seen; ++k) known = known || seen[k] == B;
+        if (known) continue;
+        if (n_seen < 8) seen[n_seen++] = B;
+        const FwdLayout one = fwd_layout(B, N, d, C, nullptr);
+        const Area* const areas[6] = {&one.main, &one.q_rows, &one.q_scale, &one.q_norm2, &one.lse, &one.slices};
+        for (int k = 0; k < 6; ++k) need[k] = areas[k]->bytes > need[k] ? areas[k]->bytes : need[k];
+    }
+    size_t off = 0;
+    auto take = [&](size_t bytes) {
+        const Area a = {off, bytes};
+        off += bytes;
+        return a;
+    };
+    L.main = take(need[0]), L.q_rows = take(need[1]), L.q_scale = take(need[2]), L.q_norm2 = take(need[3]);
+    L.lse = take(need[4]), L.slices = take(need[5]);
+    for (int k = 0; k < 3; ++k) L.q_alt[k] = take(need[1 + k]);
+    L.total = off;
+    return L;
+}
+
+FwdLayout fwd_stream_bucket(const FwdLayout& stream, int64_t i, int64_t B, int64_t N, int64_t d, int64_t C) {
+    const FwdLayout one = fwd_layout(B, N, d, C, nullptr);
+    FwdLayout L = stream;
+    L.main.bytes = one.main.bytes, L.lse.bytes = one.lse.bytes, L.slices.bytes = one.slices.bytes;
+    L.n_slices = one.n_slices;
+    if (i & 1) {
+        const Area set0[3] = {stream.q_rows, stream.q_scale, stream.q_norm2};
+        L.q_rows = stream.q_alt[0], L.q_scale = stream.q_alt[1], L.q_norm2 = stream.q_alt[2];
+        for (int k = 0; k < 3; ++k) L.q_alt[k] = set0[k];
+    }
+    return L;
+}
+
 bool fused_eligible(const float* q, const float* s, int64_t B, int64_t N, int64_t d, int64_t C) {
     const bool aligned = ((reinterpret_cast<uintptr_t>(q) | reinterpret_cast<uintptr_t>(s)) & 15) == 0;
     return N > 25 && d >= 4 && (d % 4) == 0 && aligned && B < (1 << 30) && N < (1 << 30) &&
diff --git a/nwhead_amd/csrc/fused_impl.h b/nwhead_amd/csrc/fused_impl.h
--- a/nwhead_amd/csrc/fused_impl.h
+++ b/nwhead_amd/csrc/fused_impl.h
@@ -23,7 +23,7 @@
 int launch_run_tables(const FusedWs& ws, const int64_t* sy, int N, int C, int n_stiles, int BS, hipStream_t st);
 bool bank_tables_take(const int64_t* sy, int N, int C, int n_stiles, int BS, FusedWs* ws);
 int launch_merge_runs(const FusedWs& ws, float* out, float* lse, float* m, float* den, float* num,
-                      int B, int C, int n_stiles, int BS, hipStream_t st);
+                      int B, int C, int n_stiles, int BS, hipStream_t st, const SplitJob* next = nullptr);
 struct CandOut {
     unsigned* key;
     int* row;
@@ -513,11 +513,13 @@
         if (rc != NW_OK) return rc;
     }
     QueryRows q = {a.q, nullptr, nullptr};
+    if (a.q_ready && !(p.persistent && p.split_queries && p.form == FORM_SPLIT && !cand)) return NW_ERR_UNSUPPORTED;
     if (p.split_queries) {
         float* const qr = cand ? cand->q_rows : a.ws->at(a.ws->q_rows);
         float* const qsc = cand ? cand->q_scale : a.ws->at(a.ws->q_scale);
         float* const qn = cand ? cand->q_norm2 : a.ws->at(a.ws->q_norm2);
-        const int rc = p.form == FORM_HALF ? launch_pack_rows_f16(a.q, qr, qsc, qn, a.B, a.d, st) : launch_split_rows(a.q, qr, qsc, qn, a.B, a.d, st);
+        const int rc = a.q_ready ? NW_OK
+                     : p.form == FORM_HALF ? launch_pack_rows_f16(a.q, qr, qsc, qn, a.B, a.d, st) : launch_split_rows(a.q, qr, qsc, qn, a.B, a.d, st);
         if (rc != NW_OK) return rc;
         q = {qr, qn, qsc};
     }
@@ -593,7 +595,7 @@
 #undef NW_TILE
     tile_timer_stop(timer_slot, st);
     NW_CHECK_LAUNCH();
-    return launch_merge_runs(ws, a.out, a.lse, a.m, a.den, a.num, a.B, a.C, p.n_stiles, BS, st);
+    return launch_merge_runs(ws, a.out, a.lse, a.m, a.den, a.num, a.B, a.C, p.n_stiles, BS, st, a.next);
 }
 
 }
diff --git a/nwhead_amd/csrc/fused_plan.h b/nwhead_amd/csrc/fused_plan.h
--- a/nwhead_amd/csrc/fused_plan.h
+++ b/nwhead_amd/csrc/fused_plan.h
@@ -8,6 +8,7 @@
 struct FwdOpts;
 struct FwdLayout;
 struct CandOut;
+struct SplitJob;
 #define NW_FOR_EACH_KIND(X) \
     X(NW_SCORE_EUCLIDEAN) X(NW_SCORE_HYPERSPHERE) X(NW_SCORE_COSINE) X(NW_SCORE_DOT) X(NW_SCORE_CLIP)
 
@@ -47,6 +48,8 @@
     const int *win_lo, *win_hi;
     int win_exclude;
     const float* row_logw;
+    bool q_ready;
+    const SplitJob* next;
 };
 int launch_fused(const FusedArgs& a, int form, int kind);
 
diff --git a/nwhead_amd/csrc/nw_internal.h b/nwhead_amd/csrc/nw_internal.h
--- a/nwhead_amd/csrc/nw_internal.h
+++ b/nwhead_amd/csrc/nw_internal.h
@@ -188,12 +188,21 @@
     int n_slices;
     size_t total;
     char* base;
+    Area q_alt[3];
     float* at(const Area& a) const { return base ? reinterpret_cast<float*>(base + a.off) : nullptr; }
     bool fits(size_t buffer_bytes) const { return base && buffer_bytes >= total; }
 };
 FwdLayout fwd_layout(int64_t B, int64_t N, int64_t d, int64_t C, void* base);
+FwdLayout fwd_stream_layout(const int64_t* rows, int64_t n, int64_t N, int64_t d, int64_t C, void* base);
+FwdLayout fwd_stream_bucket(const FwdLayout& stream, int64_t i, int64_t B, int64_t N, int64_t d, int64_t C);
 int launch_split_rows(const float* x, float* out, float* scale, float* norm2, int64_t rows, int64_t d,
                       hipStream_t st);
+unsigned split_lmask();
+struct SplitJob {
+    const float* x;
+    float *out, *scale, *norm2;
+    int64_t rows, d;
+};
 int launch_pack_rows_f16(const float* x, void* out, float* scale, float* norm2, int64_t rows, int64_t d, hipStream_t st);
 bool half_form_shape_ok(int64_t d);
 
diff --git a/nwhead_amd/csrc/row_forms.h b/nwhead_amd/csrc/row_forms.h
--- a/nwhead_amd/csrc/row_forms.h
+++ b/nwhead_amd/csrc/row_forms.h
@@ -43,6 +43,45 @@
     *reinterpret_cast<half4*>(dst + chunk * 64 + 32 + within) = l;
 }
 
+__device__ __forceinline__ void row_split_wave(const float* __restrict__ x, float* __restrict__ out, float* __restrict__ scale,
+                                               float* __restrict__ norm2, int64_t r, int64_t d, int lane, unsigned lmask) {
+    const float4* src = reinterpret_cast<const float4*>(x + r * d);
+    const int64_t n4 = d / 4;
+    constexpr int KEEP = 8;
+    const bool in_regs = n4 <= 64 * KEEP;
+    float4 keep[KEEP];
+    float mx = 0.f, n2 = 0.f;
+    if (in_regs) {
+#pragma unroll
+        for (int u = 0; u < KEEP; ++u) {
+            const int64_t c = lane + 64 * u;
+            keep[u] = (c < n4) ? src[c] : make_float4(0.f, 0.f, 0.f, 0.f);
+        }
+#pragma unroll
+        for (int u = 0; u < KEEP; ++u) row_split_accum(mx, n2, keep[u]);
+    } else {
+        for (int64_t c = lane; c < n4; c += 64) row_split_accum(mx, n2, src[c]);
+    }
+    mx = wave_max(mx);
+    n2 = wave_sum(n2);
+    const int e = row_scale_exponent(mx);
+    const float up = ldexpf(1.f, e);
+    if (lane == 0) {
+        scale[r] = ldexpf(1.f, -e);
+        norm2[r] = n2;
+    }
+    _Float16* dst = reinterpret_cast<_Float16*>(out + r * d);
+    if (in_regs) {
+#pragma unroll
+        for (int u = 0; u < KEEP; ++u) {
+            const int64_t c = lane + 64 * u;
+            if (c < n4) row_split_emit(dst, c, keep[u], up, lmask);
+        }
+    } else {
+        for (int64_t c = lane; c < n4; c += 64) row_split_emit(dst, c, src[c], up, lmask);
+    }
+}
+
 __device__ __forceinline__ void row_pack_emit(half4* dst, int64_t c, const float4 v, float up, float down, float& n2) {
     const float sv[4] = {v.x * up, v.y * up, v.z * up, v.w * up};
     half4 h;
diff --git a/nwhead_amd/csrc/split.hip b/nwhead_amd/csrc/split.hip
--- a/nwhead_amd/csrc/split.hip
+++ b/nwhead_amd/csrc/split.hip
@@ -14,47 +14,12 @@
     const int64_t r = (int64_t)blockIdx.x * 4 + (threadIdx.x >> 6);
     const int lane = threadIdx.x & 63;
     if (r >= rows) return;
-    const float4* src = reinterpret_cast<const float4*>(x + r * d);
-    const int64_t n4 = d / 4;
-    constexpr int KEEP = 8;
-    const bool in_regs = n4 <= 64 * KEEP;
-    float4 keep[KEEP];
-    float mx = 0.f, n2 = 0.f;
-    if (in_regs) {
-#pragma unroll
-        for (int u = 0; u < KEEP; ++u) {
-            const int64_t c = lane + 64 * u;
-            keep[u] = (c < n4) ? src[c] : make_float4(0.f, 0.f, 0.f, 0.f);
-        }
-#pragma unroll
-        for (int u = 0; u < KEEP; ++u) row_split_accum(mx, n2, keep[u]);
-    } else {
-        for (int64_t c = lane; c < n4; c += 64) row_split_accum(mx, n2, src[c]);
-    }
-    mx = wave_max(mx);
-    n2 = wave_sum(n2);
-    const int e = row_scale_exponent(mx);
-    const float up = ldexpf(1.f, e);
-    if (lane == 0) {
-        scale[r] = ldexpf(1.f, -e);
-        norm2[r] = n2;
-    }
-    _Float16* dst = reinterpret_cast<_Float16*>(out + r * d);
-    auto emit = [&](int64_t c, const float4 v) { row_split_emit(dst, c, v, up, lmask); };
-    if (in_regs) {
-#pragma unroll
-        for (int u = 0; u < KEEP; ++u) {
-            const int64_t c = lane + 64 * u;
-            if (c < n4) emit(c, keep[u]);
-        }
-    } else {
-        for (int64_t c = lane; c < n4; c += 64) emit(c, src[c]);
-    }
-}
-
-}
-
-static unsigned split_lmask() {
+    row_split_wave(x, out, scale, norm2, r, d, lane, lmask);
+}
+
+}
+
+unsigned split_lmask() {
     const int kb = knob(KNOB_SPLIT_LBITS);
     const int keep = kb == KNOB_UNSET ? 10 : kb;
     return keep >= 10 ? 0xffffu : (0xffffu << (10 - (keep < 0 ? 0 : keep))) & 0xffffu;
diff --git a/nwhead_amd/ops.py b/nwhead_amd/ops.py
--- a/nwhead_amd/ops.py
+++ b/nwhead_amd/ops.py
@@ -704,6 +704,79 @@
     if not needs_grad:
         return _NWHeadFn.forward(_NoCtx, call.q, call.s, logit_scale, call, int(n_classes), kid, bool(return_weights))
     return _NWHeadFn.apply(call.q, call.s, logit_scale, call, int(n_classes), kid, bool(return_weights))
+
+
+def nw_head_stream(buckets, s, sy, n_classes, kind="euclidean", logit_scale=None, support_cache=None, rows=None):
+    if rows is None:
+        buckets = list(buckets)
+        for k, qb in enumerate(buckets):
+            if qb.dim() != 2 or qb.shape[1] != buckets[0].shape[-1]:
+                raise ValueError(f"nw_head_stream: bucket {k} has shape {tuple(qb.shape)}, expected (B, {buckets[0].shape[-1]})")
+            if torch.is_grad_enabled() and qb.requires_grad:
+                raise ValueError("nw_head_stream is inference: call nw_head per bucket for gradients")
+        rows = [int(qb.shape[0]) for qb in buckets]
+    rows = [int(r) for r in rows]
+    n = len(rows)
+    if n == 0:
+        return []
+    kid = _kind_id(kind)
+    if kid == SCORE_KINDS["clip"] and logit_scale is None:
+        raise ValueError("clip kernel needs logit_scale")
+    if s.dim() != 2 or sy.dim() != 1:
+        raise ValueError("nw_head_stream: one shared (N,d) support with (N,) labels")
+    if support_cache is not None:
+        if not support_cache.matches(s):
+            raise ValueError("support_cache was prepared from another support tensor (or the tensor was modified in place since)")
+        _check_label_range(None, support_cache.label_max, n_classes)
+    grad = torch.is_grad_enabled()
+    if grad and (s.requires_grad or (logit_scale is not None and logit_scale.requires_grad)):
+        raise ValueError("nw_head_stream is inference: call nw_head per bucket for gradients")
+    C = int(n_classes)
+    rows_c = (ctypes.c_int64 * n)(*rows)
+    qptr, optr = (ctypes.c_void_p * n)(), (ctypes.c_void_p * n)()
+    it = iter(buckets)
+    qcs, outs, shared, width = [], [], None, None
+
+    def prepare(upto):
+        nonlocal shared, width
+        while len(qcs) < upto:
+            k, qb = len(qcs), next(it)
+            if width is None and qb.dim() == 2:
+                width = qb.shape[1]
+            if qb.dim() != 2 or qb.shape[0] != rows[k] or qb.shape[1] != width:
+                raise ValueError(f"nw_head_stream: bucket {k} has shape {tuple(qb.shape)}, expected ({max(rows[k], 0)}, {width})")
+            if grad and qb.requires_grad:
+                raise ValueError("nw_head_stream is inference: call nw_head per bucket for gradients")
+            call = _resolve(support_cache, qb, s, sy, n_classes, False, False, True, 0, None, False)
+            qc = _f32c(call.q)
+            if shared is None:
+                shared = (_f32c(call.s),) + tuple(call[2:])
+                _need_hip(shared[0], shared[1], logit_scale, shared[2])
+            _need_hip(qc)
+            out = torch.empty(rows[k], C, dtype=torch.float32, device=shared[0].device)
+            qptr[k], optr[k] = qc.data_ptr(), out.data_ptr()
+            qcs.append(qc)
+            outs.append(out)
+
+    prepare(1)
+    sc, syc, sn2, ssplit, sscale, opts = shared
+    lib = _lib.load()
+    dev, N, d = sc.device, sc.shape[0], qcs[0].shape[1]
+    ls = None if logit_scale is None else _f32c(logit_scale)
+    st = _stream(sc)
+    need = lib.nw_fwd_stream_workspace_bytes(rows_c, n, N, d, C)
+    ws = _workspace(need, dev, st)
+    first, step = 0, 1
+    with _OnDevice(dev):
+        while first < n:
+            count = min(step, n - first)
+            prepare(min(n, first + count + 1))
+            rc = lib.nw_fwd_stream_f32(qptr, rows_c, optr, n, first, count, _ptr(sc), _ptr(syc), _ptr(sn2), _ptr(ssplit),
+                                       _ptr(sscale), _ptr(ws), need, N, d, C, kid, _ptr(ls), opts, st)
+            if rc:
+                _lib.check(rc, "nw_fwd_stream_f32")
+            first, step = first + count, 2 * step
+    return outs
 
 
 def _window_empty(lo, hi, exclude, N):
diff --git a/nwhead_amd/sharded.py b/nwhead_amd/sharded.py
--- a/nwhead_amd/sharded.py
+++ b/nwhead_amd/sharded.py
@@ -166,6 +166,20 @@
                 work.wait()
             split(self._merge(gathered, sum(sizes)), sizes)
 
+        if G == 1 and self._partial == self._hip_partial:
+            chunks = [batches[i0:i0 + bucket] for i0 in range(0, len(batches), bucket)]
+            qcats = (c[0] if len(c) == 1 else _coalesce(c) for c in chunks)
+            sizes = [[int(b.shape[0]) for b in c] for c in chunks]
+            if len(chunks) == 1 or (torch.is_grad_enabled() and (
+                    any(b.requires_grad for b in batches) or (self.logit_scale is not None and self.logit_scale.requires_grad))):
+                res = [ops.nw_head(qc, self.feat, self.y, self.C, self.kind, self.logit_scale, support_cache=self.cache)
+                       for qc in qcats]
+            else:
+                res = ops.nw_head_stream(qcats, self.feat, self.y, self.C, self.kind, self.logit_scale,
+                                         support_cache=self.cache, rows=[sum(z) for z in sizes])
+            for out, z in zip(res, sizes):
+                split(out, z)
+            return outs
         for n_bucket, i0 in enumerate(range(0, len(batches), bucket)):
             chunk = batches[i0:i0 + bucket]
             sizes = [int(c.shape[0]) for c in chunk]
@@ -177,10 +191,6 @@
                              torch.empty(G, L, dtype=torch.float32, device=dev))
             packed, gathered = ring[key]
             qcat = chunk[0] if len(chunk) == 1 else _coalesce(chunk)
-            if G == 1 and self._partial == self._hip_partial:
-                split(ops.nw_head(qcat, self.feat, self.y, self.C, self.kind, self.logit_scale, support_cache=self.cache),
-                      sizes)
-                continue
             self._partial(packed, qcat.detach().to(torch.float32).contiguous())
             if G > 1:
                 work = dist.all_gather_into_tensor(gathered.view(-1), packed, group=self.group, async_op=True)
```

Result: no change. 8.170 million query-predictions/s, median of 6 (+0.5%).
